# dark-Stallion/alac

Measured on AMD Instinct MI355X. Metric: encode Msamples/s (bit-exact) 44.1kHz/16-bit stereo, 1/2/4/8 GPU, higher is better.
Workload: dtype int32 (int16 PCM, int16 coefficients)

## Files before the change

alac_amd/csrc/alac_capi.hip:

```cpp
#include "alac_hip.h"
#include "alac_dev.hpp"
#include "alac_kernels.hpp"
#include "alac_verify.hpp"
#include "alac_encode_v1_types.hpp"
#include "alac_host.hpp"

#include <cstdio>
#include <cstdlib>
#include <cstring>
#include <new>
#include <string>
#include <vector>

using namespace alacdev;
using namespace alachost;

struct alac_hip_ctx {
    int device = 0;
    hipStream_t stream = nullptr;
    bool ownStream = false;
    std::string err;
    bool profile = false;
    std::vector<hipEvent_t> events;
    uint32_t profCalls = 0;
    std::vector<bool> profLane;
    V1Streams vs{};
    bool vsReady = false;
    hipStream_t mcStream = nullptr;
    hipEvent_t mcFork = nullptr, mcJoin = nullptr;
    bool mcReady = false;
    uint32_t *errHost = nullptr;
    uint32_t *errDev = nullptr;
    uint64_t *tabHost = nullptr;
    uint64_t tabCap = 0;
    hipEvent_t tabDone = nullptr;
    AlacOptions opt;
};

namespace alacdev {

const AlacOptionKey *alac_option_keys(uint32_t *count)
{
    static const AlacOptionKey table[] = {
        {"thru", "ALAC_HIP_THRU", &AlacOptions::thru, -1, 1},
        {"narrow", "ALAC_HIP_NARROW", &AlacOptions::narrow, -1, 1},
        {"split_coder", "ALAC_HIP_SPLIT_CODER", &AlacOptions::splitCoder, 0, 1},
        {"overlap_pos", "ALAC_HIP_OVERLAP_POS", &AlacOptions::overlapPos, 0, 1},
        {"fused", "ALAC_HIP_FUSED", &AlacOptions::fused, 0, 1},
        {"fold", "ALAC_HIP_FOLD", &AlacOptions::fold, 0, 1},
        {"fast_mode", nullptr, &AlacOptions::fastMode, 0, 1},
        {"encoder_lane", "ALAC_HIP_ENCODER", &AlacOptions::laneEncoder, 0, 1},
        {"decoder_lane", "ALAC_HIP_DECODER", &AlacOptions::laneDecoder, 0, 1},
        {"dec_fused", "ALAC_HIP_DEC_FUSED", &AlacOptions::decFused, -1, 1},
        {"dec_pair", "ALAC_HIP_DEC_PAIR", &AlacOptions::decPair, 0, 1},
        {"dec_direct", "ALAC_HIP_DEC_DIRECT", &AlacOptions::decDirect, 0, 2},
        {"stage_taps", "ALAC_HIP_STAGE_TAPS", &AlacOptions::stageTaps, 0, 1},
        {"lpc", nullptr, &AlacOptions::lpc, 0, 1},
        {"debug_lose_handoff", "ALAC_HIP_DEBUG_LOSE_HANDOFF", &AlacOptions::loseHandoff, 0, 1},
        {"debug_waves", nullptr, &AlacOptions::debugWaves, 0, 1},
    };
    if (count) *count = (uint32_t)(sizeof(table) / sizeof(table[0]));
    return table;
}

AlacOptions alac_options_from_env()
{
    AlacOptions o;
    uint32_t n = 0;
    const AlacOptionKey *t = alac_option_keys(&n);
    for (uint32_t i = 0; i < n; i++) {
        const char *v = t[i].env ? getenv(t[i].env) : nullptr;
        if (!v || !*v) continue;
        const bool lane = t[i].slot == &AlacOptions::laneEncoder || t[i].slot == &AlacOptions::laneDecoder;
        if (lane && strcmp(v, "lane") == 0) v = "1";
        char *end = nullptr;
        const long x = strtol(v, &end, 10);
        if (*end == '\0' && x >= t[i].lo && x <= t[i].hi) o.*(t[i].slot) = (int32_t)x;
    }
    return o;
}

const AlacOptionKey *alac_option_find(const char *key)
{
    if (!key) return nullptr;
    uint32_t n = 0;
    const AlacOptionKey *t = alac_option_keys(&n);
    for (uint32_t i = 0; i < n; i++)
        if (strcmp(t[i].name, key) == 0) return t + i;
    return nullptr;
}

}

namespace {

int32_t fail(alac_hip_ctx *ctx, int32_t code, const char *what, hipError_t e = hipSuccess)
{
    if (ctx) {
        ctx->err = what;
        if (e != hipSuccess) {
            ctx->err += ": ";
            ctx->err += hipGetErrorString(e);
        }
    }
    return code;
}

auto on_fail(alac_hip_ctx *ctx) { return [ctx](int32_t code, const char *what, hipError_t e) { return fail(ctx, code, what, e); }; }

bool format_ok(const alac_hip_format *f)
{
    if (!f) return false;
    if (!(f->bit_depth == 16 || f->bit_depth == 20 || f->bit_depth == 24 || f->bit_depth == 32)) return false;
    if (f->num_channels < 1 || f->num_channels > kMaxChannels) return false;
    if (f->frame_size == 0 || f->frame_size > (1u << 20)) return false;
    return true;
}

inline uint64_t align_up(uint64_t x, uint64_t a) { return (x + a - 1) / a * a; }

const uint8_t *read_cookie(const uint8_t *ck, uint32_t size, alac_hip_format *out)
{
    if (!ck || !out) return nullptr;
    for (const char *atom : {"frma", "alac"})
        if (size >= 12 && memcmp(ck + 4, atom, 4) == 0) {
            ck += 12;
            size -= 12;
        }
    if (size < 24 || ck[4] > 0) return nullptr;
    out->frame_size = ((uint32_t)ck[0] << 24) | ((uint32_t)ck[1] << 16) | ((uint32_t)ck[2] << 8) | ck[3];
    out->bit_depth = ck[5];
    out->num_channels = ck[9];
    out->sample_rate = ((uint32_t)ck[20] << 24) | ((uint32_t)ck[21] << 16) | ((uint32_t)ck[22] << 8) | ck[23];
    return ck;
}

HandoffCtl handoff_ctl(const alac_hip_ctx *ctx)
{
    HandoffCtl h;
    h.err = ctx->errDev;
    h.lose = ctx->opt.loseHandoff ? 1u : 0u;
    h.spinLimit = h.lose ? (1u << 8) : (1u << 22);
    return h;
}

bool ensure_second_stream(alac_hip_ctx *ctx)
{
    if (ctx->mcReady) return true;
    if (hipStreamCreateWithFlags(&ctx->mcStream, hipStreamNonBlocking) != hipSuccess ||
        hipEventCreateWithFlags(&ctx->mcFork, hipEventDisableTiming) != hipSuccess ||
        hipEventCreateWithFlags(&ctx->mcJoin, hipEventDisableTiming) != hipSuccess)
        return false;
    ctx->mcReady = true;
    return true;
}

int32_t check_handoff(alac_hip_ctx *ctx)
{
    if (!ctx->errHost) return ALAC_HIP_noErr;
    volatile uint32_t *w = (volatile uint32_t *)ctx->errHost;
    if (w[1] != 0) {
        w[1] = 0;
        w[0] = 0;
        return fail(ctx, ALAC_HIP_ParamError,
                    "d_seg_first is not ascending inside [0, num_packets] or a segment is longer than max_segment_packets: the "
                    "results of the calls since the last synchronize are invalid");
    }
    if (w[0] == 0) return ALAC_HIP_noErr;
    w[0] = 0;
    return fail(ctx, ALAC_HIP_MemFullError,
                "an in-launch producer/consumer hand-off timed out: the results of the calls since the last synchronize are invalid");
}

struct EncLayout {
    uint64_t recs, bitWords, pred, total;
    uint32_t wcap;
    uint64_t predStride;
    uint64_t resA, resB, resC, bits1, cost2, state, flags, rowReady, cls, colChain;
    uint64_t bitWordsB, bitsB;
    uint64_t segBad;
    uint32_t chainsPad, colsPad;
};

EncLayout enc_layout(const alac_hip_format *f, uint32_t numPackets, uint32_t numSegments)
{
    EncLayout L;
    const uint64_t escapeBits = (uint64_t)f->frame_size * f->bit_depth * f->num_channels + 32 + 16;
    L.wcap = (uint32_t)(((escapeBits + 31) / 32 + 44 + 3) & ~3ull);
    if (f->bit_depth == 24) L.wcap += 4;
    if (const char *e = getenv("ALAC_HIP_WCAP_PAD")) L.wcap += (uint32_t)atoi(e) & ~3u;
    const uint64_t lanes = align_up((uint64_t)numSegments * f->num_channels, 64);
    L.predStride = lanes;
    uint64_t off = 0;
    L.recs = off;
    off = align_up(off + (uint64_t)numPackets * sizeof(PacketRec), 256);
    L.bitWords = off;
    off = align_up(off + ((uint64_t)numPackets + 1) * 2 * L.wcap * 4, 256);
    L.pred = off;
    off = align_up(off + (uint64_t)(f->frame_size / 8 + 1) * lanes * 4, 256);
    L.chainsPad = (uint32_t)lanes;
    const uint64_t n8 = f->frame_size / 8 + 1 + 16;
    L.resA = off;
    off = align_up(off + (f->num_channels == 2 ? n8 * 5 * lanes * 4 : 0), 256);
    L.resB = off;
    off = align_up(off + n8 * 2 * lanes * 4, 256);
    L.colsPad = (uint32_t)lanes + 256;
    L.resC = off;
    off = align_up(off + ((uint64_t)f->frame_size + 16) * L.colsPad * 4, 256);
    L.bits1 = off;
    off = align_up(off + 5 * lanes * 4, 256);
    L.cost2 = off;
    off = align_up(off + 2 * lanes * 4, 256);
    L.state = off;
    off = align_up(off + (uint64_t)numSegments * 128, 256);
    L.flags = off;
    off = align_up(off + 2 * (lanes / 8 + 16) * 4, 256);
    L.rowReady = off;
    off = align_up(off + lanes * 4, 256);
    L.cls = off;
    off = align_up(off + 256 + ((uint64_t)numSegments / 1024 + 2) * 8, 256);
    L.colChain = off;
    off = align_up(off + (uint64_t)L.colsPad * 4, 256);
    L.bitWordsB = L.bitsB = 0;
    if (lanes <= kSplitCoderMaxChains) {
        L.bitWordsB = off;
        off = align_up(off + ((uint64_t)numPackets + 1) * 2 * L.wcap * 4, 256);
        L.bitsB = off;
        off = align_up(off + ((uint64_t)numPackets + 1) * 2 * 4, 256);
    }
    L.segBad = off;
    off += 256;
    L.total = off;
    return L;
}

bool use_lane_encoder(const alac_hip_ctx *ctx) { return ctx->opt.laneEncoder != 0; }

alac_hip_format element_format(const alac_hip_format *f, uint32_t channels)
{
    alac_hip_format e = *f;
    e.num_channels = channels;
    return e;
}

uint64_t max_output_bytes(const alac_hip_format *fmt, uint32_t num_packets)
{
    const uint64_t elems = fmt->num_channels > 2 ? fmt->num_channels : 1;
    const uint64_t per = ((uint64_t)fmt->frame_size * fmt->num_channels * fmt->bit_depth + 55 * elems + 3 + 7) / 8;
    return align_up(per * num_packets + 8, 16);
}

struct McGroup {
    uint32_t channels, count, elem[kMaxChannels];
    uint64_t gather, sub, subBytes, out, outCap, sizes, offs, ns, seg, state;
};

struct McLayout {
    uint32_t numElements;
    McElement el[kMaxChannels];
    uint32_t groupOf[kMaxChannels], indexInGroup[kMaxChannels];
    McGroup g[2];
    uint64_t elemBits, total;
};

McLayout mc_layout(const alac_hip_format *f, uint32_t numPackets, uint32_t numSegments)
{
    McLayout M;
    M.numElements = channel_elements(f->num_channels, M.el);
    M.g[0].channels = 2;
    M.g[1].channels = 1;
    M.g[0].count = M.g[1].count = 0;
    for (uint32_t e = 0; e < M.numElements; e++) {
        McGroup &G = M.g[M.el[e].channels == 2 ? 0 : 1];
        M.groupOf[e] = M.el[e].channels == 2 ? 0 : 1;
        M.indexInGroup[e] = G.count;
        G.elem[G.count++] = e;
    }
    uint64_t off = 0;
    for (int gi = 0; gi < 2; gi++) {
        McGroup &G = M.g[gi];
        const alac_hip_format gf = element_format(f, G.channels);
        const uint64_t subPackets = (uint64_t)G.count * numPackets, subSegments = (uint64_t)G.count * numSegments;
        G.gather = off;
        off = align_up(off + subPackets * f->frame_size * G.channels * bytes_per_sample(f->bit_depth) + 64, 256);
        G.sub = off;
        G.subBytes = G.count ? enc_layout(&gf, (uint32_t)subPackets, (uint32_t)subSegments).total : 0;
        off = align_up(off + G.subBytes, 256);
        G.outCap = max_output_bytes(&gf, (uint32_t)subPackets);
        G.out = off;
        off = align_up(off + G.outCap + 16, 256);
        G.sizes = off;
        off = align_up(off + subPackets * 4, 256);
        G.offs = off;
        off = align_up(off + (subPackets + 1) * 8, 256);
        G.ns = off;
        off = align_up(off + subPackets * 4, 256);
        G.seg = off;
        off = align_up(off + (subSegments + 1) * 4, 256);
        G.state = off;
        off = align_up(off + subSegments * ALAC_HIP_STATE_INT16 * 2, 256);
    }
    M.elemBits = off;
    off = align_up(off + (uint64_t)M.numElements * numPackets * 4, 256);
    M.total = off;
    return M;
}

struct DecLayout {
    uint64_t recs, resid, words, capWords, prog, elemBit, mismatch, total;
    uint32_t maxElems;
};

DecLayout dec_layout(const alac_hip_format *f, uint32_t numPackets, uint64_t streamBytes = 0)
{
    DecLayout L;
    uint64_t off = 0;
    L.recs = off;
    L.maxElems = f->num_channels;
    off = align_up(off + (uint64_t)numPackets * L.maxElems * sizeof(DecRec), 256);
    L.resid = off;
    off = align_up(off + (uint64_t)f->num_channels * f->frame_size * numPackets * 4 + 256, 256);
    L.prog = off;
    off = align_up(off + (uint64_t)numPackets * 28 + 64, 256);
    L.elemBit = off;
    off = align_up(off + (uint64_t)numPackets * 4, 256);
    L.mismatch = off;
    off = align_up(off + 4, 256);
    L.words = off;
    const uint64_t regular = (uint64_t)numPackets * max_output_bytes(f, 1);
    L.capWords = ((streamBytes > regular ? streamBytes : regular) + 3) / 4 + 64;
    off = align_up(off + L.capWords * 4, 256);
    L.total = off;
    return L;
}

uint64_t lpc_table_bytes(uint32_t numPackets) { return align_up((uint64_t)numPackets * 2 * sizeof(LpcChan), 256); }

bool use_lane_decoder(const alac_hip_ctx *ctx) { return ctx->opt.laneDecoder != 0; }

int32_t host_segment_refusal(alac_hip_ctx *ctx, const uint32_t *h_seg_first, uint32_t num_segments, uint32_t num_packets)
{
    if (h_seg_first[0] != 0 || h_seg_first[num_segments] != num_packets)
        return fail(ctx, ALAC_HIP_ParamError, "segment table must start at 0 and end at num_packets");
    for (uint32_t s = 0; s < num_segments; s++)
        if (h_seg_first[s] > h_seg_first[s + 1]) return fail(ctx, ALAC_HIP_ParamError, "segment table not ascending");
    if (hipSetDevice(ctx->device) != hipSuccess) return fail(ctx, ALAC_HIP_ParamError, "hipSetDevice");
    return ALAC_HIP_noErr;
}

}

extern "C" {

int32_t alac_hip_device_count(void)
{
    int n = 0;
    if (hipGetDeviceCount(&n) != hipSuccess) return -1;
    return n;
}

int32_t alac_hip_create(alac_hip_ctx **out_ctx, int32_t device, void *stream)
{
    if (!out_ctx) return ALAC_HIP_ParamError;
    *out_ctx = nullptr;
    int n = 0;
    if (hipGetDeviceCount(&n) != hipSuccess || device < 0 || device >= n) return ALAC_HIP_ParamError;
    alac_hip_ctx *c = new (std::nothrow) alac_hip_ctx;
    if (!c) return ALAC_HIP_MemFullError;
    c->device = device;
    c->opt = alac_options_from_env();
    if (hipSetDevice(device) != hipSuccess) {
        delete c;
        return ALAC_HIP_ParamError;
    }
    if (stream) {
        c->stream = (hipStream_t)stream;
    } else {
        if (hipStreamCreateWithFlags(&c->stream, hipStreamNonBlocking) != hipSuccess) {
            delete c;
            return ALAC_HIP_MemFullError;
        }
        c->ownStream = true;
    }
    if (hipHostMalloc((void **)&c->errHost, 64, hipHostMallocMapped) != hipSuccess ||
        hipHostGetDevicePointer((void **)&c->errDev, c->errHost, 0) != hipSuccess) {
        alac_hip_destroy(c);
        return ALAC_HIP_MemFullError;
    }
    c->errHost[0] = c->errHost[1] = 0;
    *out_ctx = c;
    return ALAC_HIP_noErr;
}

void alac_hip_destroy(alac_hip_ctx *ctx)
{
    if (!ctx) return;
    for (hipEvent_t e : ctx->events) (void)hipEventDestroy(e);
    ctx->events.clear();
    (void)hipSetDevice(ctx->device);
    if (ctx->vsReady) {
        (void)hipStreamSynchronize(ctx->vs.side[0]);
        (void)hipStreamDestroy(ctx->vs.side[0]);
        for (uint32_t i = 0; i < kSideEvents; i++) {
            (void)hipEventDestroy(ctx->vs.stagger[i]);
            (void)hipEventDestroy(ctx->vs.join[i]);
        }
        (void)hipEventDestroy(ctx->vs.fork);
    }
    if (ctx->mcReady) {
        (void)hipStreamSynchronize(ctx->mcStream);
        (void)hipStreamDestroy(ctx->mcStream);
        (void)hipEventDestroy(ctx->mcFork);
        (void)hipEventDestroy(ctx->mcJoin);
    }
    if (ctx->ownStream && ctx->stream) {
        (void)hipStreamSynchronize(ctx->stream);
        (void)hipStreamDestroy(ctx->stream);
    }
    if (ctx->errHost) (void)hipHostFree(ctx->errHost);
    if (ctx->tabDone) (void)hipEventDestroy(ctx->tabDone);
    if (ctx->tabHost) (void)hipHostFree(ctx->tabHost);
    delete ctx;
}

int32_t alac_hip_synchronize(alac_hip_ctx *ctx)
{
    if (!ctx) return ALAC_HIP_ParamError;
    hipError_t e = hipStreamSynchronize(ctx->stream);
    if (e != hipSuccess) return fail(ctx, ALAC_HIP_ParamError, "hipStreamSynchronize", e);
    return check_handoff(ctx);
}

int32_t alac_hip_set_option(alac_hip_ctx *ctx, const char *key, int32_t value)
{
    if (!ctx) return ALAC_HIP_ParamError;
    const AlacOptionKey *k = alac_option_find(key);
    if (!k) return fail(ctx, ALAC_HIP_ParamError, "unknown option");
    if (value < k->lo || value > k->hi) return fail(ctx, ALAC_HIP_ParamError, "option value outside its documented range");
    ctx->opt.*(k->slot) = value;
    return ALAC_HIP_noErr;
}

int32_t alac_hip_get_option(alac_hip_ctx *ctx, const char *key, int32_t *value)
{
    if (!ctx || !value) return ALAC_HIP_ParamError;
    const AlacOptionKey *k = alac_option_find(key);
    if (!k) return fail(ctx, ALAC_HIP_ParamError, "unknown option");
    *value = ctx->opt.*(k->slot);
    return ALAC_HIP_noErr;
}

uint64_t alac_hip_debug_waves_offset(const alac_hip_format *fmt, uint32_t num_packets, uint32_t num_segments)
{
    if (!format_ok(fmt) || fmt->num_channels > 2) return 0;
    return enc_layout(fmt, num_packets, num_segments ? num_segments : num_packets).rowReady;
}

const char *alac_hip_encode_regime(alac_hip_ctx *ctx, const alac_hip_format *fmt, uint32_t num_segments)
{
    if (!ctx || !format_ok(fmt)) return "";
    return v1_regime_name(v1_plan(fmt->num_channels, num_segments, 1, fmt->frame_size, ctx->opt).shape);
}

const char *alac_hip_last_error(const alac_hip_ctx *ctx) { return ctx ? ctx->err.c_str() : "null context"; }

void *alac_hip_stream(const alac_hip_ctx *ctx) { return ctx ? (void *)ctx->stream : nullptr; }

uint64_t alac_hip_encode_workspace_bytes(const alac_hip_format *fmt, uint32_t num_packets, uint32_t num_segments)
{
    if (!format_ok(fmt)) return 0;
    if (fmt->num_channels > 2) return mc_layout(fmt, num_packets, num_segments ? num_segments : num_packets).total;
    return enc_layout(fmt, num_packets, num_segments ? num_segments : num_packets).total + lpc_table_bytes(num_packets);
}

uint32_t alac_hip_state_int16(const alac_hip_format *fmt)
{
    if (!format_ok(fmt)) return 0;
    McElement el[kMaxChannels];
    return ALAC_HIP_STATE_INT16 * (fmt->num_channels > 2 ? channel_elements(fmt->num_channels, el) : 1);
}

uint64_t alac_hip_encode_max_output_bytes(const alac_hip_format *fmt, uint32_t num_packets)
{
    if (!format_ok(fmt)) return 0;
    return max_output_bytes(fmt, num_packets);
}

enum class SegKind {
    Host,
    Bound,
    Unread,
};

struct EncodeCall {
    alac_hip_format fmt;
    const void *pcm;
    const uint32_t *numSamples;
    uint32_t numPackets;
    const uint32_t *segFirst;
    uint32_t numSegments;
    SegKind segKind;
    uint32_t maxSeg;
    int16_t *state;
    int32_t stateIn;
    uint8_t *ws, *out;
    uint32_t *packetBytes;
    uint64_t *offsets;
    hipStream_t stream;
    bool lpc;
    bool fast;
    bool timed;
};

static EncodeCall describe_encode(const alac_hip_ctx *ctx, const alac_hip_format *fmt, const void *pcm,
                                  const uint32_t *num_samples, uint32_t num_packets, const uint32_t *seg_first,
                                  uint32_t num_segments, uint32_t max_segment_packets, int16_t *state, int32_t state_in,
                                  void *ws, uint8_t *out, uint32_t *packet_bytes, uint64_t *offsets)
{
    const bool lpc = ctx->opt.lpc != 0;
    const uint32_t *seg = lpc ? nullptr : seg_first;
    const SegKind kind = !seg ? SegKind::Host : max_segment_packets ? SegKind::Bound : SegKind::Unread;
    return {*fmt, pcm, num_samples, num_packets, seg, seg ? num_segments : num_packets, kind, seg ? max_segment_packets : 1,
            lpc ? nullptr : state, lpc ? 0 : state_in, (uint8_t *)ws, out, packet_bytes, offsets, ctx->stream, lpc,
            ctx->opt.fastMode != 0, true};
}

static int32_t encode_refusal(alac_hip_ctx *ctx, const alac_hip_format *fmt, uint32_t np, uint32_t num_segments,
                              const EncodeCall *b, uint64_t workspace_bytes, uint64_t out_capacity)
{
    const bool mc = fmt->num_channels > 2, lpc = ctx->opt.lpc != 0;
    if (mc && lpc) return fail(ctx, ALAC_HIP_ParamError, "option lpc: mono and stereo streams only");
    if (lpc) {
        if (ctx->opt.fastMode) return fail(ctx, ALAC_HIP_ParamError, "options lpc and fast_mode exclude each other");
        if ((uint64_t)fmt->frame_size * fmt->num_channels * 4 > 65536)
            return fail(ctx, ALAC_HIP_ParamError, "option lpc: frame_size x channels above 16 384");
    }
    if (np == 0) return ALAC_HIP_noErr;
    if (b && (!b->pcm || !b->ws || !b->out || !b->packetBytes || !b->offsets)) return fail(ctx, ALAC_HIP_ParamError, "null buffer");
    if (num_segments == 0 || num_segments > np) return fail(ctx, ALAC_HIP_ParamError, "bad segment count");
    if (mc) {
        if (b && ((uintptr_t)b->ws & 255)) return fail(ctx, ALAC_HIP_ParamError, "misaligned workspace (256 B)");
        if ((uint64_t)np * kMaxChannels > 0x7fffffffull) return fail(ctx, ALAC_HIP_ParamError, "too many packets");
        if (b && workspace_bytes < mc_layout(fmt, np, num_segments).total)
            return fail(ctx, ALAC_HIP_ParamError, "workspace too small");
    } else if (b) {
        if (((uintptr_t)b->out & 3) || ((uintptr_t)b->ws & 255) || ((uintptr_t)b->pcm & 15))
            return fail(ctx, ALAC_HIP_ParamError, "misaligned buffer (out 4 B, pcm 16 B, workspace 256 B)");
        if (workspace_bytes < enc_layout(fmt, np, num_segments).total + (lpc ? lpc_table_bytes(np) : 0))
            return fail(ctx, ALAC_HIP_ParamError, lpc ? "workspace too small (option lpc: size it for num_segments = num_packets)"
                                                      : "workspace too small");
    }
    if (b && out_capacity < max_output_bytes(fmt, np))
        return fail(ctx, ALAC_HIP_ParamError, "output capacity below alac_hip_encode_max_output_bytes");
    return ALAC_HIP_noErr;
}

static int32_t read_max_segment(alac_hip_ctx *ctx, hipStream_t st, const uint32_t *d_seg_first, uint32_t num_segments,
                                uint32_t num_packets, uint32_t &maxSeg)
{
    std::vector<uint32_t> sf(num_segments + 1);
    if (hipMemcpyAsync(sf.data(), d_seg_first, (num_segments + 1) * 4ull, hipMemcpyDeviceToHost, st) != hipSuccess ||
        hipStreamSynchronize(st) != hipSuccess)
        return fail(ctx, ALAC_HIP_ParamError, "reading d_seg_first");
    maxSeg = 0;
    for (uint32_t s = 0; s < num_segments; s++) {
        if (sf[s + 1] < sf[s] || sf[s + 1] > num_packets) return fail(ctx, ALAC_HIP_ParamError, "bad d_seg_first");
        maxSeg = sf[s + 1] - sf[s] > maxSeg ? sf[s + 1] - sf[s] : maxSeg;
    }
    return ALAC_HIP_noErr;
}

static V1Args v1_args(const alac_hip_ctx *ctx, const EncodeArgs &ea, const EncLayout &L, uint8_t *ws, const V1Plan &P,
                      bool stateInternal)
{
    V1Args A{};
    A.S = {ea.pcm, ea.numSamples, ea.segFirst, ea.numSegments, ea.frameSize, 0, 0, ea.numSegments, ea.numPackets, ea.segMax};
    A.state = stateInternal ? (int16_t *)(ws + L.state) : ea.state;
    A.recs = ea.recs;
    A.resA = (int32_t *)(ws + L.resA);
    A.resB = (int32_t *)(ws + L.resB);
    A.resC = (int32_t *)(ws + L.resC);
    A.bits1 = (uint32_t *)(ws + L.bits1);
    A.cost2 = (uint32_t *)(ws + L.cost2);
    A.chainsPad = L.chainsPad;
    A.bitWords = ea.bitWords;
    A.wcap = ea.wcap;
    A.dumpSlot = ea.numPackets * 2;
    A.packetBytes = ea.packetBytes;
    A.flags = (uint32_t *)(ws + L.flags);
    A.flagsF = A.ovFlagsF = A.flags + (L.chainsPad / 8 + 16);
    A.ovRowReady = (uint32_t *)(ws + L.rowReady);
    A.dbg = ctx->opt.debugWaves ? A.ovRowReady : nullptr;
    A.virgin = stateInternal && !P.fast ? 1u : 0u;
    A.foldDecide = P.shape == V1Shape::Latency ? 1u : 0u;
    A.idleFast = P.shape == V1Shape::Throughput ? 0u : 1u;
    A.ho = handoff_ctl(ctx);
    A.cls = (ClassInfo *)(ws + L.cls);
    A.colChain = (uint32_t *)(ws + L.colChain);
    A.colsPad = L.colsPad;
    A.bitWordsB = P.split ? (uint32_t *)(ws + L.bitWordsB) : nullptr;
    A.bitsB = L.bitsB ? (uint32_t *)(ws + L.bitsB) : nullptr;
    A.splitAt = v1_split_at(ea.frameSize);
    return A;
}

static int32_t encode_core(alac_hip_ctx *ctx, const EncodeCall &c)
{
    const alac_hip_format *fmt = &c.fmt;
    const uint32_t num_packets = c.numPackets;
    const EncLayout L = enc_layout(fmt, num_packets, c.numSegments);
    uint8_t *ws = c.ws;
    EncodeArgs ea;
    ea.pcm = (const uint8_t *)c.pcm;
    ea.numSamples = c.numSamples;
    ea.segFirst = c.segFirst;
    ea.numSegments = c.numSegments;
    ea.frameSize = fmt->frame_size;
    ea.state = c.state;
    ea.stateIn = c.stateIn;
    ea.pred = (int32_t *)(ws + L.pred);
    ea.predStride = L.predStride;
    ea.bitWords = (uint32_t *)(ws + L.bitWords);
    ea.wcap = L.wcap;
    ea.recs = (PacketRec *)(ws + L.recs);
    ea.packetBytes = c.packetBytes;
    const bool bound = c.segKind == SegKind::Bound;
    ea.numPackets = num_packets;
    ea.segMax = bound ? (c.maxSeg < num_packets ? c.maxSeg : num_packets) : 0xffffffffu;
    ea.segBad = bound ? (uint32_t *)(ws + L.segBad) : nullptr;
    PackArgs pa;
    pa.pcm = ea.pcm;
    pa.recs = ea.recs;
    pa.bitWords = ea.bitWords;
    pa.wcap = L.wcap;
    pa.frameSize = fmt->frame_size;
    pa.offsets = c.offsets;
    pa.out = c.out;
    pa.segBad = ea.segBad;
    constexpr uint32_t EV = kEventBlocks * (kNumStages + 1);
    hipEvent_t *ev = nullptr;
    if (c.timed && ctx->profile && (uint64_t)(ctx->profCalls + 1) * EV <= ctx->events.size())
        ev = &ctx->events[ctx->profCalls++ * EV];
    if (ev) ctx->profLane.push_back(use_lane_encoder(ctx));
    hipError_t e;
    if (bound && (e = launch_check_segments(c.segFirst, c.numSegments, num_packets, ea.segMax, ctx->errDev ? ctx->errDev + 1 : nullptr,
                                            ea.segBad, c.stream)))
        return fail(ctx, ALAC_HIP_ParamError, "segment check launch", e);
    if (use_lane_encoder(ctx)) {
        e = launch_encode(fmt->bit_depth, fmt->num_channels, ea, pa, num_packets, c.stream, ev ? ev + (kNumStages + 1) : nullptr);
    } else {
        if (!ctx->vsReady) {
            bool ok = hipEventCreateWithFlags(&ctx->vs.fork, hipEventDisableTiming) == hipSuccess &&
                      hipStreamCreateWithFlags(&ctx->vs.side[0], hipStreamNonBlocking) == hipSuccess;
            for (uint32_t i = 0; ok && i < kSideEvents; i++)
                ok = hipEventCreateWithFlags(&ctx->vs.stagger[i], hipEventDisableTiming) == hipSuccess &&
                     hipEventCreateWithFlags(&ctx->vs.join[i], hipEventDisableTiming) == hipSuccess;
            if (!ok) return fail(ctx, ALAC_HIP_MemFullError, "creating side streams");
            ctx->vsReady = true;
        }
        uint32_t maxSeg = bound ? ea.segMax : c.maxSeg;
        if (c.segKind == SegKind::Unread)
            if (int32_t rc = read_max_segment(ctx, c.stream, c.segFirst, c.numSegments, num_packets, maxSeg)) return rc;
        AlacOptions opt = ctx->opt;
        opt.fastMode = c.fast ? 1 : 0;
        const V1Plan P = v1_plan(fmt->num_channels, c.numSegments, maxSeg, fmt->frame_size, opt);
        const V1Args A = v1_args(ctx, ea, L, ws, P, c.state == nullptr);
        const bool initState = !(c.state && c.stateIn) && !A.virgin;
        e = launch_encode_v1(fmt->bit_depth, fmt->num_channels, A, P, initState, pa, ctx->vs, num_packets, maxSeg, c.stream, ev);
    }
    if (e != hipSuccess) return fail(ctx, ALAC_HIP_ParamError, "encode launch", e);
    if (c.lpc) {
        LpcArgs la;
        la.pcm = ea.pcm;
        la.frameSize = fmt->frame_size;
        la.recs = ea.recs;
        la.packetBytes = c.packetBytes;
        la.bitWords = ea.bitWords;
        la.wcap = L.wcap;
        la.lpc = (LpcChan *)(ws + L.total);
        e = launch_lpc(fmt->bit_depth, fmt->num_channels, la, num_packets, c.stream);
        if (e != hipSuccess) return fail(ctx, ALAC_HIP_ParamError, "lpc launch", e);
        pa.lpc = la.lpc;
        e = launch_scan_pack(fmt->bit_depth, fmt->num_channels, c.packetBytes, pa, num_packets, c.stream, nullptr);
        if (e != hipSuccess) return fail(ctx, ALAC_HIP_ParamError, "lpc pack launch", e);
    }
    return ALAC_HIP_noErr;
}

static int32_t encode_elements(alac_hip_ctx *ctx, const EncodeCall &c)
{
    const alac_hip_format *fmt = &c.fmt;
    const uint32_t num_packets = c.numPackets;
    const McLayout M = mc_layout(fmt, num_packets, c.numSegments);
    uint8_t *ws = c.ws;
    const uint32_t bps = bytes_per_sample(fmt->bit_depth);

    const bool side = M.g[0].count && M.g[1].count;
    if (side && !ensure_second_stream(ctx)) return fail(ctx, ALAC_HIP_MemFullError, "creating the second stream");
    hipError_t e;
    if (side && ((e = hipEventRecord(ctx->mcFork, c.stream)) || (e = hipStreamWaitEvent(ctx->mcStream, ctx->mcFork, 0))))
        return fail(ctx, ALAC_HIP_ParamError, "forking the second stream", e);
    int32_t rc = ALAC_HIP_noErr;
    hipError_t copyErr = hipSuccess;
    for (int gi = 0; gi < 2 && rc == ALAC_HIP_noErr; gi++) {
        const McGroup &G = M.g[gi];
        if (!G.count) continue;
        hipStream_t st = (side && gi == 1) ? ctx->mcStream : c.stream;
        const uint64_t elemPcm = (uint64_t)num_packets * fmt->frame_size * G.channels * bps;
        e = hipSuccess;
        for (uint32_t k = 0; k < G.count && e == hipSuccess; k++)
            e = launch_mc_gather((const uint8_t *)c.pcm, ws + G.gather + k * elemPcm, c.numSamples, num_packets, fmt->frame_size,
                                 fmt->num_channels, M.el[G.elem[k]].first, G.channels, bps, st);
        uint32_t *ns = c.numSamples ? (uint32_t *)(ws + G.ns) : nullptr;
        uint32_t *seg = c.segFirst ? (uint32_t *)(ws + G.seg) : nullptr;
        if (e == hipSuccess) e = launch_mc_tables(c.numSamples, num_packets, c.segFirst, c.numSegments, G.count, ns, seg, st);
        if (e != hipSuccess) {
            rc = fail(ctx, ALAC_HIP_ParamError, "element gather launch", e);
            break;
        }
        int16_t *gstate = c.state ? (int16_t *)(ws + G.state) : nullptr;
        const uint64_t rowBytes = (uint64_t)c.numSegments * ALAC_HIP_STATE_INT16 * 2;
        if (gstate && c.stateIn)
            for (uint32_t k = 0; k < G.count && copyErr == hipSuccess; k++)
                copyErr = hipMemcpyAsync((uint8_t *)gstate + k * rowBytes, (const uint8_t *)c.state + G.elem[k] * rowBytes,
                                         rowBytes, hipMemcpyDeviceToDevice, st);
        const EncodeCall g{element_format(fmt, G.channels), ws + G.gather, ns, G.count * num_packets, seg,
                           G.count * c.numSegments, c.segKind, c.maxSeg, gstate, c.stateIn, ws + G.sub, ws + G.out,
                           (uint32_t *)(ws + G.sizes), (uint64_t *)(ws + G.offs), st, false, false, false};
        rc = encode_core(ctx, g);
        if (gstate && rc == ALAC_HIP_noErr)
            for (uint32_t k = 0; k < G.count && copyErr == hipSuccess; k++)
                copyErr = hipMemcpyAsync((uint8_t *)c.state + G.elem[k] * rowBytes, (const uint8_t *)gstate + k * rowBytes,
                                         rowBytes, hipMemcpyDeviceToDevice, st);
    }
    if (side && ((e = hipEventRecord(ctx->mcJoin, ctx->mcStream)) || (e = hipStreamWaitEvent(c.stream, ctx->mcJoin, 0))) &&
        rc == ALAC_HIP_noErr)
        rc = fail(ctx, ALAC_HIP_ParamError, "joining the second stream", e);
    if (rc != ALAC_HIP_noErr) return rc;
    if (copyErr != hipSuccess) return fail(ctx, ALAC_HIP_ParamError, "coefficient state copy", copyErr);
    McSpliceArgs sa;
    sa.numElements = M.numElements;
    sa.numPackets = num_packets;
    for (uint32_t el = 0; el < M.numElements; el++) {
        const McGroup &G = M.g[M.groupOf[el]];
        sa.el[el] = M.el[el];
        sa.src[el] = ws + G.out;
        sa.srcOffsets[el] = (const uint64_t *)(ws + G.offs) + (uint64_t)M.indexInGroup[el] * num_packets;
    }
    sa.elemBits = (uint32_t *)(ws + M.elemBits);
    sa.packetBytes = c.packetBytes;
    sa.offsets = c.offsets;
    sa.out = c.out;
    e = launch_mc_splice(sa, c.stream);
    if (e != hipSuccess) return fail(ctx, ALAC_HIP_ParamError, "splice launch", e);
    return ALAC_HIP_noErr;
}

static int32_t encode_device(alac_hip_ctx *ctx, const alac_hip_format *fmt, const void *d_pcm, const uint32_t *d_num_samples,
                             uint32_t num_packets, const uint32_t *d_seg_first, uint32_t num_segments,
                             uint32_t max_segment_packets, int16_t *d_state, int32_t state_in, void *d_workspace,
                             uint64_t workspace_bytes, uint8_t *d_out, uint64_t out_capacity, uint32_t *d_packet_bytes,
                             uint64_t *d_packet_offsets)
{
    if (!ctx) return ALAC_HIP_ParamError;
    if (!format_ok(fmt)) return fail(ctx, ALAC_HIP_ParamError, "unsupported format");
    const EncodeCall c = describe_encode(ctx, fmt, d_pcm, d_num_samples, num_packets, d_seg_first, num_segments,
                                         max_segment_packets, d_state, state_in, d_workspace, d_out, d_packet_bytes,
                                         d_packet_offsets);
    if (int32_t rc = encode_refusal(ctx, fmt, num_packets, c.numSegments, &c, workspace_bytes, out_capacity)) return rc;
    if (num_packets == 0) return ALAC_HIP_noErr;
    if (hipSetDevice(ctx->device) != hipSuccess) return fail(ctx, ALAC_HIP_ParamError, "hipSetDevice");
    return (c.fmt.num_channels > 2 ? encode_elements : encode_core)(ctx, c);
}

int32_t alac_hip_encode_segmented(alac_hip_ctx *ctx, const alac_hip_format *fmt, const void *d_pcm,
                                  const uint32_t *d_num_samples, uint32_t num_packets, const uint32_t *d_seg_first,
                                  uint32_t num_segments, uint32_t max_segment_packets, int16_t *d_state, int32_t state_in,
                                  void *d_workspace, uint64_t workspace_bytes, uint8_t *d_out, uint64_t out_capacity,
                                  uint32_t *d_packet_bytes, uint64_t *d_packet_offsets)
{
    return encode_device(ctx, fmt, d_pcm, d_num_samples, num_packets, d_seg_first, num_segments, max_segment_packets, d_state,
                         state_in, d_workspace, workspace_bytes, d_out, out_capacity, d_packet_bytes, d_packet_offsets);
}

int32_t alac_hip_encode(alac_hip_ctx *ctx, const alac_hip_format *fmt, const void *d_pcm,
                        const uint32_t *d_num_samples, uint32_t num_packets, const uint32_t *d_seg_first,
                        uint32_t num_segments, int16_t *d_state, int32_t state_in, void *d_workspace,
                        uint64_t workspace_bytes, uint8_t *d_out, uint64_t out_capacity,
                        uint32_t *d_packet_bytes, uint64_t *d_packet_offsets)
{
    return encode_device(ctx, fmt, d_pcm, d_num_samples, num_packets, d_seg_first, num_segments, 0, d_state, state_in,
                         d_workspace, workspace_bytes, d_out, out_capacity, d_packet_bytes, d_packet_offsets);
}

static uint64_t float_stage_bytes(const alac_hip_format *fmt, uint32_t num_packets)
{
    return align_up((uint64_t)num_packets * fmt->frame_size * fmt->num_channels * bytes_per_sample(fmt->bit_depth) + 64, 256);
}

uint64_t alac_hip_encode_float_workspace_bytes(const alac_hip_format *fmt, uint32_t num_packets, uint32_t num_segments)
{
    if (!format_ok(fmt)) return 0;
    return align_up(alac_hip_encode_workspace_bytes(fmt, num_packets, num_segments), 256) + float_stage_bytes(fmt, num_packets);
}

static int32_t float_stride_refusal(alac_hip_ctx *ctx, const alac_hip_format *fmt, uint32_t num_packets, uint64_t channel_stride,
                                    uint64_t frame_stride)
{
    const uint32_t C = fmt->num_channels;
    if (frame_stride == 0) return fail(ctx, ALAC_HIP_ParamError, "frame_stride 0");
    if (channel_stride == 0 && C > 1) return fail(ctx, ALAC_HIP_ParamError, "channel_stride 0 with more than one channel");
    uint64_t rows, cols, last;
    if (__builtin_mul_overflow((uint64_t)(C - 1), channel_stride, &rows) ||
        __builtin_mul_overflow((uint64_t)num_packets * fmt->frame_size - 1, frame_stride, &cols) ||
        __builtin_add_overflow(rows, cols, &last) || last > UINT64_MAX / sizeof(float))
        return fail(ctx, ALAC_HIP_ParamError, "the largest index into d_in overflows 64 bits");
    return ALAC_HIP_noErr;
}

static const char *dither_refusal(const alac_hip_format *fmt, const alac_hip_dither *dither, const uint64_t *packet_origin)
{
    if (!dither) return nullptr;
    if (dither->mode > ALAC_HIP_DITHER_TPDF) return "unknown dither mode";
    if (dither->reserved != 0) return "alac_hip_dither.reserved is not 0";
    if (dither->mode == ALAC_HIP_DITHER_NONE) return nullptr;
    if (fmt->bit_depth == 32) return "no dither at 32 bits: a float32 carries nothing below a 32-bit LSB";
    if ((uintptr_t)packet_origin & 7) return "misaligned packet origin table (8 B)";
    return nullptr;
}
static bool dither_on(const alac_hip_dither *dither) { return dither && dither->mode == ALAC_HIP_DITHER_TPDF; }

static int32_t float_host_span(alac_hip_ctx *ctx, const alac_hip_format *fmt, const uint32_t *h_num_samples, uint32_t np,
                               uint64_t channel_stride, uint64_t frame_stride, uint64_t &span)
{
    const uint32_t fs = fmt->frame_size;
    span = 0;
    for (uint32_t p = 0; p < np; p++) {
        const uint32_t n = h_num_samples && h_num_samples[p] < fs ? h_num_samples[p] : fs;
        if (!n) continue;
        uint64_t rows, cols, last;
        if (__builtin_mul_overflow((uint64_t)(fmt->num_channels - 1), channel_stride, &rows) ||
            __builtin_mul_overflow((uint64_t)p * fs + n - 1, frame_stride, &cols) || __builtin_add_overflow(rows, cols, &last) ||
            last >= UINT64_MAX / sizeof(float))
            return fail(ctx, ALAC_HIP_ParamError, "the largest index into h_in overflows 64 bits");
        span = last + 1 > span ? last + 1 : span;
    }
    return ALAC_HIP_noErr;
}

static int32_t encode_float_run(alac_hip_ctx *ctx, const EncodeCall &c, const float *d_in, uint64_t channel_stride,
                                uint64_t frame_stride, uint32_t *d_clipped, const alac_hip_dither *dither = nullptr,
                                const uint64_t *d_origin = nullptr)
{
    const FloatInArgs a{d_in,        channel_stride,     frame_stride,    c.numSamples, c.numPackets, c.fmt.frame_size,
                        c.fmt.num_channels, (uint8_t *)c.pcm, d_clipped};
    FloatDitherArgs dz = {};
    if (dither_on(dither)) {
        dz.origin = d_origin;
        philox_round_keys(dither->seed, dz.roundKey);
    }
    const hipError_t e = launch_float_to_pcm(c.fmt.bit_depth, a, c.stream, dither_on(dither) ? &dz : nullptr);
    if (e != hipSuccess) return fail(ctx, ALAC_HIP_ParamError, "float conversion launch", e);
    return (c.fmt.num_channels > 2 ? encode_elements : encode_core)(ctx, c);
}

int32_t alac_hip_encode_float(alac_hip_ctx *ctx, const alac_hip_format *fmt, const float *d_in, uint64_t channel_stride,
                              uint64_t frame_stride, const uint32_t *d_num_samples, uint32_t num_packets,
                              const uint32_t *d_seg_first, uint32_t num_segments, uint32_t max_segment_packets,
                              int16_t *d_state, int32_t state_in, void *d_workspace, uint64_t workspace_bytes, uint8_t *d_out,
                              uint64_t out_capacity, uint32_t *d_packet_bytes, uint64_t *d_packet_offsets,
                              uint32_t *d_clipped)
{
    return alac_hip_encode_float_dither(ctx, fmt, d_in, channel_stride, frame_stride, d_num_samples, num_packets, d_seg_first,
                                        num_segments, max_segment_packets, d_state, state_in, d_workspace, workspace_bytes,
                                        d_out, out_capacity, d_packet_bytes, d_packet_offsets, d_clipped, nullptr, nullptr);
}

int32_t alac_hip_encode_float_dither(alac_hip_ctx *ctx, const alac_hip_format *fmt, const float *d_in, uint64_t channel_stride,
                                     uint64_t frame_stride, const uint32_t *d_num_samples, uint32_t num_packets,
                                     const uint32_t *d_seg_first, uint32_t num_segments, uint32_t max_segment_packets,
                                     int16_t *d_state, int32_t state_in, void *d_workspace, uint64_t workspace_bytes,
                                     uint8_t *d_out, uint64_t out_capacity, uint32_t *d_packet_bytes,
                                     uint64_t *d_packet_offsets, uint32_t *d_clipped, const alac_hip_dither *dither,
                                     const uint64_t *d_packet_origin)
{
    if (!ctx) return ALAC_HIP_ParamError;
    if (!format_ok(fmt)) return fail(ctx, ALAC_HIP_ParamError, "unsupported format");
    if (const char *why = dither_refusal(fmt, dither, d_packet_origin)) return fail(ctx, ALAC_HIP_ParamError, why);
    EncodeCall c = describe_encode(ctx, fmt, nullptr, d_num_samples, num_packets, d_seg_first, num_segments, max_segment_packets,
                                   d_state, state_in, d_workspace, d_out, d_packet_bytes, d_packet_offsets);
    if (num_packets == 0) return encode_refusal(ctx, fmt, 0, c.numSegments, &c, workspace_bytes, out_capacity);
    if (!d_in) return fail(ctx, ALAC_HIP_ParamError, "null d_in");
    if ((uintptr_t)d_in & 3) return fail(ctx, ALAC_HIP_ParamError, "misaligned d_in (4 B)");
    if (int32_t rc = float_stride_refusal(ctx, fmt, num_packets, channel_stride, frame_stride)) return rc;
    const uint64_t stage = float_stage_bytes(fmt, num_packets);
    if (workspace_bytes < stage) return fail(ctx, ALAC_HIP_ParamError, "workspace too small");
    const uint64_t encBytes = (workspace_bytes - stage) & ~255ull;
    c.pcm = d_workspace ? (uint8_t *)d_workspace + encBytes : nullptr;
    if (int32_t rc = encode_refusal(ctx, fmt, num_packets, c.numSegments, &c, encBytes, out_capacity)) return rc;
    if (c.segKind == SegKind::Unread && fmt->num_channels <= 2 && !use_lane_encoder(ctx)) {
        if (int32_t rc = read_max_segment(ctx, c.stream, c.segFirst, c.numSegments, num_packets, c.maxSeg)) return rc;
        c.segKind = SegKind::Host;
    }
    if (hipSetDevice(ctx->device) != hipSuccess) return fail(ctx, ALAC_HIP_ParamError, "hipSetDevice");
    return encode_float_run(ctx, c, d_in, channel_stride, frame_stride, d_clipped, dither, d_packet_origin);
}

uint64_t alac_hip_float_probe_workspace_bytes(uint32_t num_segments)
{
    return num_segments ? align_up(((uint64_t)num_segments + 1) * 8, 256) : 0;
}

static int32_t float_probe_refusal(alac_hip_ctx *ctx, const float *in, uint32_t num_channels, uint64_t channel_stride,
                                   uint64_t frame_stride, uint64_t total_frames, const uint64_t *h_seg_first_frame,
                                   uint32_t num_segments, uint64_t &lo, uint64_t &hi)
{
    if (!in) return fail(ctx, ALAC_HIP_ParamError, "null input");
    if ((uintptr_t)in & 3) return fail(ctx, ALAC_HIP_ParamError, "misaligned input (4 B)");
    if (num_channels < 1 || num_channels > kMaxChannels) return fail(ctx, ALAC_HIP_ParamError, "num_channels outside 1..8");
    if (frame_stride == 0) return fail(ctx, ALAC_HIP_ParamError, "frame_stride 0");
    if (channel_stride == 0 && num_channels > 1)
        return fail(ctx, ALAC_HIP_ParamError, "channel_stride 0 with more than one channel");
    uint64_t rows, cols, last;
    if (total_frames &&
        (__builtin_mul_overflow((uint64_t)(num_channels - 1), channel_stride, &rows) ||
         __builtin_mul_overflow(total_frames - 1, frame_stride, &cols) || __builtin_add_overflow(rows, cols, &last) ||
         last >= UINT64_MAX / sizeof(float)))
        return fail(ctx, ALAC_HIP_ParamError, "the largest index into the input overflows 64 bits");
    if (num_segments == 0) return fail(ctx, ALAC_HIP_ParamError, "num_segments 0");
    lo = 0, hi = total_frames;
    if (!h_seg_first_frame)
        return num_segments == 1 ? ALAC_HIP_noErr : fail(ctx, ALAC_HIP_ParamError, "no segment table for more than one segment");
    for (uint32_t s = 0; s < num_segments; s++)
        if (h_seg_first_frame[s] > h_seg_first_frame[s + 1]) return fail(ctx, ALAC_HIP_ParamError, "segment table not ascending");
    if (h_seg_first_frame[num_segments] > total_frames)
        return fail(ctx, ALAC_HIP_ParamError, "segment table ends behind total_frames");
    lo = h_seg_first_frame[0], hi = h_seg_first_frame[num_segments];
    return ALAC_HIP_noErr;
}

static hipError_t upload_segment_table(alac_hip_ctx *ctx, const uint64_t *h_table, uint64_t entries, void *d_dst)
{
    hipError_t e;
    if (!ctx->tabDone && (e = hipEventCreateWithFlags(&ctx->tabDone, hipEventDisableTiming))) return e;
    if (ctx->tabHost && (e = hipEventSynchronize(ctx->tabDone))) return e;
    if (entries > ctx->tabCap) {
        if (ctx->tabHost) (void)hipHostFree(ctx->tabHost);
        ctx->tabHost = nullptr, ctx->tabCap = 0;
        const uint64_t cap = entries < 1024 ? 1024 : entries;
        if ((e = hipHostMalloc((void **)&ctx->tabHost, cap * 8, hipHostMallocDefault))) return e;
        ctx->tabCap = cap;
    }
    memcpy(ctx->tabHost, h_table, entries * 8);
    if ((e = hipMemcpyAsync(d_dst, ctx->tabHost, entries * 8, hipMemcpyHostToDevice, ctx->stream))) return e;
    return hipEventRecord(ctx->tabDone, ctx->stream);
}

int32_t alac_hip_float_probe(alac_hip_ctx *ctx, const float *d_in, uint32_t num_channels, uint64_t channel_stride,
                             uint64_t frame_stride, uint64_t total_frames, const uint64_t *h_seg_first_frame,
                             uint32_t num_segments, void *d_workspace, uint64_t workspace_bytes,
                             alac_hip_float_report *d_reports)
{
    if (!ctx) return ALAC_HIP_ParamError;
    uint64_t lo, hi;
    if (int32_t rc = float_probe_refusal(ctx, d_in, num_channels, channel_stride, frame_stride, total_frames, h_seg_first_frame,
                                         num_segments, lo, hi))
        return rc;
    if (!d_reports || ((uintptr_t)d_reports & 7)) return fail(ctx, ALAC_HIP_ParamError, "null or misaligned d_reports (8 B)");
    if (workspace_bytes < alac_hip_float_probe_workspace_bytes(num_segments))
        return fail(ctx, ALAC_HIP_ParamError, "workspace too small");
    if (h_seg_first_frame && (!d_workspace || ((uintptr_t)d_workspace & 7)))
        return fail(ctx, ALAC_HIP_ParamError, "null or misaligned workspace (8 B)");
    if (hipSetDevice(ctx->device) != hipSuccess) return fail(ctx, ALAC_HIP_ParamError, "hipSetDevice");
    hipError_t e;
    if (h_seg_first_frame && (e = upload_segment_table(ctx, h_seg_first_frame, (uint64_t)num_segments + 1, d_workspace)))
        return fail(ctx, ALAC_HIP_ParamError, "segment table upload", e);
    const FloatProbeArgs a{d_in, channel_stride, frame_stride, lo, hi, h_seg_first_frame ? (const uint64_t *)d_workspace : nullptr,
                           num_segments, num_channels, (uint32_t *)d_reports};
    if ((e = launch_float_probe(a, ctx->stream))) return fail(ctx, ALAC_HIP_ParamError, "float probe launch", e);
    return ALAC_HIP_noErr;
}

uint32_t alac_hip_float_report_depth(const alac_hip_float_report *r)
{
    if (!r || r->nan || r->over_range || r->need_bits > 32) return 0;
    return r->need_bits <= 16 ? 16 : r->need_bits <= 20 ? 20 : r->need_bits <= 24 ? 24 : 32;
}

uint64_t alac_hip_pcm_crc32_workspace_bytes(uint32_t num_ranges)
{
    return num_ranges ? align_up((uint64_t)num_ranges * 16, 256) : 0;
}

static int32_t pcm_crc_refusal(alac_hip_ctx *ctx, const void *pcm, uint64_t total_bytes, const uint64_t *h_ranges,
                               uint32_t num_ranges, uint64_t &lo, uint64_t &hi)
{
    if (!pcm && total_bytes) return fail(ctx, ALAC_HIP_ParamError, "null PCM");
    if (num_ranges == 0) return fail(ctx, ALAC_HIP_ParamError, "num_ranges 0");
    lo = 0, hi = total_bytes;
    if (!h_ranges) return num_ranges == 1 ? ALAC_HIP_noErr : fail(ctx, ALAC_HIP_ParamError, "no range table for more than one range");
    uint64_t at = 0;
    for (uint32_t s = 0; s < num_ranges; s++) {
        uint64_t end;
        if (h_ranges[2 * s] < at) return fail(ctx, ALAC_HIP_ParamError, "range table not ascending, or ranges overlap");
        if (__builtin_add_overflow(h_ranges[2 * s], h_ranges[2 * s + 1], &end))
            return fail(ctx, ALAC_HIP_ParamError, "a range's end overflows 64 bits");
        at = end;
    }
    if (at > total_bytes) return fail(ctx, ALAC_HIP_ParamError, "range table ends behind total_bytes");
    lo = h_ranges[0], hi = at;
    return ALAC_HIP_noErr;
}

int32_t alac_hip_pcm_crc32(alac_hip_ctx *ctx, const void *d_pcm, uint64_t total_bytes, const uint64_t *h_ranges,
                           uint32_t num_ranges, void *d_workspace, uint64_t workspace_bytes, alac_hip_pcm_digest *d_digests)
{
    if (!ctx) return ALAC_HIP_ParamError;
    uint64_t lo, hi;
    if (int32_t rc = pcm_crc_refusal(ctx, d_pcm, total_bytes, h_ranges, num_ranges, lo, hi)) return rc;
    if (!d_digests || ((uintptr_t)d_digests & 7)) return fail(ctx, ALAC_HIP_ParamError, "null or misaligned d_digests (8 B)");
    if (h_ranges && workspace_bytes < alac_hip_pcm_crc32_workspace_bytes(num_ranges))
        return fail(ctx, ALAC_HIP_ParamError, "workspace too small");
    if (h_ranges && (!d_workspace || ((uintptr_t)d_workspace & 7)))
        return fail(ctx, ALAC_HIP_ParamError, "null or misaligned workspace (8 B)");
    if (hipSetDevice(ctx->device) != hipSuccess) return fail(ctx, ALAC_HIP_ParamError, "hipSetDevice");
    hipError_t e;
    if (h_ranges && (e = upload_segment_table(ctx, h_ranges, (uint64_t)num_ranges * 2, d_workspace)))
        return fail(ctx, ALAC_HIP_ParamError, "range table upload", e);
    const PcmCrcArgs a{(const uint8_t *)d_pcm, lo, hi, h_ranges ? (const uint64_t *)d_workspace : nullptr, num_ranges,
                       (uint32_t *)d_digests};
    if ((e = launch_pcm_crc(a, ctx->stream))) return fail(ctx, ALAC_HIP_ParamError, "pcm crc launch", e);
    return ALAC_HIP_noErr;
}

uint32_t alac_hip_crc32_combine(uint32_t crc_a, uint32_t crc_b, uint64_t len_b)
{
    return crc_mul_host(crc_a, crc_x8_pow(len_b)) ^ crc_b;
}

uint32_t alac_hip_num_stages(void) { return kNumStages; }

const char *alac_hip_stage_name(uint32_t stage)
{
    static const char *names[kNumStages] = {"lms_search1", "golomb_count1", "lms_search2", "golomb_count2",
                                            "lms_final",   "golomb_final",  "finalize_scan", "pack"};
    return stage < kNumStages ? names[stage] : "";
}

int32_t alac_hip_profile_begin(alac_hip_ctx *ctx, uint32_t max_calls)
{
    if (!ctx) return ALAC_HIP_ParamError;
    if (hipSetDevice(ctx->device) != hipSuccess) return fail(ctx, ALAC_HIP_ParamError, "hipSetDevice");
    while (ctx->events.size() < (size_t)max_calls * kEventBlocks * (kNumStages + 1)) {
        hipEvent_t e;
        if (hipEventCreate(&e) != hipSuccess) return fail(ctx, ALAC_HIP_MemFullError, "hipEventCreate");
        ctx->events.push_back(e);
    }
    ctx->profCalls = 0;
    ctx->profLane.clear();
    ctx->profile = max_calls != 0;
    return ALAC_HIP_noErr;
}

int32_t alac_hip_profile_end(alac_hip_ctx *ctx, uint32_t *out_calls, float *out_stage_ms, uint32_t *out_launches)
{
    if (!ctx) return ALAC_HIP_ParamError;
    ctx->profile = false;
    hipError_t e = hipStreamSynchronize(ctx->stream);
    if (e != hipSuccess) return fail(ctx, ALAC_HIP_ParamError, "hipStreamSynchronize", e);
    constexpr uint32_t BLK = kNumStages + 1;
    constexpr uint32_t EV = kEventBlocks * BLK;
    double t[kNumStages] = {0};
    double launches[kNumStages] = {0};
    auto elapsed = [&](hipEvent_t a, hipEvent_t b, double &acc) -> bool {
        float ms = 0;
        if (hipEventElapsedTime(&ms, a, b) != hipSuccess) return false;
        acc += ms;
        return true;
    };
    for (uint32_t c = 0; c < ctx->profCalls; c++) {
        hipEvent_t *base = &ctx->events[(size_t)c * EV];
        for (uint32_t k = 0; k < kNumStages; k++) {
            hipEvent_t *blk = (ctx->profLane[c] || k >= kStageScan) ? base + BLK : base;
            if (!elapsed(blk[k], blk[k + 1], t[k])) return fail(ctx, ALAC_HIP_ParamError, "hipEventElapsedTime");
            launches[k] += 1;
        }
    }
    if (out_calls) *out_calls = ctx->profCalls;
    const double n = ctx->profCalls ? ctx->profCalls : 1;
    for (uint32_t k = 0; k < kNumStages; k++) {
        if (out_stage_ms) out_stage_ms[k] = launches[k] > 0 ? (float)(t[k] / launches[k]) : 0.0f;
        if (out_launches) out_launches[k] = (uint32_t)(launches[k] / n + 0.5);
    }
    return ALAC_HIP_noErr;
}

uint32_t alac_hip_magic_cookie(const alac_hip_format *fmt, uint32_t max_frame_bytes, uint32_t avg_bit_rate,
                               uint8_t *c)
{
    if (!format_ok(fmt) || !c) return 0;
    auto be32 = [](uint8_t *p, uint32_t v) {
        p[0] = (uint8_t)(v >> 24);
        p[1] = (uint8_t)(v >> 16);
        p[2] = (uint8_t)(v >> 8);
        p[3] = (uint8_t)v;
    };
    be32(c + 0, fmt->frame_size);
    c[4] = 0;
    c[5] = (uint8_t)fmt->bit_depth;
    c[6] = (uint8_t)kPB0;
    c[7] = (uint8_t)kMB0;
    c[8] = (uint8_t)kKB0;
    c[9] = (uint8_t)fmt->num_channels;
    c[10] = 0;
    c[11] = 255;
    be32(c + 12, max_frame_bytes);
    be32(c + 16, avg_bit_rate);
    be32(c + 20, fmt->sample_rate);
    return 24;
}

uint32_t alac_hip_magic_cookie_size(const alac_hip_format *fmt)
{
    if (!format_ok(fmt)) return 0;
    return fmt->num_channels > 2 ? 48 : 24;
}

uint32_t alac_hip_magic_cookie_full(const alac_hip_format *fmt, uint32_t max_frame_bytes, uint32_t avg_bit_rate,
                                    uint8_t *c, uint32_t capacity)
{
    const uint32_t need = alac_hip_magic_cookie_size(fmt);
    if (!need || !c || capacity < need) return 0;
    alac_hip_magic_cookie(fmt, max_frame_bytes, avg_bit_rate, c);
    if (need == 24) return 24;
    static const uint32_t tags[kMaxChannels] = {(100u << 16) | 1, (101u << 16) | 2, (113u << 16) | 3, (116u << 16) | 4,
                                                (120u << 16) | 5, (124u << 16) | 6, (142u << 16) | 7, (127u << 16) | 8};
    memset(c + 24, 0, 24);
    c[27] = 24;
    memcpy(c + 28, "chan", 4);
    const uint32_t t = tags[fmt->num_channels - 1];
    c[36] = (uint8_t)t;
    c[37] = (uint8_t)(t >> 8);
    c[38] = (uint8_t)(t >> 16);
    c[39] = (uint8_t)(t >> 24);
    return 48;
}

int32_t alac_hip_format_from_cookie(const uint8_t *ck, uint32_t size, alac_hip_format *out)
{
    return read_cookie(ck, size, out) ? ALAC_HIP_noErr : ALAC_HIP_ParamError;
}

uint64_t alac_hip_decode_workspace_bytes(const alac_hip_format *fmt, uint32_t num_packets)
{
    return alac_hip_decode_workspace_bytes_stream(fmt, num_packets, 0);
}

uint64_t alac_hip_decode_workspace_bytes_stream(const alac_hip_format *fmt, uint32_t num_packets, uint64_t stream_bytes)
{
    if (!format_ok(fmt)) return 0;
    return dec_layout(fmt, num_packets, stream_bytes).total;
}

}

namespace {
int32_t parse_cookie(alac_hip_ctx *ctx, const uint8_t *cookie, uint32_t size, alac_hip_format &fmt, DecodeArgs &da)
{
    if (!ctx) return ALAC_HIP_ParamError;
    const uint8_t *ck = read_cookie(cookie, size, &fmt);
    if (!ck) return fail(ctx, ALAC_HIP_ParamError, "bad magic cookie");
    if (!format_ok(&fmt)) return fail(ctx, ALAC_HIP_ParamError, "unsupported format in cookie");
    da.frameSize = fmt.frame_size;
    da.bitDepth = fmt.bit_depth;
    da.numChannels = fmt.num_channels;
    da.pb = ck[6];
    da.mb = ck[7];
    da.kb = ck[8];
    da.frameBytes = fmt.num_channels * bytes_per_sample(fmt.bit_depth);
    return ALAC_HIP_noErr;
}

void decode_buffers(DecodeArgs &da, const uint8_t *stream, const uint64_t *offsets, uint32_t num_packets, const void *pcm_out,
                    uint32_t *num_samples_out, int32_t *status)
{
    da.stream = stream;
    da.offsets = offsets;
    da.numPackets = num_packets;
    da.pcmOut = (uint8_t *)pcm_out;
    da.numSamplesOut = num_samples_out;
    da.statusOut = status;
}

int32_t decode_impl(alac_hip_ctx *ctx, const alac_hip_format &fmt, DecodeArgs da, void *d_workspace, uint64_t workspace_bytes)
{
    const uint32_t num_packets = da.numPackets;
    if (num_packets == 0) return ALAC_HIP_noErr;
    if (!da.stream || !da.offsets || !d_workspace || !da.pcmOut || !da.numSamplesOut || !da.statusOut)
        return fail(ctx, ALAC_HIP_ParamError, "null buffer");
    if (((uintptr_t)d_workspace & 255) || ((uintptr_t)da.pcmOut & 3)) return fail(ctx, ALAC_HIP_ParamError, "misaligned buffer");
    DecLayout L = dec_layout(&fmt, num_packets);
    if (workspace_bytes < L.total) return fail(ctx, ALAC_HIP_ParamError, "workspace too small");
    L.capWords = (workspace_bytes - L.words) / 4;
    if (hipSetDevice(ctx->device) != hipSuccess) return fail(ctx, ALAC_HIP_ParamError, "hipSetDevice");
    if (da.kb < 1 || da.kb > 16 || da.pb == 0) return fail(ctx, ALAC_HIP_ParamError, "bad AG parameters in cookie (pb / kb)");
    uint8_t *ws = (uint8_t *)d_workspace;
    da.maxElems = L.maxElems;
    da.recs = (DecRec *)(ws + L.recs);
    da.resid = (int32_t *)(ws + L.resid);
    da.ho = handoff_ctl(ctx);
    da.optFused = ctx->opt.decFused;
    da.optPair = ctx->opt.decPair;
    da.optDirect = ctx->opt.decDirect;
    hipError_t e;
    if (use_lane_decoder(ctx)) {
        e = launch_decode(da, ctx->stream);
    } else if (fmt.num_channels > 2) {
        McElement el[kMaxChannels];
        const uint32_t nel = channel_elements(fmt.num_channels, el);
        e = launch_decode_v1_elements(da, el, nel, (uint32_t *)(ws + L.words), L.capWords, da.resid, (uint32_t *)(ws + L.prog),
                                      (uint32_t *)(ws + L.elemBit), (uint32_t *)(ws + L.mismatch), ctx->stream);
        uint32_t mismatch = 0;
        if (e == hipSuccess) e = hipMemcpyAsync(&mismatch, ws + L.mismatch, 4, hipMemcpyDeviceToHost, ctx->stream);
        if (e == hipSuccess) e = hipStreamSynchronize(ctx->stream);
        if (e == hipSuccess && mismatch) e = launch_decode(da, ctx->stream);
    } else {
        e = launch_decode_v1(da, (uint32_t *)(ws + L.words), L.capWords, da.resid, (uint32_t *)(ws + L.prog), ctx->stream,
                             (uint32_t *)(ws + L.mismatch));
        if (e == hipSuccess) {
            DecodeArgs dg = da;
            dg.gate = (const uint32_t *)(ws + L.mismatch);
            e = launch_decode(dg, ctx->stream);
        }
    }
    if (e != hipSuccess) return fail(ctx, ALAC_HIP_ParamError, "decode launch", e);
    return ALAC_HIP_noErr;
}

uint64_t verify_ns_bytes(uint32_t numPackets) { return align_up((uint64_t)numPackets * 4, 256); }

VerifyFloatArgs verify_float_args(uint64_t channel_stride, uint64_t frame_stride, const alac_hip_dither *dither,
                                  const uint64_t *d_origin)
{
    VerifyFloatArgs vf = {};
    vf.channelStride = channel_stride;
    vf.frameStride = frame_stride;
    if (dither_on(dither)) {
        vf.dither = 1;
        vf.dz.origin = d_origin;
        philox_round_keys(dither->seed, vf.dz.roundKey);
    }
    return vf;
}

int32_t verify_impl(alac_hip_ctx *ctx, const alac_hip_format &fmt, DecodeArgs da, uint32_t *d_first_mismatch,
                    const uint32_t *d_num_samples_expected, void *d_workspace, uint64_t workspace_bytes, uint32_t *d_bad_packets,
                    const VerifyFloatArgs *vf = nullptr)
{
    const uint32_t num_packets = da.numPackets;
    VerifyFloatArgs block;
    if (vf) {
        block = *vf;
        block.firstMismatch = d_first_mismatch;
        block.numSamplesExpected = d_num_samples_expected;
        da.pcmMode = kPcmVerifyFloat;
        da.verifyFloat = &block;
    } else {
        da.pcmMode = kPcmVerify;
        da.firstMismatch = d_first_mismatch;
    }
    if (!d_bad_packets) return fail(ctx, ALAC_HIP_ParamError, "null buffer");
    if (hipSetDevice(ctx->device) != hipSuccess) return fail(ctx, ALAC_HIP_ParamError, "hipSetDevice");
    if (num_packets == 0) {
        const hipError_t e = hipMemsetAsync(d_bad_packets, 0, 4, ctx->stream);
        return e == hipSuccess ? ALAC_HIP_noErr : fail(ctx, ALAC_HIP_ParamError, "verify launch", e);
    }
    if (!da.stream || !da.offsets || !d_workspace || !da.pcmOut || !d_first_mismatch || !da.statusOut)
        return fail(ctx, ALAC_HIP_ParamError, "null buffer");
    if (((uintptr_t)d_workspace & 255) || ((uintptr_t)da.pcmOut & 3)) return fail(ctx, ALAC_HIP_ParamError, "misaligned buffer");
    const DecLayout L = dec_layout(&fmt, num_packets);
    const uint64_t nsBytes = verify_ns_bytes(num_packets);
    if (workspace_bytes < nsBytes + L.total) return fail(ctx, ALAC_HIP_ParamError, "workspace too small");
    uint8_t *ws = (uint8_t *)d_workspace;
    da.numSamplesOut = (uint32_t *)ws;
    hipError_t e = launch_verify_init(d_first_mismatch, num_packets, d_bad_packets, ctx->stream);
    if (e != hipSuccess) return fail(ctx, ALAC_HIP_ParamError, "verify launch", e);
    if (int32_t rc = decode_impl(ctx, fmt, da, ws + nsBytes, workspace_bytes - nsBytes)) return rc;
    e = launch_verify_finish(da.statusOut, da.numSamplesOut, d_num_samples_expected, fmt.frame_size, num_packets,
                             d_first_mismatch, d_bad_packets, ctx->stream);
    if (e != hipSuccess) return fail(ctx, ALAC_HIP_ParamError, "verify launch", e);
    return ALAC_HIP_noErr;
}

int32_t verify_float_refusal(alac_hip_ctx *ctx, const alac_hip_format &fmt, uint32_t num_packets, const float *in,
                             uint64_t channel_stride, uint64_t frame_stride, const alac_hip_dither *dither,
                             const uint64_t *packet_origin)
{
    if (const char *why = dither_refusal(&fmt, dither, packet_origin)) return fail(ctx, ALAC_HIP_ParamError, why);
    if (num_packets == 0) return ALAC_HIP_noErr;
    if (!in) return fail(ctx, ALAC_HIP_ParamError, "null d_in");
    if ((uintptr_t)in & 3) return fail(ctx, ALAC_HIP_ParamError, "misaligned d_in (4 B)");
    return float_stride_refusal(ctx, &fmt, num_packets, channel_stride, frame_stride);
}

int32_t decode_host_common(alac_hip_ctx *ctx, const alac_hip_format &fmt, DecodeArgs &da, const uint8_t *h_stream,
                           const uint32_t *h_packet_bytes, uint32_t num_packets, uint64_t pcmBytes, const void *h_expected,
                           const uint32_t *h_ns_expected, void *h_out, uint32_t rows, uint64_t pitch, uint32_t *h_ns_out,
                           uint32_t *h_fm, uint32_t *bad, int32_t *h_status, const VerifyFloatArgs *vf = nullptr,
                           const uint64_t *h_origin = nullptr)
{
    const bool verify = bad != nullptr;
    if (hipSetDevice(ctx->device) != hipSuccess) return fail(ctx, ALAC_HIP_ParamError, "hipSetDevice");
    const uint64_t n4 = num_packets * 4ull;
    hipStream_t st = ctx->stream;
    DevStream d;
    if (int32_t rc = upload_stream(h_stream, h_packet_bytes, num_packets, st, d, on_fail(ctx))) return rc;
    const uint64_t wsBytes = (verify ? alac_hip_verify_workspace_bytes_stream : alac_hip_decode_workspace_bytes_stream)(
        &fmt, num_packets, d.total);
    DevBuf dWs, dPcm, dNs, dSt, dFm, dBad, dOrigin;
    hipError_t e;
    if ((e = dWs.alloc(wsBytes)) || (e = dPcm.alloc(pcmBytes)) || (e = dNs.alloc(n4)) || (e = dSt.alloc(n4)) ||
        (verify && ((e = dFm.alloc(n4)) || (e = dBad.alloc(4)))) || (h_origin && (e = dOrigin.alloc(num_packets * 8ull))))
        return fail(ctx, ALAC_HIP_MemFullError, "hipMalloc", e);
    if (h_origin && (e = hipMemcpyAsync(dOrigin.p, h_origin, num_packets * 8ull, hipMemcpyHostToDevice, st)))
        return fail(ctx, ALAC_HIP_ParamError, "H2D copy", e);
    if ((e = verify ? hipMemcpyAsync(dPcm.p, h_expected, pcmBytes, hipMemcpyHostToDevice, st)
                    : hipMemsetAsync(dPcm.p, 0, pcmBytes, st)) ||
        (h_ns_expected && (e = hipMemcpyAsync(dNs.p, h_ns_expected, n4, hipMemcpyHostToDevice, st))))
        return fail(ctx, ALAC_HIP_ParamError, "H2D copy", e);
    decode_buffers(da, (const uint8_t *)d.bytes.p, (const uint64_t *)d.offs.p, num_packets, dPcm.p, (uint32_t *)dNs.p,
                   (int32_t *)dSt.p);
    if (verify) {
        const uint32_t *ns = h_ns_expected ? (const uint32_t *)dNs.p : nullptr;
        VerifyFloatArgs block;
        if (vf) {
            block = *vf;
            block.dz.origin = h_origin ? (const uint64_t *)dOrigin.p : nullptr;
        }
        if (int32_t rc = verify_impl(ctx, fmt, da, (uint32_t *)dFm.p, ns, dWs.p, wsBytes, (uint32_t *)dBad.p, vf ? &block : nullptr))
            return rc;
        if (!(e = hipMemcpyAsync(bad, dBad.p, 4, hipMemcpyDeviceToHost, st)) && h_fm)
            e = hipMemcpyAsync(h_fm, dFm.p, n4, hipMemcpyDeviceToHost, st);
    } else {
        if (int32_t rc = decode_impl(ctx, fmt, da, dWs.p, wsBytes)) return rc;
        const uint64_t w = pcmBytes / rows;
        if (!(e = pitch ? hipMemcpy2DAsync(h_out, pitch, dPcm.p, w, w, rows, hipMemcpyDeviceToHost, st)
                        : hipMemcpyAsync(h_out, dPcm.p, pcmBytes, hipMemcpyDeviceToHost, st)))
            e = hipMemcpyAsync(h_ns_out, dNs.p, n4, hipMemcpyDeviceToHost, st);
    }
    if (e || (h_status && (e = hipMemcpyAsync(h_status, dSt.p, n4, hipMemcpyDeviceToHost, st))) || (e = hipStreamSynchronize(st)))
        return fail(ctx, ALAC_HIP_ParamError, verify ? "verify execution" : "decode execution", e);
    return check_handoff(ctx);
}
}

extern "C" {

int32_t alac_hip_decode(alac_hip_ctx *ctx, const uint8_t *h_cookie, uint32_t cookie_size, const uint8_t *d_stream,
                        const uint64_t *d_packet_offsets, uint32_t num_packets, void *d_workspace,
                        uint64_t workspace_bytes, uint8_t *d_pcm_out, uint32_t *d_num_samples_out,
                        int32_t *d_status)
{
    alac_hip_format fmt;
    DecodeArgs da;
    if (int32_t rc = parse_cookie(ctx, h_cookie, cookie_size, fmt, da)) return rc;
    decode_buffers(da, d_stream, d_packet_offsets, num_packets, d_pcm_out, d_num_samples_out, d_status);
    return decode_impl(ctx, fmt, da, d_workspace, workspace_bytes);
}

int32_t alac_hip_decode_float(alac_hip_ctx *ctx, const uint8_t *h_cookie, uint32_t cookie_size, const uint8_t *d_stream,
                              const uint64_t *d_packet_offsets, uint32_t num_packets, void *d_workspace,
                              uint64_t workspace_bytes, float *d_out, uint64_t channel_stride, uint32_t *d_num_samples_out,
                              int32_t *d_status)
{
    alac_hip_format fmt;
    DecodeArgs da;
    if (int32_t rc = parse_cookie(ctx, h_cookie, cookie_size, fmt, da)) return rc;
    if (num_packets == 0) return ALAC_HIP_noErr;
    if (!d_out) return fail(ctx, ALAC_HIP_ParamError, "null buffer");
    if ((uintptr_t)d_out & 3) return fail(ctx, ALAC_HIP_ParamError, "misaligned buffer");
    if (channel_stride < (uint64_t)num_packets * fmt.frame_size)
        return fail(ctx, ALAC_HIP_ParamError, "channel_stride below num_packets * frame_size");
    if (channel_stride > UINT64_MAX / sizeof(float) / fmt.num_channels)
        return fail(ctx, ALAC_HIP_ParamError, "channel_stride * channels overflows");
    decode_buffers(da, d_stream, d_packet_offsets, num_packets, d_out, d_num_samples_out, d_status);
    da.pcmMode = kPcmFloat;
    da.channelStride = channel_stride;
    return decode_impl(ctx, fmt, da, d_workspace, workspace_bytes);
}

uint64_t alac_hip_verify_workspace_bytes_stream(const alac_hip_format *fmt, uint32_t num_packets, uint64_t stream_bytes)
{
    if (!format_ok(fmt)) return 0;
    return verify_ns_bytes(num_packets) + dec_layout(fmt, num_packets, stream_bytes).total;
}

int32_t alac_hip_verify(alac_hip_ctx *ctx, const uint8_t *h_cookie, uint32_t cookie_size, const uint8_t *d_stream,
                        const uint64_t *d_packet_offsets, uint32_t num_packets, const uint8_t *d_pcm_expected,
                        const uint32_t *d_num_samples_expected, void *d_workspace, uint64_t workspace_bytes,
                        uint32_t *d_first_mismatch, int32_t *d_status, uint32_t *d_bad_packets)
{
    alac_hip_format fmt;
    DecodeArgs da;
    if (int32_t rc = parse_cookie(ctx, h_cookie, cookie_size, fmt, da)) return rc;
    decode_buffers(da, d_stream, d_packet_offsets, num_packets, d_pcm_expected, nullptr, d_status);
    return verify_impl(ctx, fmt, da, d_first_mismatch, d_num_samples_expected, d_workspace, workspace_bytes, d_bad_packets);
}

int32_t alac_hip_verify_float(alac_hip_ctx *ctx, const uint8_t *h_cookie, uint32_t cookie_size, const uint8_t *d_stream,
                              const uint64_t *d_packet_offsets, uint32_t num_packets, const float *d_in,
                              uint64_t channel_stride, uint64_t frame_stride, const uint32_t *d_num_samples_expected,
                              const alac_hip_dither *dither, const uint64_t *d_packet_origin, void *d_workspace,
                              uint64_t workspace_bytes, uint32_t *d_first_mismatch, int32_t *d_status, uint32_t *d_bad_packets)
{
    alac_hip_format fmt;
    DecodeArgs da;
    if (int32_t rc = parse_cookie(ctx, h_cookie, cookie_size, fmt, da)) return rc;
    if (int32_t rc = verify_float_refusal(ctx, fmt, num_packets, d_in, channel_stride, frame_stride, dither, d_packet_origin))
        return rc;
    decode_buffers(da, d_stream, d_packet_offsets, num_packets, d_in, nullptr, d_status);
    const VerifyFloatArgs vf = verify_float_args(channel_stride, frame_stride, dither, d_packet_origin);
    return verify_impl(ctx, fmt, da, d_first_mismatch, d_num_samples_expected, d_workspace, workspace_bytes, d_bad_packets, &vf);
}


static int32_t pc_block_any(alac_hip_ctx *ctx, const int32_t *d_in, int32_t *d_out, uint32_t num_rows, uint32_t row_stride,
                            int32_t num, int16_t *d_coefs, int32_t numactive, uint32_t chanbits, uint32_t denshift, bool decode)
{
    if (!ctx || !d_in || !d_out) return ALAC_HIP_ParamError;
    if (numactive < 0 || numactive > 31 || chanbits < 1 || chanbits > 32 || denshift > 15 || num < 0)
        return fail(ctx, ALAC_HIP_ParamError, decode ? "bad unpc_block parameters" : "bad pc_block parameters");
    if (numactive != 0 && numactive != 31 && !d_coefs) return fail(ctx, ALAC_HIP_ParamError, "null coefs");
    hipError_t e = launch_pc_block(d_in, d_out, num_rows, row_stride, num, d_coefs, numactive, chanbits, denshift, decode,
                                   ctx->stream, decode || ctx->opt.stageTaps != 0);
    return e == hipSuccess ? ALAC_HIP_noErr : fail(ctx, ALAC_HIP_ParamError, decode ? "unpc_block launch" : "pc_block launch", e);
}

int32_t alac_hip_pc_block(alac_hip_ctx *ctx, const int32_t *d_in, int32_t *d_pc, uint32_t num_rows,
                          uint32_t row_stride, int32_t num, int16_t *d_coefs, int32_t numactive, uint32_t chanbits,
                          uint32_t denshift)
{
    return pc_block_any(ctx, d_in, d_pc, num_rows, row_stride, num, d_coefs, numactive, chanbits, denshift, false);
}

int32_t alac_hip_unpc_block(alac_hip_ctx *ctx, const int32_t *d_pc, int32_t *d_out, uint32_t num_rows,
                            uint32_t row_stride, int32_t num, int16_t *d_coefs, int32_t numactive,
                            uint32_t chanbits, uint32_t denshift)
{
    return pc_block_any(ctx, d_pc, d_out, num_rows, row_stride, num, d_coefs, numactive, chanbits, denshift, true);
}

int32_t alac_hip_dyn_comp(alac_hip_ctx *ctx, uint32_t mb0, uint32_t pb, uint32_t kb, const int32_t *d_pc,
                          uint32_t num_rows, uint32_t row_stride, int32_t num_samples, int32_t bit_size,
                          uint8_t *d_bits, uint32_t bytes_stride, uint32_t *d_num_bits)
{
    if (!ctx || !d_pc || !d_num_bits) return ALAC_HIP_ParamError;
    if (bit_size < 1 || bit_size > 32 || kb < 1 || kb > 16 || num_samples < 0)
        return fail(ctx, ALAC_HIP_ParamError, "bad dyn_comp parameters");
    if (d_bits && ((bytes_stride & 3) || ((uintptr_t)d_bits & 3)))
        return fail(ctx, ALAC_HIP_ParamError, "bit buffer must be 4-byte aligned/strided");
    hipError_t e = launch_dyn_comp(mb0, pb, kb, d_pc, num_rows, row_stride, num_samples, bit_size, d_bits,
                                   bytes_stride, d_num_bits, ctx->stream);
    return e == hipSuccess ? ALAC_HIP_noErr : fail(ctx, ALAC_HIP_ParamError, "dyn_comp launch", e);
}

int32_t alac_hip_dyn_decomp(alac_hip_ctx *ctx, uint32_t mb0, uint32_t pb, uint32_t kb, const uint8_t *d_bits,
                            uint32_t bytes_stride, uint32_t num_rows, int32_t *d_pc, uint32_t row_stride,
                            int32_t num_samples, int32_t max_size, uint32_t *d_num_bits, int32_t *d_status)
{
    if (!ctx || !d_bits || !d_pc || !d_num_bits || !d_status) return ALAC_HIP_ParamError;
    if (max_size < 1 || max_size > 32 || kb < 1 || kb > 16 || num_samples < 0)
        return fail(ctx, ALAC_HIP_ParamError, "bad dyn_decomp parameters");
    hipError_t e = launch_dyn_decomp(mb0, pb, kb, d_bits, bytes_stride, num_rows, d_pc, row_stride, num_samples,
                                     max_size, d_num_bits, d_status, ctx->stream);
    return e == hipSuccess ? ALAC_HIP_noErr : fail(ctx, ALAC_HIP_ParamError, "dyn_decomp launch", e);
}


static int32_t encode_host_segments(alac_hip_ctx *ctx, const alac_hip_format *fmt, const void *h_pcm,
                                    const uint32_t *h_num_samples, uint32_t num_packets, const uint32_t *h_seg_first,
                                    uint32_t num_segments, int16_t *h_state, int32_t state_in, uint8_t *h_out,
                                    uint64_t out_capacity, uint32_t *h_packet_bytes, uint64_t *out_total_bytes)
{
    if (out_total_bytes) *out_total_bytes = 0;
    if (num_packets == 0) return ALAC_HIP_noErr;
    if (!h_pcm || !h_out || !h_packet_bytes || !h_num_samples || !h_seg_first || num_segments == 0)
        return fail(ctx, ALAC_HIP_ParamError, "null buffer");
    if (int32_t rc = host_segment_refusal(ctx, h_seg_first, num_segments, num_packets)) return rc;
    if (int32_t rc = encode_refusal(ctx, fmt, num_packets, ctx->opt.lpc ? num_packets : num_segments, nullptr, 0, 0)) return rc;
    const uint32_t np = num_packets, nseg = num_segments;
    const uint64_t pcmBytes = (uint64_t)np * fmt->frame_size * fmt->num_channels * bytes_per_sample(fmt->bit_depth);
    const uint64_t wsBytes = alac_hip_encode_workspace_bytes(fmt, np, ctx->opt.lpc ? np : nseg);
    DevBuf dPcm;
    hipError_t e;
    if ((e = dPcm.alloc(pcmBytes))) return fail(ctx, ALAC_HIP_MemFullError, "hipMalloc", e);
    if ((e = hipMemcpyAsync(dPcm.p, h_pcm, pcmBytes, hipMemcpyHostToDevice, ctx->stream)))
        return fail(ctx, ALAC_HIP_ParamError, "H2D copy", e);
    return encode_host_common(
        ctx->stream, fmt, h_num_samples, np, h_seg_first, nseg, h_state, state_in, h_out, out_capacity, h_packet_bytes,
        out_total_bytes, wsBytes,
        [&](uint32_t maxSeg, const uint32_t *ns, const uint32_t *seg, int16_t *state, int32_t stIn, void *ws, uint8_t *out,
            uint64_t, uint32_t *sizes, uint64_t *offs) {
            const EncodeCall c = describe_encode(ctx, fmt, dPcm.p, ns, np, seg, nseg, maxSeg, state, stIn, ws, out, sizes, offs);
            return (c.fmt.num_channels > 2 ? encode_elements : encode_core)(ctx, c);
        },
        on_fail(ctx), [ctx] { return alac_hip_synchronize(ctx); });
}

int32_t alac_hip_encode_host_segments(alac_hip_ctx *ctx, const alac_hip_format *fmt, const void *h_pcm,
                                      const uint32_t *h_num_samples, uint32_t num_packets, const uint32_t *h_seg_first,
                                      uint32_t num_segments, int16_t *h_state, int32_t state_in, uint8_t *h_out,
                                      uint64_t out_capacity, uint32_t *h_packet_bytes, uint64_t *out_total_bytes)
{
    if (!ctx) return ALAC_HIP_ParamError;
    if (!format_ok(fmt)) return fail(ctx, ALAC_HIP_ParamError, "unsupported format");
    return encode_host_segments(ctx, fmt, h_pcm, h_num_samples, num_packets, h_seg_first, num_segments, h_state, state_in,
                                h_out, out_capacity, h_packet_bytes, out_total_bytes);
}

int32_t alac_hip_encode_float_host(alac_hip_ctx *ctx, const alac_hip_format *fmt, const float *h_in, uint64_t channel_stride,
                                   uint64_t frame_stride, const uint32_t *h_num_samples, uint32_t num_packets,
                                   const uint32_t *h_seg_first, uint32_t num_segments, int16_t *h_state, int32_t state_in,
                                   uint8_t *h_out, uint64_t out_capacity, uint32_t *h_packet_bytes, uint64_t *out_total_bytes,
                                   uint32_t *h_clipped)
{
    return alac_hip_encode_float_dither_host(ctx, fmt, h_in, channel_stride, frame_stride, h_num_samples, num_packets,
                                             h_seg_first, num_segments, h_state, state_in, h_out, out_capacity, h_packet_bytes,
                                             out_total_bytes, h_clipped, nullptr, nullptr);
}

int32_t alac_hip_encode_float_dither_host(alac_hip_ctx *ctx, const alac_hip_format *fmt, const float *h_in,
                                          uint64_t channel_stride, uint64_t frame_stride, const uint32_t *h_num_samples,
                                          uint32_t num_packets, const uint32_t *h_seg_first, uint32_t num_segments,
                                          int16_t *h_state, int32_t state_in, uint8_t *h_out, uint64_t out_capacity,
                                          uint32_t *h_packet_bytes, uint64_t *out_total_bytes, uint32_t *h_clipped,
                                          const alac_hip_dither *dither, const uint64_t *h_packet_origin)
{
    if (!ctx) return ALAC_HIP_ParamError;
    if (!format_ok(fmt)) return fail(ctx, ALAC_HIP_ParamError, "unsupported format");
    if (const char *why = dither_refusal(fmt, dither, h_packet_origin)) return fail(ctx, ALAC_HIP_ParamError, why);
    if (out_total_bytes) *out_total_bytes = 0;
    if (num_packets == 0) return ALAC_HIP_noErr;
    if (!h_in || !h_out || !h_packet_bytes || !h_num_samples || !h_seg_first || num_segments == 0)
        return fail(ctx, ALAC_HIP_ParamError, "null buffer");
    if (int32_t rc = host_segment_refusal(ctx, h_seg_first, num_segments, num_packets)) return rc;
    const uint32_t np = num_packets, nseg = num_segments;
    uint64_t span = 0;
    if (int32_t rc = float_host_span(ctx, fmt, h_num_samples, np, channel_stride, frame_stride, span)) return rc;
    if (int32_t rc = float_stride_refusal(ctx, fmt, np, channel_stride, frame_stride)) return rc;
    if (int32_t rc = encode_refusal(ctx, fmt, np, ctx->opt.lpc ? np : nseg, nullptr, 0, 0)) return rc;
    const uint64_t wsBytes = alac_hip_encode_float_workspace_bytes(fmt, np, ctx->opt.lpc ? np : nseg);
    const uint64_t encBytes = (wsBytes - float_stage_bytes(fmt, np)) & ~255ull;
    const bool origin = dither_on(dither) && h_packet_origin;
    DevBuf dIn, dClip, dOrigin;
    hipError_t e;
    if ((e = dIn.alloc(span * sizeof(float))) || (e = dClip.alloc(np * 4ull)) || (origin && (e = dOrigin.alloc(np * 8ull))))
        return fail(ctx, ALAC_HIP_MemFullError, "hipMalloc", e);
    if ((e = hipMemcpyAsync(dIn.p, h_in, span * sizeof(float), hipMemcpyHostToDevice, ctx->stream)) ||
        (origin && (e = hipMemcpyAsync(dOrigin.p, h_packet_origin, np * 8ull, hipMemcpyHostToDevice, ctx->stream))))
        return fail(ctx, ALAC_HIP_ParamError, "H2D copy", e);
    int32_t rc = encode_host_common(
        ctx->stream, fmt, h_num_samples, np, h_seg_first, nseg, h_state, state_in, h_out, out_capacity, h_packet_bytes,
        out_total_bytes, wsBytes,
        [&](uint32_t maxSeg, const uint32_t *ns, const uint32_t *seg, int16_t *state, int32_t stIn, void *ws, uint8_t *out,
            uint64_t, uint32_t *sizes, uint64_t *offs) {
            const EncodeCall c = describe_encode(ctx, fmt, (uint8_t *)ws + encBytes, ns, np, seg, nseg, maxSeg, state, stIn, ws,
                                                 out, sizes, offs);
            return encode_float_run(ctx, c, (const float *)dIn.p, channel_stride, frame_stride,
                                    h_clipped ? (uint32_t *)dClip.p : nullptr, dither, (const uint64_t *)dOrigin.p);
        },
        on_fail(ctx), [ctx] { return alac_hip_synchronize(ctx); });
    if (rc != ALAC_HIP_noErr || !h_clipped) return rc;
    if ((e = hipMemcpyAsync(h_clipped, dClip.p, np * 4ull, hipMemcpyDeviceToHost, ctx->stream)) ||
        (e = hipStreamSynchronize(ctx->stream)))
        return fail(ctx, ALAC_HIP_ParamError, "D2H copy", e);
    return ALAC_HIP_noErr;
}

int32_t alac_hip_float_probe_host(alac_hip_ctx *ctx, const float *h_in, uint32_t num_channels, uint64_t channel_stride,
                                  uint64_t frame_stride, uint64_t total_frames, const uint64_t *h_seg_first_frame,
                                  uint32_t num_segments, alac_hip_float_report *h_reports)
{
    if (!ctx) return ALAC_HIP_ParamError;
    uint64_t lo, hi;
    if (int32_t rc = float_probe_refusal(ctx, h_in, num_channels, channel_stride, frame_stride, total_frames, h_seg_first_frame,
                                         num_segments, lo, hi))
        return rc;
    if (!h_reports) return fail(ctx, ALAC_HIP_ParamError, "null h_reports");
    if (hipSetDevice(ctx->device) != hipSuccess) return fail(ctx, ALAC_HIP_ParamError, "hipSetDevice");
    const uint64_t span = hi > lo ? (num_channels - 1) * channel_stride + (hi - 1) * frame_stride + 1 : 0;
    const uint64_t wsBytes = alac_hip_float_probe_workspace_bytes(num_segments), repBytes = (uint64_t)num_segments * 32;
    DevBuf dIn, dWs, dRep;
    hipError_t e;
    if ((e = dIn.alloc(span * sizeof(float))) || (e = dWs.alloc(wsBytes)) || (e = dRep.alloc(repBytes)))
        return fail(ctx, ALAC_HIP_MemFullError, "hipMalloc", e);
    if (span && (e = hipMemcpyAsync(dIn.p, h_in, span * sizeof(float), hipMemcpyHostToDevice, ctx->stream)))
        return fail(ctx, ALAC_HIP_ParamError, "H2D copy", e);
    if (int32_t rc = alac_hip_float_probe(ctx, (const float *)dIn.p, num_channels, channel_stride, frame_stride, total_frames,
                                          h_seg_first_frame, num_segments, dWs.p, wsBytes, (alac_hip_float_report *)dRep.p))
        return rc;
    if ((e = hipMemcpyAsync(h_reports, dRep.p, repBytes, hipMemcpyDeviceToHost, ctx->stream)) ||
        (e = hipStreamSynchronize(ctx->stream)))
        return fail(ctx, ALAC_HIP_ParamError, "D2H copy", e);
    return ALAC_HIP_noErr;
}

int32_t alac_hip_pcm_crc32_host(alac_hip_ctx *ctx, const void *h_pcm, uint64_t total_bytes, const uint64_t *h_ranges,
                                uint32_t num_ranges, alac_hip_pcm_digest *h_digests)
{
    if (!ctx) return ALAC_HIP_ParamError;
    uint64_t lo, hi;
    if (int32_t rc = pcm_crc_refusal(ctx, h_pcm, total_bytes, h_ranges, num_ranges, lo, hi)) return rc;
    if (!h_digests) return fail(ctx, ALAC_HIP_ParamError, "null h_digests");
    if (hipSetDevice(ctx->device) != hipSuccess) return fail(ctx, ALAC_HIP_ParamError, "hipSetDevice");
    const uint64_t wsBytes = h_ranges ? alac_hip_pcm_crc32_workspace_bytes(num_ranges) : 0, digBytes = (uint64_t)num_ranges * 16;
    DevBuf dPcm, dWs, dDig;
    hipError_t e;
    if ((e = dPcm.alloc(hi)) || (e = dWs.alloc(wsBytes)) || (e = dDig.alloc(digBytes)))
        return fail(ctx, ALAC_HIP_MemFullError, "hipMalloc", e);
    if (hi && (e = hipMemcpyAsync(dPcm.p, h_pcm, hi, hipMemcpyHostToDevice, ctx->stream)))
        return fail(ctx, ALAC_HIP_ParamError, "H2D copy", e);
    if (int32_t rc = alac_hip_pcm_crc32(ctx, dPcm.p, hi, h_ranges, num_ranges, dWs.p, wsBytes, (alac_hip_pcm_digest *)dDig.p))
        return rc;
    if ((e = hipMemcpyAsync(h_digests, dDig.p, digBytes, hipMemcpyDeviceToHost, ctx->stream)) ||
        (e = hipStreamSynchronize(ctx->stream)))
        return fail(ctx, ALAC_HIP_ParamError, "D2H copy", e);
    return ALAC_HIP_noErr;
}

int32_t alac_hip_encode_host(alac_hip_ctx *ctx, const alac_hip_format *fmt, const void *h_pcm,
                             uint64_t total_samples, uint32_t segment_packets, int16_t *h_state, int32_t state_in,
                             uint8_t *h_out, uint64_t out_capacity, uint32_t *h_packet_bytes,
                             uint64_t *out_total_bytes)
{
    if (!ctx) return ALAC_HIP_ParamError;
    if (!format_ok(fmt)) return fail(ctx, ALAC_HIP_ParamError, "unsupported format");
    if (out_total_bytes) *out_total_bytes = 0;
    if (total_samples == 0) return ALAC_HIP_noErr;
    if (!h_pcm || !h_out || !h_packet_bytes) return fail(ctx, ALAC_HIP_ParamError, "null buffer");
    const uint32_t bpf = fmt->num_channels * bytes_per_sample(fmt->bit_depth);
    const uint64_t np64 = (total_samples + fmt->frame_size - 1) / fmt->frame_size;
    if (np64 > 0x7fffffffull) return fail(ctx, ALAC_HIP_ParamError, "too many packets");
    const uint32_t np = (uint32_t)np64;
    const uint32_t nseg = segment_packets ? (np + segment_packets - 1) / segment_packets : 1;
    std::vector<uint32_t> ns(np, fmt->frame_size), segFirst(nseg + 1);
    ns[np - 1] = (uint32_t)(total_samples - (uint64_t)(np - 1) * fmt->frame_size);
    for (uint32_t s = 0; s <= nseg; s++) {
        uint64_t f = segment_packets ? (uint64_t)s * segment_packets : (s ? np : 0);
        segFirst[s] = (uint32_t)(f < np ? f : np);
    }
    const uint64_t inBytes = total_samples * bpf, pcmBytes = (uint64_t)np * fmt->frame_size * bpf;
    const void *src = h_pcm;
    std::vector<uint8_t> padded;
    if (inBytes != pcmBytes) {
        padded.assign(pcmBytes, 0);
        memcpy(padded.data(), h_pcm, inBytes);
        src = padded.data();
    }
    return encode_host_segments(ctx, fmt, src, ns.data(), np, segFirst.data(), nseg, h_state, state_in, h_out, out_capacity,
                                h_packet_bytes, out_total_bytes);
}

int32_t alac_hip_decode_host(alac_hip_ctx *ctx, const uint8_t *h_cookie, uint32_t cookie_size,
                             const uint8_t *h_stream, const uint32_t *h_packet_bytes, uint32_t num_packets,
                             uint8_t *h_pcm_out, uint32_t *h_num_samples_out, int32_t *h_status)
{
    alac_hip_format fmt;
    DecodeArgs da;
    if (int32_t rc = parse_cookie(ctx, h_cookie, cookie_size, fmt, da)) return rc;
    if (num_packets == 0) return ALAC_HIP_noErr;
    if (!h_stream || !h_packet_bytes || !h_pcm_out || !h_num_samples_out || !h_status)
        return fail(ctx, ALAC_HIP_ParamError, "null buffer");
    const uint64_t pcmBytes = (uint64_t)num_packets * fmt.frame_size * fmt.num_channels * bytes_per_sample(fmt.bit_depth);
    return decode_host_common(ctx, fmt, da, h_stream, h_packet_bytes, num_packets, pcmBytes, nullptr, nullptr, h_pcm_out, 1, 0,
                              h_num_samples_out, nullptr, nullptr, h_status);
}

int32_t alac_hip_decode_float_host(alac_hip_ctx *ctx, const uint8_t *h_cookie, uint32_t cookie_size,
                                   const uint8_t *h_stream, const uint32_t *h_packet_bytes, uint32_t num_packets, float *h_out,
                                   uint64_t channel_stride, uint32_t *h_num_samples_out, int32_t *h_status)
{
    alac_hip_format fmt;
    DecodeArgs da;
    if (int32_t rc = parse_cookie(ctx, h_cookie, cookie_size, fmt, da)) return rc;
    if (num_packets == 0) return ALAC_HIP_noErr;
    if (!h_stream || !h_packet_bytes || !h_out || !h_num_samples_out || !h_status)
        return fail(ctx, ALAC_HIP_ParamError, "null buffer");
    if (channel_stride < (uint64_t)num_packets * fmt.frame_size)
        return fail(ctx, ALAC_HIP_ParamError, "channel_stride below num_packets * frame_size");
    if (channel_stride > UINT64_MAX / sizeof(float) / fmt.num_channels)
        return fail(ctx, ALAC_HIP_ParamError, "channel_stride * channels overflows");
    const uint64_t row = (uint64_t)num_packets * fmt.frame_size;
    da.pcmMode = kPcmFloat;
    da.channelStride = row;
    return decode_host_common(ctx, fmt, da, h_stream, h_packet_bytes, num_packets, row * fmt.num_channels * sizeof(float), nullptr,
                              nullptr, h_out, fmt.num_channels, channel_stride * sizeof(float), h_num_samples_out, nullptr,
                              nullptr, h_status);
}

int32_t alac_hip_verify_host(alac_hip_ctx *ctx, const uint8_t *h_cookie, uint32_t cookie_size, const uint8_t *h_stream,
                             const uint32_t *h_packet_bytes, uint32_t num_packets, const uint8_t *h_pcm_expected,
                             const uint32_t *h_num_samples_expected, uint32_t *h_first_mismatch, int32_t *h_status)
{
    alac_hip_format fmt;
    DecodeArgs da;
    if (int32_t rc = parse_cookie(ctx, h_cookie, cookie_size, fmt, da)) return rc;
    if (num_packets == 0) return 0;
    if (!h_stream || !h_packet_bytes || !h_pcm_expected) return fail(ctx, ALAC_HIP_ParamError, "null buffer");
    if (num_packets > 0x7fffffffu) return fail(ctx, ALAC_HIP_ParamError, "more packets than the return value counts");
    const uint64_t pcmBytes = (uint64_t)num_packets * fmt.frame_size * fmt.num_channels * bytes_per_sample(fmt.bit_depth);
    uint32_t bad = 0;
    const int32_t rc = decode_host_common(ctx, fmt, da, h_stream, h_packet_bytes, num_packets, pcmBytes, h_pcm_expected,
                                          h_num_samples_expected, nullptr, 1, 0, nullptr, h_first_mismatch, &bad, h_status);
    return rc != ALAC_HIP_noErr ? rc : (int32_t)bad;
}

int32_t alac_hip_verify_float_host(alac_hip_ctx *ctx, const uint8_t *h_cookie, uint32_t cookie_size, const uint8_t *h_stream,
                                   const uint32_t *h_packet_bytes, uint32_t num_packets, const float *h_in,
                                   uint64_t channel_stride, uint64_t frame_stride, const uint32_t *h_num_samples_expected,
                                   const alac_hip_dither *dither, const uint64_t *h_packet_origin, uint32_t *h_first_mismatch,
                                   int32_t *h_status)
{
    alac_hip_format fmt;
    DecodeArgs da;
    if (int32_t rc = parse_cookie(ctx, h_cookie, cookie_size, fmt, da)) return rc;
    if (int32_t rc = verify_float_refusal(ctx, fmt, num_packets, h_in, channel_stride, frame_stride, dither, h_packet_origin))
        return rc;
    if (num_packets == 0) return 0;
    if (!h_stream || !h_packet_bytes) return fail(ctx, ALAC_HIP_ParamError, "null buffer");
    if (num_packets > 0x7fffffffu) return fail(ctx, ALAC_HIP_ParamError, "more packets than the return value counts");
    uint64_t span = 0;
    if (int32_t rc = float_host_span(ctx, &fmt, h_num_samples_expected, num_packets, channel_stride, frame_stride, span)) return rc;
    static const float kNone = 0.0f;
    const VerifyFloatArgs vf = verify_float_args(channel_stride, frame_stride, dither, nullptr);
    uint32_t bad = 0;
    const int32_t rc = decode_host_common(ctx, fmt, da, h_stream, h_packet_bytes, num_packets, (span ? span : 1) * sizeof(float),
                                          span ? h_in : &kNone, h_num_samples_expected, nullptr, 1, 0, nullptr, h_first_mismatch,
                                          &bad, h_status, &vf, dither_on(dither) ? h_packet_origin : nullptr);
    return rc != ALAC_HIP_noErr ? rc : (int32_t)bad;
}

}
```

alac_amd/csrc/alac_dev.hpp:

```cpp
#pragma once

#include <hip/hip_runtime.h>
#include <stdint.h>

namespace alacdev {

constexpr uint32_t kQBShift = 9;
constexpr uint32_t kPB0 = 40;
constexpr uint32_t kMB0 = 10;
constexpr uint32_t kKB0 = 14;
constexpr uint32_t kDenShift = 9;
constexpr uint32_t kMaxPrefix = 9;
constexpr uint32_t kMaxRunBits = 16;
constexpr uint32_t kMeanClamp = 0xffffu;
constexpr int32_t kMixBits = 2;
constexpr int32_t kMaxRes = 4;

__host__ __device__ constexpr uint32_t bytes_per_sample(uint32_t depth)
{
    return depth == 16 ? 2u : (depth == 32 ? 4u : 3u);
}
__host__ __device__ constexpr uint32_t bytes_shifted(uint32_t depth)
{
    return depth == 32 ? 2u : (depth >= 24 ? 1u : 0u);
}

__device__ __forceinline__ int32_t sext(int32_t x, uint32_t chanshift)
{
    return (int32_t)((uint32_t)x << chanshift) >> chanshift;
}
__device__ __forceinline__ int32_t sign_of(int32_t x) { return min(max(x, -1), 1); }
__device__ __forceinline__ int32_t wsub(int32_t a, int32_t b) { return (int32_t)((uint32_t)a - (uint32_t)b); }
__device__ __forceinline__ int32_t wadd(int32_t a, int32_t b) { return (int32_t)((uint32_t)a + (uint32_t)b); }
__device__ __forceinline__ int32_t wmul(int32_t a, int32_t b) { return (int32_t)((uint32_t)a * (uint32_t)b); }
__device__ __forceinline__ int32_t wabs(int32_t a) { return a < 0 ? wsub(0, a) : a; }
__device__ __forceinline__ uint32_t times5(uint32_t x)
{
    uint32_t r;
    asm("v_lshl_add_u32 %0, %1, 2, %1" : "=v"(r) : "v"(x));
    return r;
}

__device__ __forceinline__ int32_t lead(uint32_t m) { return m ? __clz((int)m) : 32; }
__device__ __forceinline__ int32_t lg3a(uint32_t x) { return 31 - lead(x + 3); }

template <int DEPTH>
__device__ __forceinline__ int32_t load_sample(const uint8_t *pk, uint32_t t)
{
    if constexpr (DEPTH == 16) {
        return ((const int16_t *)pk)[t];
    } else if constexpr (DEPTH == 32) {
        return ((const int32_t *)pk)[t];
    } else {
        const uint8_t *p = pk + 3u * t;
        uint32_t w = ((uint32_t)p[2] << 24) | ((uint32_t)p[1] << 16) | ((uint32_t)p[0] << 8);
        return (int32_t)w >> (DEPTH == 20 ? 12 : 8);
    }
}

template <int DEPTH>
__device__ __forceinline__ void load_lr(const uint8_t *pk, uint32_t j, int32_t &l, int32_t &r)
{
    constexpr int SH = 8 * (int)bytes_shifted(DEPTH);
    if constexpr (DEPTH == 16) {
        int32_t w = ((const int32_t *)pk)[j];
        l = (int16_t)w;
        r = w >> 16;
    } else {
        l = load_sample<DEPTH>(pk, 2 * j) >> SH;
        r = load_sample<DEPTH>(pk, 2 * j + 1) >> SH;
    }
}

__device__ __forceinline__ int32_t mix_sample(int32_t mixres, int ch, int32_t l, int32_t r)
{
    if (mixres != 0) {
        int32_t m2 = (1 << kMixBits) - mixres;
        return ch == 0 ? ((mixres * l + m2 * r) >> kMixBits) : (l - r);
    }
    return ch == 0 ? l : r;
}

template <int NA>
struct Lms {
    int32_t a[NA];
    int32_t h[NA + 1];
};

template <int NA>
__device__ __forceinline__ void lms_push(Lms<NA> &s, int32_t x)
{
#pragma unroll
    for (int k = NA; k > 0; k--) s.h[k] = s.h[k - 1];
    s.h[0] = x;
}

template <int NA>
__device__ __forceinline__ void lms_adapt(Lms<NA> &s, const int32_t (&b)[NA], int32_t del, uint32_t denshift)
{
    const int32_t sg = sign_of(del);
    int32_t del0 = del;
    bool go = sg != 0;
#pragma unroll
    for (int k = NA - 1; k >= 0; k--) {
        const int32_t sgn = sign_of(b[k]);
        const int32_t step = wmul(sg, sgn);
        s.a[k] = (int16_t)(s.a[k] - (go ? step : 0));
        del0 = wsub(del0, wmul(NA - k, wmul(step, b[k]) >> denshift));
        go = go && (sg > 0 ? del0 > 0 : del0 < 0);
    }
}

template <int NA>
__device__ __forceinline__ int32_t lms_step_enc(Lms<NA> &s, int32_t x, uint32_t chanshift)
{
    const int32_t top = s.h[NA];
    int32_t b[NA];
    int32_t sum = 0;
#pragma unroll
    for (int k = 0; k < NA; k++) {
        b[k] = wsub(top, s.h[k]);
        sum = wadd(sum, wmul(s.a[k], b[k]));
    }
    int32_t del = sext(wsub(wsub(x, top), wsub(1 << (kDenShift - 1), sum) >> kDenShift), chanshift);
    lms_adapt<NA>(s, b, del, kDenShift);
    lms_push<NA>(s, x);
    return del;
}

template <int NA>
__device__ __forceinline__ int32_t lms_step_dec(Lms<NA> &s, int32_t del, uint32_t chanshift,
                                                uint32_t denshift)
{
    const int32_t top = s.h[NA];
    int32_t b[NA];
    int32_t sum = 0;
#pragma unroll
    for (int k = 0; k < NA; k++) {
        b[k] = wsub(top, s.h[k]);
        sum = wadd(sum, wmul(s.a[k], b[k]));
    }
    const int32_t denhalf = denshift ? (1 << (denshift - 1)) : 0;
    const int32_t out = sext(wadd(wadd(del, top), wsub(denhalf, sum) >> denshift), chanshift);
    lms_adapt<NA>(s, b, del, denshift);
    lms_push<NA>(s, out);
    return out;
}

struct Golomb {
    uint32_t mb, zmode, inrun, nz, bits;
    uint32_t pb, kb, wb;
    uint64_t acc;
    uint32_t nacc, widx, wcap;
    uint32_t *wp;
};

__device__ __forceinline__ void gol_reset(Golomb &g, uint32_t mb0, uint32_t pb, uint32_t kb)
{
    g.mb = mb0;
    g.zmode = 0;
    g.inrun = 0;
    g.nz = 0;
    g.bits = 0;
    g.pb = pb;
    g.kb = kb;
    g.wb = (1u << kb) - 1;
    g.acc = 0;
    g.nacc = 0;
    g.widx = 0;
}

template <bool WRITE>
__device__ __forceinline__ void gol_put(Golomb &g, uint32_t value, uint32_t nbits)
{
    g.bits += nbits;
    if constexpr (WRITE) {
        const uint64_t v = nbits >= 32 ? (uint64_t)value : (uint64_t)(value & ((1u << nbits) - 1));
        g.acc = (g.acc << nbits) | v;
        g.nacc += nbits;
        if (g.nacc >= 32) {
            g.nacc -= 32;
            if (g.widx < g.wcap) g.wp[g.widx] = (uint32_t)(g.acc >> g.nacc);
            g.widx++;
        }
    }
}

template <bool WRITE>
__device__ __forceinline__ void gol_flush(Golomb &g)
{
    if constexpr (WRITE) {
        if (g.nacc > 0) {
            if (g.widx < g.wcap) g.wp[g.widx] = (uint32_t)(g.acc << (32 - g.nacc));
            g.widx++;
            g.nacc = 0;
        }
    }
}

template <bool WRITE>
__device__ __forceinline__ void gol_close_run(Golomb &g)
{
    const uint32_t k = (uint32_t)(lead(g.mb) - 24 + (int32_t)((g.mb + 16u) >> 6));
    const uint32_t mz = ((1u << k) - 1) & g.wb;
    const uint32_t nz = g.nz;
    const uint32_t div = nz / mz;
    uint32_t numBits, value;
    if (div >= kMaxPrefix) {
        numBits = kMaxPrefix + kMaxRunBits;
        value = (((1u << kMaxPrefix) - 1) << kMaxRunBits) + nz;
    } else {
        const uint32_t mod = nz - div * mz;
        const uint32_t de = (mod == 0);
        numBits = div + k + 1 - de;
        value = (((1u << div) - 1) << (numBits - div)) + mod + 1 - de;
        if (numBits > kMaxPrefix + kMaxRunBits) {
            numBits = kMaxPrefix + kMaxRunBits;
            value = (((1u << kMaxPrefix) - 1) << kMaxRunBits) + nz;
        }
    }
    gol_put<WRITE>(g, value, numBits);
    g.mb = 0;
    g.inrun = 0;
}

template <bool WRITE>
__device__ __forceinline__ void gol_sym(Golomb &g, int32_t del, bool last, uint32_t bitSize)
{
    if (g.inrun) {
        if (del == 0) {
            g.nz++;
            if (g.nz >= 65535) {
                gol_close_run<WRITE>(g);
                g.zmode = 0;
            } else if (last) {
                gol_close_run<WRITE>(g);
            }
            return;
        }
        gol_close_run<WRITE>(g);
    }
    uint32_t m = g.mb >> kQBShift;
    uint32_t k = (uint32_t)lg3a(m);
    k = k > g.kb ? g.kb : k;
    m = (1u << k) - 1;
    const uint32_t a = (uint32_t)(del < 0 ? -del : del);
    const uint32_t n = (a << 1) - ((uint32_t)del >> 31) - g.zmode;
    const uint32_t div = n / m;
    bool esc = true;
    if (div < kMaxPrefix) {
        const uint32_t mod = n - m * div;
        const uint32_t de = (mod == 0);
        const uint32_t numBits = div + k + 1 - de;
        if (numBits <= 25) {
            gol_put<WRITE>(g, (((1u << div) - 1) << (numBits - div)) + mod + 1 - de, numBits);
            esc = false;
        }
    }
    if (esc) {
        gol_put<WRITE>(g, (1u << kMaxPrefix) - 1, kMaxPrefix);
        gol_put<WRITE>(g, n, bitSize);
    }
    g.mb = g.pb * (n + g.zmode) + g.mb - ((g.pb * g.mb) >> kQBShift);
    if (n > kMeanClamp) g.mb = kMeanClamp;
    g.zmode = 0;
    if (((g.mb << 2) < (1u << kQBShift)) && !last) {
        g.zmode = 1;
        g.inrun = 1;
        g.nz = 0;
    }
}

__device__ __forceinline__ uint32_t peek32(const uint8_t *base, uint64_t limitBytes, uint64_t pos)
{
    const uint64_t byte = pos >> 3;
    uint64_t v = 0;
#pragma unroll
    for (int i = 0; i < 5; i++) {
        const uint64_t bi = byte + i;
        v = (v << 8) | (bi < limitBytes ? (uint64_t)base[bi] : 0ull);
    }
    return (uint32_t)(v >> (8 - (pos & 7)));
}

__device__ __forceinline__ uint32_t read_bits(const uint8_t *base, uint64_t limitBytes,
                                              uint64_t &pos, uint32_t n)
{
    const uint32_t v = n ? (peek32(base, limitBytes, pos) >> (32 - n)) : 0u;
    pos += n;
    return v;
}

}
```

alac_amd/csrc/alac_encode.hip:

```cpp
#include <cstdlib>
#include <type_traits>
#include "alac_dev.hpp"
#include "alac_kernels.hpp"

namespace alacdev {


template <int DEPTH, int CH, int NA, class Sink>
__device__ __forceinline__ void lms_pass(const uint8_t *pk, int mixres, int ch, uint32_t P,
                                         uint32_t num, int32_t *coefs, uint32_t chanshift,
                                         Sink &&sink)
{
    Lms<NA> s;
#pragma unroll
    for (int k = 0; k < NA; k++) s.a[k] = coefs[k];
#pragma unroll
    for (int k = 0; k <= NA; k++) s.h[k] = 0;

    auto fetch = [&](uint32_t j) -> int32_t {
        if constexpr (CH == 2) {
            int32_t l, r;
            load_lr<DEPTH>(pk, j, l, r);
            return mix_sample(mixres, ch, l, r);
        } else {
            return load_sample<DEPTH>(pk, j) >> (8 * (int)bytes_shifted(DEPTH));
        }
    };

    int32_t xn = P ? fetch(0) : 0;
    for (uint32_t j = 0; j < P; j++) {
        const int32_t x = xn;
        if (j + 1 < P) xn = fetch(j + 1);
        int32_t del;
        if (j == 0) {
            del = x;
            lms_push<NA>(s, x);
        } else if (j <= (uint32_t)NA) {
            del = sext(x - s.h[0], chanshift);
            lms_push<NA>(s, x);
        } else {
            del = lms_step_enc<NA>(s, x, chanshift);
        }
        sink(j, del);
    }
#pragma unroll
    for (int k = 0; k < NA; k++) coefs[k] = s.a[k];
    (void)num;
}


template <int DEPTH, int NA>
__device__ __forceinline__ uint32_t numuv_cost(const uint8_t *pk, int best, int ch, uint32_t N,
                                               int32_t *row, uint32_t chanBits,
                                               const int32_t *pred, uint64_t predStride)
{
    const uint32_t chanshift = 32 - chanBits;
    const uint32_t n8 = N / 8, n32 = N / 32;
    uint32_t P2 = n32 > (uint32_t)(NA + 1) ? n32 : (uint32_t)(NA + 1);
    P2 = P2 < n8 ? P2 : n8;
    Golomb g;
    gol_reset(g, kMB0, kPB0, kKB0);
    for (int conv = 0; conv < 8; conv++) {
        if (conv < 7) {
            if (n32 > (uint32_t)(NA + 1))
                lms_pass<DEPTH, 2, NA>(pk, best, ch, n32, n32, row, chanshift, [](uint32_t, int32_t) {});
        } else {
            lms_pass<DEPTH, 2, NA>(pk, best, ch, P2, n32, row, chanshift, [&](uint32_t j, int32_t del) {
                gol_sym<false>(g, del, j + 1 == n8, chanBits);
            });
        }
    }
    for (uint32_t j = P2; j < n8; j++) gol_sym<false>(g, pred[(uint64_t)j * predStride], j + 1 == n8, chanBits);
    return g.bits * 8 + 16 * NA;
}

template <int DEPTH, int NA>
__device__ __forceinline__ uint32_t final_pass(const uint8_t *pk, int best, int ch, uint32_t N,
                                               int32_t *row, uint32_t chanBits, uint32_t pb,
                                               uint32_t *words, uint32_t wcap)
{
    Golomb g;
    gol_reset(g, kMB0, pb, kKB0);
    g.wp = words;
    g.wcap = wcap;
    lms_pass<DEPTH, 2, NA>(pk, best, ch, N, N, row, 32 - chanBits, [&](uint32_t j, int32_t del) {
        gol_sym<true>(g, del, j + 1 == N, chanBits);
    });
    gol_flush<true>(g);
    return g.bits;
}

template <int DEPTH>
__global__ __launch_bounds__(64) void k_encode_stereo(EncodeArgs A)
{
    const uint32_t gl = blockIdx.x * 64u + threadIdx.x;
    const uint32_t seg = gl >> 1;
    const int ch = (int)(gl & 1);
    if (seg >= A.numSegments) return;

    constexpr uint32_t SHB = bytes_shifted(DEPTH);
    constexpr uint32_t chanBits = DEPTH - 8 * SHB + 1;
    constexpr uint32_t chanshift = 32 - chanBits;
    const uint32_t frameBytes = A.frameSize * 2u * bytes_per_sample(DEPTH);

    int32_t a3[4], a7[8];
    if (A.state && A.stateIn) {
        const int16_t *s = A.state + (uint64_t)seg * 64 + ch * 32;
#pragma unroll
        for (int k = 0; k < 4; k++) a3[k] = s[k];
#pragma unroll
        for (int k = 0; k < 8; k++) a7[k] = s[16 + k];
    } else {
        a3[0] = a7[0] = (38 * 512) >> 4;
        a3[1] = a7[1] = (-29 * 512) >> 4;
        a3[2] = a7[2] = (-2 * 512) >> 4;
        a3[3] = a7[3] = 0;
#pragma unroll
        for (int k = 4; k < 8; k++) a7[k] = 0;
    }

    uint32_t p0 = A.segFirst ? A.segFirst[seg] : seg;
    const uint32_t p1 = A.segFirst ? A.segFirst[seg + 1] : seg + 1;
    if (p1 < p0 || p1 > A.numPackets || p1 - p0 > A.segMax) p0 = p1;
    int32_t *pred = A.pred + gl;
    const uint64_t predStride = A.predStride;

    for (uint32_t p = p0; p < p1; p++) {
        uint32_t N = A.numSamples ? A.numSamples[p] : A.frameSize;
        N = N < A.frameSize ? N : A.frameSize;
        const uint8_t *pk = A.pcm + (uint64_t)p * frameBytes;
        const uint32_t partial = (N != A.frameSize);
        const uint32_t n8 = N / 8;

        int best = 0;
        uint32_t minb = 1u << 31;
        for (int r = 0; r <= kMaxRes; r++) {
            Golomb g;
            gol_reset(g, kMB0, kPB0, kKB0);
            const bool keep = (r == kMaxRes);
            lms_pass<DEPTH, 2, 8>(pk, r, ch, n8, n8, a7, chanshift, [&](uint32_t j, int32_t del) {
                gol_sym<false>(g, del, j + 1 == n8, chanBits);
                if (keep) pred[(uint64_t)j * predStride] = del;
            });
            const uint32_t tot = g.bits + __shfl_xor(g.bits, 1);
            if (tot < minb) {
                minb = tot;
                best = r;
            }
        }

        uint32_t numMine = 4;
        uint32_t minMine = numuv_cost<DEPTH, 4>(pk, best, ch, N, a3, chanBits, pred, predStride);
        {
            const uint32_t c8 = numuv_cost<DEPTH, 8>(pk, best, ch, N, a7, chanBits, pred, predStride);
            if (c8 < minMine) {
                minMine = c8;
                numMine = 8;
            }
        }

        uint32_t minBits = minMine + __shfl_xor(minMine, 1) + 64 + (partial ? 32 : 0);
        minBits += N * (SHB * 8) * 2;
        const uint32_t escapeBits = N * DEPTH * 2 + (partial ? 32 : 0) + 16;
        bool doEscape = (minBits >= escapeBits);

        PacketRec *rec = A.recs + p;
        rec->c[ch].num = (uint16_t)numMine;
#pragma unroll
        for (int k = 0; k < 8; k++) rec->c[ch].coefs[k] = (int16_t)(numMine == 4 ? (k < 4 ? a3[k] : 0) : a7[k]);

        uint32_t bits = 0;
        if (!doEscape) {
            uint32_t *words = A.bitWords + ((uint64_t)p * 2 + ch) * A.wcap;
            bits = numMine == 4
                       ? final_pass<DEPTH, 4>(pk, best, ch, N, a3, chanBits, kPB0, words, A.wcap)
                       : final_pass<DEPTH, 8>(pk, best, ch, N, a7, chanBits, kPB0, words, A.wcap);
        }
        rec->c[ch].bits = bits;
        const uint32_t obits = __shfl_xor(bits, 1);
        const uint32_t onum = __shfl_xor(numMine, 1);
        uint32_t body = 0;
        if (!doEscape) {
            body = 12 + 4 + (partial ? 32 : 0) + 16 + (16 + 16 * numMine) + (16 + 16 * onum) +
                   N * (SHB * 8) * 2 + bits + obits;
            if (body >= escapeBits) doEscape = true;
        }
        if (doEscape) body = 12 + 4 + (partial ? 32 : 0) + N * DEPTH * 2;
        if (ch == 0) {
            rec->numSamples = N;
            rec->escape = doEscape ? 1u : 0u;
            rec->mixRes = (uint32_t)best;
            rec->totalBits = 7 + body + 3;
            A.packetBytes[p] = (7 + body + 3 + 7) / 8;
        }
    }

    if (A.state) {
        int16_t *s = A.state + (uint64_t)seg * 64 + ch * 32;
#pragma unroll
        for (int k = 0; k < 16; k++) {
            s[k] = (int16_t)(k < 4 ? a3[k] : 0);
            s[16 + k] = (int16_t)(k < 8 ? a7[k] : 0);
        }
    }
}


template <int DEPTH, int NA>
__device__ __forceinline__ uint32_t mono_cost(const uint8_t *pk, uint32_t N, int32_t *row,
                                              uint32_t chanBits)
{
    const uint32_t chanshift = 32 - chanBits;
    const uint32_t n8 = N / 8, n32 = N / 32;
    for (int conv = 0; conv < 7; conv++)
        if (n32 > (uint32_t)(NA + 1))
            lms_pass<DEPTH, 1, NA>(pk, 0, 0, n32, n32, row, chanshift, [](uint32_t, int32_t) {});
    Golomb g;
    gol_reset(g, kMB0, kPB0, kKB0);
    lms_pass<DEPTH, 1, NA>(pk, 0, 0, n8, n8, row, chanshift, [&](uint32_t j, int32_t del) {
        gol_sym<false>(g, del, j + 1 == n8, chanBits);
    });
    return g.bits * 8 + 16 * NA;
}

template <int DEPTH, int NA>
__device__ __forceinline__ uint32_t mono_final(const uint8_t *pk, uint32_t N, int32_t *row,
                                               uint32_t chanBits, uint32_t *words, uint32_t wcap)
{
    Golomb g;
    gol_reset(g, kMB0, kPB0, kKB0);
    g.wp = words;
    g.wcap = wcap;
    lms_pass<DEPTH, 1, NA>(pk, 0, 0, N, N, row, 32 - chanBits, [&](uint32_t j, int32_t del) {
        gol_sym<true>(g, del, j + 1 == N, chanBits);
    });
    gol_flush<true>(g);
    return g.bits;
}

template <int DEPTH>
__global__ __launch_bounds__(64) void k_encode_mono(EncodeArgs A)
{
    const uint32_t seg = blockIdx.x * 64u + threadIdx.x;
    if (seg >= A.numSegments) return;

    constexpr uint32_t SHB = bytes_shifted(DEPTH);
    constexpr uint32_t chanBits = DEPTH - 8 * SHB;
    const uint32_t frameBytes = A.frameSize * bytes_per_sample(DEPTH);

    int32_t a3[4], a7[8];
    if (A.state && A.stateIn) {
        const int16_t *s = A.state + (uint64_t)seg * 64;
#pragma unroll
        for (int k = 0; k < 4; k++) a3[k] = s[k];
#pragma unroll
        for (int k = 0; k < 8; k++) a7[k] = s[16 + k];
    } else {
        a3[0] = a7[0] = (38 * 512) >> 4;
        a3[1] = a7[1] = (-29 * 512) >> 4;
        a3[2] = a7[2] = (-2 * 512) >> 4;
        a3[3] = a7[3] = 0;
#pragma unroll
        for (int k = 4; k < 8; k++) a7[k] = 0;
    }

    uint32_t p0 = A.segFirst ? A.segFirst[seg] : seg;
    const uint32_t p1 = A.segFirst ? A.segFirst[seg + 1] : seg + 1;
    if (p1 < p0 || p1 > A.numPackets || p1 - p0 > A.segMax) p0 = p1;

    for (uint32_t p = p0; p < p1; p++) {
        uint32_t N = A.numSamples ? A.numSamples[p] : A.frameSize;
        N = N < A.frameSize ? N : A.frameSize;
        const uint8_t *pk = A.pcm + (uint64_t)p * frameBytes;
        const uint32_t partial = (N != A.frameSize);

        uint32_t bestU = 4;
        uint32_t minBits = mono_cost<DEPTH, 4>(pk, N, a3, chanBits);
        {
            const uint32_t c8 = mono_cost<DEPTH, 8>(pk, N, a7, chanBits);
            if (c8 < minBits) {
                minBits = c8;
                bestU = 8;
            }
        }
        minBits += 32 + (partial ? 32 : 0) + N * (SHB * 8);
        const uint32_t escapeBits = N * DEPTH + (partial ? 32 : 0) + 16;
        bool doEscape = (minBits >= escapeBits);

        PacketRec *rec = A.recs + p;
        rec->c[0].num = (uint16_t)bestU;
#pragma unroll
        for (int k = 0; k < 8; k++) rec->c[0].coefs[k] = (int16_t)(bestU == 4 ? (k < 4 ? a3[k] : 0) : a7[k]);
        rec->c[1].num = 0;
        rec->c[1].bits = 0;

        uint32_t bits = 0, body;
        if (!doEscape) {
            uint32_t *words = A.bitWords + (uint64_t)p * 2 * A.wcap;
            bits = bestU == 4 ? mono_final<DEPTH, 4>(pk, N, a3, chanBits, words, A.wcap)
                              : mono_final<DEPTH, 8>(pk, N, a7, chanBits, words, A.wcap);
            body = 12 + 4 + (partial ? 32 : 0) + 16 + (16 + 16 * bestU) + N * (SHB * 8) + bits;
            if (body >= escapeBits) doEscape = true;
        }
        if (doEscape) body = 12 + 4 + (partial ? 32 : 0) + N * DEPTH;
        rec->c[0].bits = bits;
        rec->numSamples = N;
        rec->escape = doEscape ? 1u : 0u;
        rec->mixRes = 0;
        rec->totalBits = 7 + body + 3;
        A.packetBytes[p] = (7 + body + 3 + 7) / 8;
    }

    if (A.state) {
        int16_t *s = A.state + (uint64_t)seg * 64;
#pragma unroll
        for (int k = 0; k < 16; k++) {
            s[k] = (int16_t)(k < 4 ? a3[k] : 0);
            s[16 + k] = (int16_t)(k < 8 ? a7[k] : 0);
            if (!A.stateIn) {
                const int16_t init = (int16_t)(k == 0 ? 1216 : k == 1 ? -928 : k == 2 ? -64 : 0);
                s[32 + k] = init;
                s[48 + k] = init;
            }
        }
    }
}


__global__ __launch_bounds__(1024) void k_scan_sizes(const uint32_t *sizes, uint64_t *offsets, uint32_t n, const uint32_t *segBad)
{
    const bool refused = segBad && *segBad != 0;
    __shared__ uint64_t waveSum[16];
    __shared__ uint64_t wavePre[16];
    const uint32_t tid = threadIdx.x, lane = tid & 63, wave = tid >> 6;
    const uint32_t base = blockIdx.x * 1024u;
    uint64_t before = 0;
    {
        typedef uint32_t U4 __attribute__((ext_vector_type(4), aligned(4)));
        const U4 *s4 = (const U4 *)sizes;
#pragma unroll 4
        for (uint32_t i = tid; i < base / 4; i += 1024) {
            const U4 q = s4[i];
            before += refused ? 0ull : (uint64_t)q.x + q.y + q.z + q.w;
        }
    }
#pragma unroll
    for (int d = 32; d >= 1; d >>= 1) before += __shfl_xor(before, d);
    const uint32_t i = base + tid;
    const uint64_t v = (i < n && !refused) ? sizes[i] : 0;
    uint64_t incl = v;
#pragma unroll
    for (int d = 1; d < 64; d <<= 1) {
        const uint64_t t = __shfl_up(incl, d);
        if ((int)lane >= d) incl += t;
    }
    if (lane == 63) waveSum[wave] = incl;
    if (lane == 0) wavePre[wave] = before;
    __syncthreads();
    uint64_t pre = 0;
    for (uint32_t w = 0; w < 16; w++) pre += wavePre[w] + (w < wave ? waveSum[w] : 0);
    if (i < n) offsets[i] = pre + incl - v;
    if (i == n - 1) offsets[n] = pre + incl;
    if (n == 0 && i == 0) offsets[0] = 0;
}


__device__ __forceinline__ uint32_t words_fetch32(const uint32_t *w, uint32_t len, uint32_t s0)
{
    const uint32_t i = s0 >> 5, sh = s0 & 31;
    const uint32_t nw = (len + 31) >> 5;
    const uint32_t a = w[i];
    const uint32_t b = (i + 1 < nw) ? w[i + 1] : 0u;
    uint32_t v = sh ? ((a << sh) | (b >> (32 - sh))) : a;
    const uint32_t rem = len - s0;
    if (rem < 32) v &= ~0u << (32 - rem);
    return v;
}

template <int W, class Field>
__device__ __forceinline__ uint32_t fields_fetch32(Field &&field, uint32_t count, uint64_t s0)
{
    uint32_t out = 0;
#pragma unroll
    for (int half = 0; half < 2; half++) {
        const uint64_t s = s0 + 16u * half;
        uint32_t t = (uint32_t)(s / W);
        const uint32_t o = (uint32_t)(s % W);
        uint64_t acc = 0;
        uint32_t have = 0;
        while (have < o + 16) {
            const uint64_t f = t < count ? (uint64_t)field(t) : 0ull;
            acc = (W == 32) ? ((acc << 32) | f) : ((acc << W) | (f & ((1ull << W) - 1)));
            have += W;
            t++;
        }
        out = (out << 16) | (uint32_t)((acc >> (have - o - 16)) & 0xffffu);
    }
    return out;
}

template <class Fetch>
__device__ __forceinline__ uint32_t take(Fetch &&fetch32, uint64_t len, int64_t s)
{
    if (s >= (int64_t)len || s <= -32) return 0;
    if (s >= 0) return fetch32((uint64_t)s);
    return fetch32(0) >> (uint32_t)(-s);
}

template <int DEPTH, int CH>
__global__ __launch_bounds__(256) void k_pack(PackArgs A, uint32_t numPackets)
{
    constexpr uint32_t kHdrWords = (23 + 32 + 16 + 2 * (16 + 16 * kLpcMaxOrder) + 31) / 32;
    __shared__ uint32_t hdr[kHdrWords];
    const uint32_t lane = threadIdx.x & 63;
    const bool seamWave = (threadIdx.x >> 6) == (blockDim.x >> 6) - 1;
    constexpr uint32_t SHB = bytes_shifted(DEPTH);
    const uint32_t refused = A.segBad ? *A.segBad : 0u;
    PacketRec recNext = A.recs[blockIdx.x];
    uint64_t offNext = A.offsets[blockIdx.x];
    if (refused) return;
    for (uint32_t p = blockIdx.x; p < numPackets; p += gridDim.x) {
    const PacketRec rec = recNext;
    const uint64_t outOff = offNext;
    if (p + gridDim.x < numPackets) {
        recNext = A.recs[p + gridDim.x];
        offNext = A.offsets[p + gridDim.x];
    }
    const uint32_t N = rec.numSamples;
    const uint32_t partial = (N != A.frameSize);
    const uint8_t *pk = A.pcm + (uint64_t)p * A.frameSize * CH * bytes_per_sample(DEPTH);
    uint32_t hb = 3 + 4 + 12 + 4 + (partial ? 32u : 0u);
    if (!rec.escape) {
        hb += 16;
        for (int c = 0; c < CH; c++) hb += 16 + 16 * rec.c[c].num;
    }
    const uint64_t lenHdr = hb;
    const uint64_t lenShift = rec.escape ? 0 : (uint64_t)N * CH * SHB * 8;
    const uint64_t lenU = rec.escape ? 0 : rec.c[0].bits;
    const uint64_t lenV = (rec.escape || CH == 1) ? 0 : rec.c[1].bits;
    const uint64_t lenRaw = rec.escape ? (uint64_t)N * CH * DEPTH : 0;
    const int64_t offShift = (int64_t)lenHdr;
    const int64_t offU = offShift + (int64_t)lenShift;
    const int64_t offV = offU + (int64_t)lenU;
    const int64_t offRaw = offV + (int64_t)lenV;
    const int64_t offEnd = offRaw + (int64_t)lenRaw;
    const uint32_t nb = (uint32_t)((offEnd + 3 + 7) / 8);

    const uint32_t *wU = A.bitWords + (uint64_t)p * 2 * A.wcap;
    const uint32_t *wV = wU + A.wcap;
    const uint32_t mis = (uint32_t)(outOff & 15);
    uint8_t *outAligned = A.out + (outOff - mis);
    const uint32_t nwords = (mis + nb + 3) / 4;

    auto sampleField = [&](uint32_t t) -> uint32_t { return (uint32_t)load_sample<DEPTH>(pk, t); };

    struct Span {
        uint32_t w0, w1;
    };
    auto span_of = [&](int64_t off, uint64_t len) {
        const int64_t base = off + (int64_t)mis * 8;
        Span sp;
        sp.w0 = ((uint32_t)((base + 31) >> 5) + 3) & ~3u;
        sp.w1 = (uint32_t)((base + (int64_t)len) >> 5) & ~3u;
        if (sp.w1 < sp.w0) sp.w1 = sp.w0;
        return sp;
    };
    auto first_bit = [&](const Span &sp, int64_t off) { return (uint32_t)((int64_t)sp.w0 * 32 - (off + (int64_t)mis * 8)); };
    auto load5 = [&](uint32_t a[5], bool have, uint32_t i, uint32_t sh, auto &&src) {
        if constexpr (std::is_pointer_v<std::decay_t<decltype(src)>>) {
            typedef uint32_t U4 __attribute__((ext_vector_type(4), aligned(4)));
            const char *at = (const char *)src + i * 4u;
            U4 v = {0, 0, 0, 0};
            uint32_t e = 0;
            if (have) {
                v = *(const U4 *)at;
                if (sh) e = *(const uint32_t *)(at + 16);
            }
            a[0] = v.x, a[1] = v.y, a[2] = v.z, a[3] = v.w, a[4] = e;
        } else {
#pragma unroll
            for (int q = 0; q < 5; q++) a[q] = (have && (q < 4 || sh)) ? src(i + q) : 0u;
        }
    };
    auto store4 = [&](const uint32_t a[5], uint32_t sh, uint32_t w) {
        uint4 v;
        v.x = __builtin_bswap32(sh ? __builtin_amdgcn_alignbit(a[0], a[1], 32 - sh) : a[0]);
        v.y = __builtin_bswap32(sh ? __builtin_amdgcn_alignbit(a[1], a[2], 32 - sh) : a[1]);
        v.z = __builtin_bswap32(sh ? __builtin_amdgcn_alignbit(a[2], a[3], 32 - sh) : a[2]);
        v.w = __builtin_bswap32(sh ? __builtin_amdgcn_alignbit(a[3], a[4], 32 - sh) : a[3]);
        *(uint4 *)(outAligned + (uint64_t)w * 4) = v;
    };
    auto copy_span = [&](const Span &sp, int64_t off, auto &&srcWord) {
        const uint32_t fb = first_bit(sp, off), i0 = fb >> 5, sh = fb & 31;
        for (uint32_t w = sp.w0 + 4 * threadIdx.x; w < sp.w1; w += 4 * blockDim.x) {
            uint32_t a[5];
            load5(a, true, i0 + (w - sp.w0), sh, srcWord);
            store4(a, sh, w);
        }
    };
    typedef uint32_t U4 __attribute__((ext_vector_type(4), aligned(4)));
    auto shift_word24 = [](uint32_t d0, uint32_t d1, uint32_t d2) {
        return (d0 << 24) | ((d0 >> 24) << 16) | (((d1 >> 16) & 0xffu) << 8) | ((d2 >> 8) & 0xffu);
    };
    auto shift_word_slow = [&](uint32_t i) -> uint32_t {
        const uint32_t fields = N * CH;
        if constexpr (DEPTH == 24) {
            uint32_t v = 0;
            for (uint32_t q = 0; q < 4; q++)
                v = (v << 8) | (4 * i + q < fields ? ((uint32_t)load_sample<24>(pk, 4 * i + q) & 0xffu) : 0u);
            return v;
        } else {
            const uint32_t *pw = (const uint32_t *)pk;
            const uint32_t t = 2 * i;
            const uint32_t a = t < fields ? pw[t] : 0u, b = t + 1 < fields ? pw[t + 1] : 0u;
            return (a << 16) | (b & 0xffffu);
        }
    };
    auto load5_shift = [&](uint32_t a[5], bool have, uint32_t i, uint32_t sh) {
        const uint32_t *pw = (const uint32_t *)pk;
        const uint32_t fields = N * CH;
#pragma unroll
        for (int q = 0; q < 5; q++) a[q] = 0;
        if (!have) return;
        if constexpr (DEPTH == 24) {
            const char *at = (const char *)pw + i * 12u;
            const U4 x = *(const U4 *)at, y = *(const U4 *)(at + 16), z = *(const U4 *)(at + 32);
            a[0] = shift_word24(x.x, x.y, x.z);
            a[1] = shift_word24(x.w, y.x, y.y);
            a[2] = shift_word24(y.z, y.w, z.x);
            a[3] = shift_word24(z.y, z.z, z.w);
            if (sh) {
                if (4 * (i + 4) + 4 <= fields) {
                    const uint32_t d0 = *(const uint32_t *)(at + 48), d1 = *(const uint32_t *)(at + 52), d2 = *(const uint32_t *)(at + 56);
                    a[4] = shift_word24(d0, d1, d2);
                } else {
                    a[4] = shift_word_slow(i + 4);
                }
            }
        } else {
            const char *at = (const char *)pw + i * 8u;
            const U4 x = *(const U4 *)at, y = *(const U4 *)(at + 16);
            a[0] = (x.x << 16) | (x.y & 0xffffu);
            a[1] = (x.z << 16) | (x.w & 0xffffu);
            a[2] = (y.x << 16) | (y.y & 0xffffu);
            a[3] = (y.z << 16) | (y.w & 0xffffu);
            if (sh) {
                if (2 * (i + 4) + 2 <= fields) {
                    const uint32_t d0 = *(const uint32_t *)(at + 32), d1 = *(const uint32_t *)(at + 36);
                    a[4] = (d0 << 16) | (d1 & 0xffffu);
                } else {
                    a[4] = shift_word_slow(i + 4);
                }
            }
        }
    };
    auto copy_bulk = [&](const Span &ss, const Span &sa, const Span &sb) {
        constexpr bool SHIFT = SHB != 0 && (DEPTH == 24 || DEPTH == 32);
        const uint32_t fs = first_bit(ss, offShift), is0 = fs >> 5, shS = fs & 31;
        const uint32_t fa = first_bit(sa, offU), ia0 = fa >> 5, shA = fa & 31;
        const uint32_t fb = first_bit(sb, offV), ib0 = fb >> 5, shB = fb & 31;
        const uint32_t ns = SHIFT ? (ss.w1 - ss.w0) / 4 : 0u, na = (sa.w1 - sa.w0) / 4, nb2 = CH == 2 ? (sb.w1 - sb.w0) / 4 : 0u;
        for (uint32_t g = threadIdx.x; g < max(ns, max(na, nb2)); g += blockDim.x) {
            const bool hs = g < ns, ha = g < na, hb = g < nb2;
            uint32_t x[5], a[5], b[5];
            if constexpr (SHIFT) load5_shift(x, hs, is0 + 4 * g, shS);
            load5(a, ha, ia0 + 4 * g, shA, wU);
            if constexpr (CH == 2) load5(b, hb, ib0 + 4 * g, shB, wV);
            if constexpr (SHIFT)
                if (hs) store4(x, shS, ss.w0 + 4 * g);
            if (ha) store4(a, shA, sa.w0 + 4 * g);
            if constexpr (CH == 2)
                if (hb) store4(b, shB, sb.w0 + 4 * g);
        }
    };
    Span spU = {0, 0}, spV = {0, 0}, spR = {0, 0}, spS = {0, 0};
    if (!rec.escape) {
        if constexpr (SHB != 0 && (DEPTH == 24 || DEPTH == 32)) spS = span_of(offShift, lenShift);
        spU = span_of(offU, lenU);
        if constexpr (CH == 2) spV = span_of(offV, lenV);
    } else {
        spR = span_of(offRaw, lenRaw);
    }
    const Span s1 = rec.escape ? spR : spS, s2 = spU, s3 = spV;
    const uint32_t nSeam = nwords - (s1.w1 - s1.w0) - (s2.w1 - s2.w0) - (s3.w1 - s3.w0);
    auto seam_word = [&](uint32_t k) {
        uint32_t aw = k;
        if (aw >= s1.w0) aw += s1.w1 - s1.w0;
        if (aw >= s2.w0) aw += s2.w1 - s2.w0;
        if (aw >= s3.w0) aw += s3.w1 - s3.w0;
        return aw;
    };
    struct Pair {
        uint32_t a, b;
    };
    auto fetch_pair = [&](const uint32_t *w, uint64_t len, int64_t s) {
        const uint32_t nw = (uint32_t)((len + 31) >> 5);
        const uint32_t i = s > 0 ? (uint32_t)(s >> 5) : 0u;
        const uint32_t last = nw ? nw - 1 : 0u;
        Pair pr;
        pr.a = w[min(i, last)];
        pr.b = w[min(i + 1, last)];
        return pr;
    };
    auto combine_pair = [&](const Pair &pr, uint64_t len, int64_t s) -> uint32_t {
        if (s >= (int64_t)len || s <= -32) return 0u;
        const uint32_t s0 = s > 0 ? (uint32_t)s : 0u;
        const uint32_t i = s0 >> 5, sh = s0 & 31;
        const uint32_t nw = (uint32_t)((len + 31) >> 5);
        const uint32_t b = (i + 1 < nw) ? pr.b : 0u;
        uint32_t v = sh ? ((pr.a << sh) | (b >> (32 - sh))) : pr.a;
        const uint32_t rem = (uint32_t)len - s0;
        if (rem < 32) v &= ~0u << (32 - rem);
        return s < 0 ? v >> (uint32_t)(-s) : v;
    };
    auto seam_store = [&](uint32_t aw, uint32_t v) {
        const int64_t b0 = (int64_t)aw * 4 - mis;
        if (b0 >= 0 && b0 + 4 <= (int64_t)nb) {
            *(uint32_t *)(outAligned + (uint64_t)aw * 4) = __builtin_bswap32(v);
        } else {
#pragma unroll
            for (int b = 0; b < 4; b++) {
                const int64_t pb = b0 + b;
                if (pb >= 0 && pb < (int64_t)nb) outAligned[(uint64_t)aw * 4 + b] = (uint8_t)(v >> (24 - 8 * b));
            }
        }
    };
    auto shift_fetch32 = [&](uint32_t s0) -> uint32_t {
        if constexpr (SHB == 0) {
            return 0u;
        } else if constexpr (DEPTH != 24 && DEPTH != 32) {
            return fields_fetch32<SHB * 8>(sampleField, N * CH, s0);
        } else {
            const uint32_t *pw = (const uint32_t *)pk;
            const uint32_t fields = N * CH, perWord = DEPTH == 24 ? 4u : 2u, dwPerWord = DEPTH == 24 ? 3u : 2u;
            const uint32_t i = s0 >> 5, sh = s0 & 31;
            const uint32_t nFull = fields / perWord;
            const bool fullA = i < nFull, fullB = i + 1 < nFull;
            const uint32_t ia = fullA ? i : 0u, ib = fullB ? i + 1 : 0u;
            uint32_t da[3], db[3];
#pragma unroll
            for (uint32_t q = 0; q < dwPerWord; q++) da[q] = nFull ? pw[ia * dwPerWord + q] : 0u;
#pragma unroll
            for (uint32_t q = 0; q < dwPerWord; q++) db[q] = nFull ? pw[ib * dwPerWord + q] : 0u;
            uint32_t a, b;
            if constexpr (DEPTH == 24) {
                a = shift_word24(da[0], da[1], da[2]);
                b = shift_word24(db[0], db[1], db[2]);
            } else {
                a = (da[0] << 16) | (da[1] & 0xffffu);
                b = (db[0] << 16) | (db[1] & 0xffffu);
            }
            if (!fullA) a = shift_word_slow(i);
            if (!fullB) b = shift_word_slow(i + 1);
            uint32_t v = sh ? ((a << sh) | (b >> (32 - sh))) : a;
            const uint32_t rem = (uint32_t)lenShift - s0;
            if (rem < 32) v &= ~0u << (32 - rem);
            return v;
        }
    };
    auto seam_rest = [&](int64_t bp) {
        uint32_t v = take([&](uint64_t s0) { return words_fetch32(hdr, (uint32_t)lenHdr, (uint32_t)s0); }, lenHdr, bp);
        if (!rec.escape) {
            if constexpr (SHB != 0)
                v |= take([&](uint64_t s0) { return shift_fetch32((uint32_t)s0); }, lenShift, bp - offShift);
        } else {
            v |= take([&](uint64_t s0) { return fields_fetch32<DEPTH>(sampleField, N * CH, s0); }, lenRaw, bp - offRaw);
        }
        v |= take([](uint64_t s0) { return 0xE0000000u << (uint32_t)s0; }, 3, bp - offEnd);
        return v;
    };
    Pair seamU = {0, 0}, seamV = {0, 0};
    const uint32_t seamAw = seam_word(lane);
    const int64_t seamBp = (int64_t)seamAw * 32 - (int64_t)mis * 8;
    if (seamWave) {
        if (lane < kHdrWords) hdr[lane] = 0;
        const uint32_t perChan = A.lpc ? 1u + kLpcMaxOrder : 9u;
        const LpcChan *lpcRec = A.lpc ? A.lpc + (uint64_t)p * 2 : nullptr;
        const uint32_t base = 23 + (partial ? 32u : 0u);
        for (uint32_t f = lane; f < 3 + perChan * CH; f += 64) {
            uint32_t fpos = 0, fn = 0, fv = 0;
            if (f == 0) {
                fn = 23;
                fv = ((CH == 2 ? 1u : 0u) << 20) | (rec.escape ? ((partial << 3) | 1u) : ((partial << 3) | (SHB << 1)));
            } else if (f == 1) {
                fpos = 23, fn = partial ? 32u : 0u, fv = N;
            } else if (!rec.escape) {
                if (f == 2) {
                    fpos = base, fn = 16, fv = CH == 2 ? (((uint32_t)kMixBits << 8) | (rec.mixRes & 0xffu)) : 0u;
                } else {
                    const uint32_t c = (f - 3) / perChan, k = (f - 3) - perChan * c;
                    const uint32_t num = c ? rec.c[CH - 1].num : rec.c[0].num;
                    const uint32_t cstart = base + 16 + (c ? 16 + 16 * (uint32_t)rec.c[0].num : 0u);
                    const bool own = lpcRec && lpcRec[c].num != 0;
                    if (k == 0) {
                        const uint32_t den = own ? lpcRec[c].den : kDenShift;
                        fpos = cstart, fn = 16, fv = (((0u << 4) | den) << 8) | ((4u << 5) | num);
                    } else if (k - 1 < num) {
                        uint32_t coef = 0;
                        if (own) {
                            coef = (uint16_t)lpcRec[c].coefs[k - 1];
                        } else {
#pragma unroll
                            for (int q = 0; q < 8; q++) {
                                const uint32_t cq = (uint16_t)(c ? rec.c[CH - 1].coefs[q] : rec.c[0].coefs[q]);
                                coef = (k - 1 == (uint32_t)q) ? cq : coef;
                            }
                        }
                        fpos = cstart + 16 * k, fn = 16, fv = coef;
                    }
                }
            }
            if (fn) {
                const uint32_t i = fpos >> 5, o = fpos & 31;
                const uint64_t x = ((uint64_t)fv << (64 - fn)) >> o;
                atomicOr(&hdr[i], (uint32_t)(x >> 32));
                if (o + fn > 32) atomicOr(&hdr[i + 1], (uint32_t)x);
            }
        }
        if (!rec.escape && lane < nSeam) {
            seamU = fetch_pair(wU, lenU, seamBp - offU);
            if constexpr (CH == 2) seamV = fetch_pair(wV, lenV, seamBp - offV);
        }
    }
    if (!rec.escape) {
        copy_bulk(spS, spU, spV);
    } else if constexpr (DEPTH == 16) {
        const uint32_t *pw = (const uint32_t *)pk;
        copy_span(spR, offRaw, [&](uint32_t i) {
            const uint32_t x = pw[i];
            return (x << 16) | (x >> 16);
        });
    } else if constexpr (DEPTH == 32) {
        const uint32_t *pw = (const uint32_t *)pk;
        copy_span(spR, offRaw, [&](uint32_t i) { return pw[i]; });
    } else if constexpr (DEPTH == 24) {
        const uint32_t *pw = (const uint32_t *)pk;
        const uint32_t ndw = (N * CH * 3 + 3) / 4;
        const uint32_t fb = first_bit(spR, offRaw), i0 = fb >> 5, sh = fb & 31;
        for (uint32_t w = spR.w0 + 4 * threadIdx.x; w < spR.w1; w += 4 * blockDim.x) {
            const uint32_t i = i0 + (w - spR.w0);
            const uint32_t g = i / 3, r = i - 3 * g, base = 3 * g;
            uint32_t d[9];
            if (base + 9 <= ndw) {
                const U4 x = *(const U4 *)(pw + base), y = *(const U4 *)(pw + base + 4);
                d[0] = x.x, d[1] = x.y, d[2] = x.z, d[3] = x.w, d[4] = y.x, d[5] = y.y, d[6] = y.z, d[7] = y.w;
                d[8] = pw[base + 8];
            } else {
#pragma unroll
                for (uint32_t q = 0; q < 9; q++) d[q] = pw[min(base + q, ndw - 1)];
            }
            uint32_t W[9];
#pragma unroll
            for (int t = 0; t < 3; t++) {
                const uint32_t d0 = d[3 * t], d1 = d[3 * t + 1], d2 = d[3 * t + 2];
                W[3 * t] = (d0 << 8) | ((d1 >> 8) & 0xffu);
                W[3 * t + 1] = (d1 << 24) | ((d0 >> 24) << 16) | ((d2 & 0xffu) << 8) | (d1 >> 24);
                W[3 * t + 2] = (((d1 >> 16) & 0xffu) << 24) | ((d2 >> 24) << 16) | (((d2 >> 16) & 0xffu) << 8) | ((d2 >> 8) & 0xffu);
            }
            uint32_t a[5];
#pragma unroll
            for (int q = 0; q < 5; q++) a[q] = r == 0 ? W[q] : (r == 1 ? W[q + 1] : W[q + 2]);
            store4(a, sh, w);
        }
    } else {
        const uint32_t *pw = (const uint32_t *)pk;
        const uint32_t ndw = (N * CH * 3 + 3) / 4;
        const uint32_t fb = first_bit(spR, offRaw), i0 = fb >> 5, sh = fb & 31;
        for (uint32_t w = spR.w0 + 4 * threadIdx.x; w < spR.w1; w += 4 * blockDim.x) {
            const uint32_t i = i0 + (w - spR.w0);
            const uint32_t g = i / 5, r = i - 5 * g, base = 6 * g;
            uint32_t d[12];
            if (base + 12 <= ndw) {
                const U4 x = *(const U4 *)(pw + base), y = *(const U4 *)(pw + base + 4), z = *(const U4 *)(pw + base + 8);
                d[0] = x.x, d[1] = x.y, d[2] = x.z, d[3] = x.w, d[4] = y.x, d[5] = y.y, d[6] = y.z, d[7] = y.w;
                d[8] = z.x, d[9] = z.y, d[10] = z.z, d[11] = z.w;
            } else {
#pragma unroll
                for (uint32_t q = 0; q < 12; q++) d[q] = pw[min(base + q, ndw - 1)];
            }
            uint32_t W[10];
#pragma unroll
            for (int t = 0; t < 2; t++) {
                uint32_t sm[8];
#pragma unroll
                for (int h = 0; h < 2; h++) {
                    const uint32_t d0 = d[6 * t + 3 * h], d1 = d[6 * t + 3 * h + 1], d2 = d[6 * t + 3 * h + 2];
                    sm[4 * h] = (d0 & 0xffffffu) >> 4;
                    sm[4 * h + 1] = (((d0 >> 24) | (d1 << 8)) & 0xffffffu) >> 4;
                    sm[4 * h + 2] = (((d1 >> 16) | (d2 << 16)) & 0xffffffu) >> 4;
                    sm[4 * h + 3] = d2 >> 12;
                }
                W[5 * t] = (sm[0] << 12) | (sm[1] >> 8);
                W[5 * t + 1] = (sm[1] << 24) | (sm[2] << 4) | (sm[3] >> 16);
                W[5 * t + 2] = (sm[3] << 16) | (sm[4] >> 4);
                W[5 * t + 3] = (sm[4] << 28) | (sm[5] << 8) | (sm[6] >> 12);
                W[5 * t + 4] = (sm[6] << 20) | sm[7];
            }
            uint32_t a[5];
#pragma unroll
            for (int q = 0; q < 5; q++)
                a[q] = r == 0 ? W[q] : (r == 1 ? W[q + 1] : (r == 2 ? W[q + 2] : (r == 3 ? W[q + 3] : W[q + 4])));
            store4(a, sh, w);
        }
    }

    if (seamWave) {
        if (lane < nSeam) {
            uint32_t v = seam_rest(seamBp);
            if (!rec.escape) {
                v |= combine_pair(seamU, lenU, seamBp - offU);
                if constexpr (CH == 2) v |= combine_pair(seamV, lenV, seamBp - offV);
            }
            seam_store(seamAw, v);
        }
        for (uint32_t k = lane + 64; k < nSeam; k += 64) {
            const uint32_t aw = seam_word(k);
            const int64_t bp = (int64_t)aw * 32 - (int64_t)mis * 8;
            uint32_t v = seam_rest(bp);
            if (!rec.escape) {
                v |= combine_pair(fetch_pair(wU, lenU, bp - offU), lenU, bp - offU);
                if constexpr (CH == 2) v |= combine_pair(fetch_pair(wV, lenV, bp - offV), lenV, bp - offV);
            }
            seam_store(aw, v);
        }
    }
    }
}


template <int DEPTH>
static hipError_t launch_scan_pack_depth(uint32_t channels, uint32_t *packetBytes, const PackArgs &pa, uint32_t numPackets,
                                         hipStream_t st, hipEvent_t *ev, bool recordScan = true)
{
    if (ev && recordScan) ALAC_TRY(hipEventRecord(ev[kStageScan], st));
    ALAC_TRY(launch_kernel(k_scan_sizes, dim3(numPackets / 1024 + 1), dim3(1024), st, (const uint32_t *)packetBytes,
                           (uint64_t *)pa.offsets, numPackets, pa.segBad));
    if (ev) ALAC_TRY(hipEventRecord(ev[kStagePack], st));
    static const uint32_t tpb = getenv("ALAC_HIP_PACK_TPB") ? (uint32_t)atoi(getenv("ALAC_HIP_PACK_TPB")) : 128u;
    static const uint32_t wgs = getenv("ALAC_HIP_PACK_WGS") ? (uint32_t)atoi(getenv("ALAC_HIP_PACK_WGS")) : (1u << 20);
    const uint32_t grid = numPackets < wgs ? numPackets : wgs;
    if (channels == 2)
        ALAC_TRY(launch_kernel(k_pack<DEPTH, 2>, dim3(grid), dim3(tpb), st, pa, numPackets));
    else
        ALAC_TRY(launch_kernel(k_pack<DEPTH, 1>, dim3(grid), dim3(tpb), st, pa, numPackets));
    return ev ? hipEventRecord(ev[kNumStages], st) : hipSuccess;
}

hipError_t launch_scan_sizes(const uint32_t *sizes, uint64_t *offsets, uint32_t n, hipStream_t st, const uint32_t *segBad)
{
    return launch_kernel(k_scan_sizes, dim3(n / 1024 + 1), dim3(1024), st, sizes, offsets, n, segBad);
}

hipError_t launch_scan_pack(uint32_t depth, uint32_t channels, uint32_t *packetBytes, const PackArgs &pa, uint32_t numPackets,
                            hipStream_t st, hipEvent_t *ev, bool recordScan)
{
    switch (depth) {
    case 16: return launch_scan_pack_depth<16>(channels, packetBytes, pa, numPackets, st, ev, recordScan);
    case 20: return launch_scan_pack_depth<20>(channels, packetBytes, pa, numPackets, st, ev, recordScan);
    case 24: return launch_scan_pack_depth<24>(channels, packetBytes, pa, numPackets, st, ev, recordScan);
    default: return launch_scan_pack_depth<32>(channels, packetBytes, pa, numPackets, st, ev, recordScan);
    }
}

template <int DEPTH>
static hipError_t launch_encode_depth(const EncodeArgs &ea, const PackArgs &pa, uint32_t channels,
                                      uint32_t numPackets, hipStream_t st, hipEvent_t *ev)
{
    if (ev)
        for (int i = 0; i <= kStageLms3; i++) ALAC_TRY(hipEventRecord(ev[i], st));
    if (channels == 2) {
        const uint32_t lanes = ea.numSegments * 2;
        ALAC_TRY(launch_kernel(k_encode_stereo<DEPTH>, dim3((lanes + 63) / 64), dim3(64), st, ea));
    } else {
        ALAC_TRY(launch_kernel(k_encode_mono<DEPTH>, dim3((ea.numSegments + 63) / 64), dim3(64), st, ea));
    }
    if (ev) ALAC_TRY(hipEventRecord(ev[kStageGol3], st));
    return launch_scan_pack_depth<DEPTH>(channels, ea.packetBytes, pa, numPackets, st, ev);
}

hipError_t launch_encode(uint32_t depth, uint32_t channels, const EncodeArgs &ea, const PackArgs &pa,
                         uint32_t numPackets, hipStream_t st, hipEvent_t *ev)
{
    switch (depth) {
    case 16: return launch_encode_depth<16>(ea, pa, channels, numPackets, st, ev);
    case 20: return launch_encode_depth<20>(ea, pa, channels, numPackets, st, ev);
    case 24: return launch_encode_depth<24>(ea, pa, channels, numPackets, st, ev);
    case 32: return launch_encode_depth<32>(ea, pa, channels, numPackets, st, ev);
    default: return hipErrorInvalidValue;
    }
}

}
```

alac_amd/csrc/alac_kernels.hpp:

```cpp
#pragma once

#include <hip/hip_runtime.h>
#include <stdint.h>

namespace alacdev {

#define ALAC_TRY(call)                          \
    do {                                        \
        const hipError_t try_e_ = (call);       \
        if (try_e_ != hipSuccess) return try_e_; \
    } while (0)
template <typename K, typename... Args>
inline hipError_t launch_kernel_lds(K kernel, dim3 grid, dim3 block, size_t ldsBytes, hipStream_t st, const Args &...args)
{
    hipLaunchKernelGGL(kernel, grid, block, ldsBytes, st, args...);
    return hipGetLastError();
}
template <typename K, typename... Args>
inline hipError_t launch_kernel(K kernel, dim3 grid, dim3 block, hipStream_t st, const Args &...args)
{
    return launch_kernel_lds(kernel, grid, block, 0, st, args...);
}

struct ChanRec {
    uint32_t bits;
    uint16_t num;
    uint16_t pad;
    int16_t coefs[8];
};
struct PacketRec {
    uint32_t numSamples;
    uint32_t escape;
    uint32_t mixRes;
    uint32_t totalBits;
    ChanRec c[2];
};
static_assert(sizeof(PacketRec) == 64, "PacketRec layout");
constexpr int kLpcMaxOrder = 30;
struct LpcChan {
    uint16_t den;
    uint16_t num;
    int16_t coefs[kLpcMaxOrder];
};
static_assert(sizeof(LpcChan) == 64, "LpcChan layout");

struct EncodeArgs {
    const uint8_t *pcm;
    const uint32_t *numSamples;
    const uint32_t *segFirst;
    uint32_t numSegments;
    uint32_t frameSize;
    int16_t *state;
    int32_t stateIn;
    int32_t *pred;
    uint64_t predStride;
    uint32_t *bitWords;
    uint32_t wcap;
    PacketRec *recs;
    uint32_t *packetBytes;
    uint32_t numPackets;
    uint32_t segMax;
    uint32_t *segBad;
};

struct PackArgs {
    const uint8_t *pcm;
    const PacketRec *recs;
    const uint32_t *bitWords;
    uint32_t wcap;
    uint32_t frameSize;
    const uint64_t *offsets;
    uint8_t *out;
    const uint32_t *segBad;
    const LpcChan *lpc = nullptr;
};

struct LpcArgs {
    const uint8_t *pcm;
    uint32_t frameSize;
    PacketRec *recs;
    uint32_t *packetBytes;
    uint32_t *bitWords;
    uint32_t wcap;
    LpcChan *lpc;
};
hipError_t launch_lpc(uint32_t depth, uint32_t channels, const LpcArgs &a, uint32_t numPackets, hipStream_t st);

enum EncodeStage {
    kStageLms1 = 0,
    kStageGol1,
    kStageLms2,
    kStageGol2,
    kStageLms3,
    kStageGol3,
    kStageScan,
    kStagePack,
    kNumStages
};

hipError_t launch_encode(uint32_t depth, uint32_t channels, const EncodeArgs &ea, const PackArgs &pa,
                         uint32_t numPackets, hipStream_t st, hipEvent_t *ev);
hipError_t launch_scan_pack(uint32_t depth, uint32_t channels, uint32_t *packetBytes, const PackArgs &pa,
                            uint32_t numPackets, hipStream_t st, hipEvent_t *ev, bool recordScan = true);

struct HandoffCtl {
    uint32_t *err = nullptr;
    uint32_t spinLimit = 1u << 22;
    uint32_t lose = 0;
};

struct AlacOptions {
    int32_t thru = -1;
    int32_t narrow = -1;
    int32_t splitCoder = 1;
    int32_t overlapPos = 1;
    int32_t fused = 1;
    int32_t fold = 1;
    int32_t fastMode = 0;
    int32_t laneEncoder = 0;
    int32_t laneDecoder = 0;
    int32_t decFused = -1;
    int32_t decPair = 1;
    int32_t decDirect = 1;
    int32_t stageTaps = 1;
    int32_t loseHandoff = 0;
    int32_t lpc = 0;
    int32_t debugWaves = 0;
};
AlacOptions alac_options_from_env();
struct AlacOptionKey {
    const char *name;
    const char *env;
    int32_t AlacOptions::*slot;
    int32_t lo, hi;
};
const AlacOptionKey *alac_option_keys(uint32_t *count);
const AlacOptionKey *alac_option_find(const char *key);

constexpr uint32_t kSideEvents = 2;
struct V1Streams {
    hipStream_t side[1];
    hipEvent_t fork, stagger[kSideEvents], join[kSideEvents];
};
constexpr uint32_t kEventBlocks = 2;
hipError_t launch_check_segments(const uint32_t *segFirst, uint32_t numSegments, uint32_t numPackets, uint32_t maxSeg, uint32_t *err,
                                 uint32_t *segBad,
                                 hipStream_t st);
enum class V1Shape { Lane, Tiny, Latency, LatencyUnfolded, Stagewise, Throughput };
struct V1Plan {
    V1Shape shape;
    bool fast;
    bool fusedSearch;
    bool split;
    bool overlap;
    bool fused() const { return shape == V1Shape::Tiny || shape == V1Shape::Latency || shape == V1Shape::LatencyUnfolded; }
};
V1Plan v1_plan(uint32_t channels, uint32_t numSegments, uint32_t maxSegPackets, uint32_t frameSize, const AlacOptions &opt);
const char *v1_regime_name(V1Shape shape);
constexpr uint32_t kSplitCoderMaxChains = 4096;
inline uint32_t v1_split_at(uint32_t frameSize) { return (frameSize * 2 / 3) / 48 * 48; }

struct DecChan {
    uint16_t mode, denShift, pbFactor, num;
    int16_t coefs[32];
};
struct DecRec {
    uint32_t numSamples;
    uint32_t escape;
    int32_t mixBits, mixRes;
    uint32_t bytesShifted;
    uint32_t elementChannels;
    uint64_t shiftPos;
    int32_t status;
    uint32_t pad;
    uint32_t chanIndex;
    uint32_t pad2;
    DecChan c[2];
};

struct DecodeArgs {
    const uint8_t *stream;
    const uint64_t *offsets;
    uint32_t numPackets;
    uint32_t frameSize, bitDepth, numChannels;
    uint32_t mb, pb, kb;
    uint32_t maxElems;
    DecRec *recs;
    const uint32_t *gate = nullptr;
    HandoffCtl ho;
    int32_t optFused = -1, optPair = 1, optDirect = 1;
    int32_t *resid;
    uint8_t *pcmOut;
    uint32_t *numSamplesOut;
    int32_t *statusOut;
    union {
        const struct VerifyFloatArgs *verifyFloat;
        uint32_t *firstMismatch = nullptr;
        uint64_t channelStride;
    };
    uint32_t frameBytes = 0;
    uint32_t pcmMode = 0;
};

hipError_t launch_decode(const DecodeArgs &da, hipStream_t st);
hipError_t launch_verify_init(uint32_t *firstMismatch, uint32_t numPackets, uint32_t *bad, hipStream_t st);
hipError_t launch_verify_finish(const int32_t *status, const uint32_t *numSamplesDecoded, const uint32_t *numSamplesExpected,
                                uint32_t frameSize, uint32_t numPackets, uint32_t *firstMismatch, uint32_t *bad, hipStream_t st);
hipError_t launch_decode_v1(const DecodeArgs &da, uint32_t *words, uint64_t capWords, int32_t *plane, uint32_t *prog,
                            hipStream_t st, uint32_t *mismatch);

struct McElement {
    uint32_t first;
    uint32_t channels;
    uint32_t tag;
};
constexpr uint32_t kMaxChannels = 8;
uint32_t channel_elements(uint32_t numChannels, McElement *out);
struct McSpliceArgs {
    uint32_t numElements, numPackets;
    McElement el[kMaxChannels];
    const uint8_t *src[kMaxChannels];
    const uint64_t *srcOffsets[kMaxChannels];
    uint32_t *elemBits;
    uint32_t *packetBytes;
    uint64_t *offsets;
    uint8_t *out;
};
hipError_t launch_mc_gather(const uint8_t *pcm, uint8_t *out, const uint32_t *numSamples, uint32_t numPackets,
                            uint32_t frameSize, uint32_t numChannels, uint32_t first, uint32_t channels, uint32_t bytesPerSample,
                            hipStream_t st);
hipError_t launch_mc_tables(const uint32_t *numSamples, uint32_t numPackets, const uint32_t *segFirst, uint32_t numSegments,
                            uint32_t count, uint32_t *numSamplesOut, uint32_t *segFirstOut, hipStream_t st);
hipError_t launch_mc_splice(const McSpliceArgs &a, hipStream_t st);
hipError_t launch_scan_sizes(const uint32_t *sizes, uint64_t *offsets, uint32_t n, hipStream_t st, const uint32_t *segBad = nullptr);

hipError_t launch_decode_v1_elements(const DecodeArgs &da, const McElement *el, uint32_t numElements, uint32_t *words,
                                     uint64_t capWords, int32_t *plane, uint32_t *prog, uint32_t *elemBit,
                                     uint32_t *mismatch, hipStream_t st);

struct FloatInArgs {
    const float *in;
    uint64_t channelStride, frameStride;
    const uint32_t *numSamples;
    uint32_t numPackets, frameSize, channels;
    uint8_t *pcm;
    uint32_t *clipped;
};
struct FloatDitherArgs {
    const uint64_t *origin;
    uint32_t roundKey[10][2];
};
void philox_round_keys(uint64_t seed, uint32_t (&roundKey)[10][2]);
enum FloatLayout : int {
    kFloatPlanar = 0,
    kFloatInterleaved = 1,
    kFloatGeneral = 2,
};
inline FloatLayout float_layout(const float *in, uint32_t channels, uint64_t channelStride, uint64_t frameStride)
{
    const bool vec = ((uintptr_t)in & 15) == 0 && channels <= 2;
    if (vec && frameStride == 1 && (channels == 1 || channelStride % 4 == 0)) return kFloatPlanar;
    if (vec && channels == 2 && channelStride == 1 && frameStride == 2) return kFloatInterleaved;
    return kFloatGeneral;
}
hipError_t launch_float_to_pcm(uint32_t depth, const FloatInArgs &a, hipStream_t st, const FloatDitherArgs *dither = nullptr);

struct FloatProbeArgs {
    const float *in;
    uint64_t channelStride, frameStride;
    uint64_t lo, hi;
    const uint64_t *segFirst;
    uint32_t numSegments, channels;
    uint32_t *reports;
};
hipError_t launch_float_probe(const FloatProbeArgs &a, hipStream_t st);

struct PcmCrcArgs {
    const uint8_t *pcm;
    uint64_t lo, hi;
    const uint64_t *ranges;
    uint32_t numRanges;
    uint32_t *digests;
};
constexpr uint32_t kPcmCrcLaneShift = 6;
constexpr uint32_t kPcmCrcLaneBytes = 1u << kPcmCrcLaneShift;
constexpr uint32_t kPcmCrcWaveBytes = 64 * kPcmCrcLaneBytes;
constexpr uint32_t kPcmCrcBlockBytes = 4 * kPcmCrcWaveBytes;
hipError_t launch_pcm_crc(const PcmCrcArgs &a, hipStream_t st);
uint32_t crc_x8_pow(uint64_t bytes);
uint32_t crc_mul_host(uint32_t a, uint32_t b);

struct VerifyFloatArgs {
    uint32_t *firstMismatch;
    const uint32_t *numSamplesExpected;
    uint64_t channelStride, frameStride;
    uint32_t dither;
    uint32_t pad;
    FloatDitherArgs dz;
};

hipError_t launch_pc_block(const int32_t *in, int32_t *pc, uint32_t rows, uint32_t stride, int32_t num,
                           int16_t *coefs, int32_t numactive, uint32_t chanbits, uint32_t denshift,
                           bool decode, hipStream_t st, bool allowTaps = true);
bool pc_block_taps_ok(int32_t num, int32_t na, uint32_t chanbits, uint32_t denshift);
hipError_t launch_pc_block_taps(const int32_t *in, int32_t *pc, uint32_t rows, uint32_t stride, int32_t num, int16_t *coefs,
                                int32_t na, uint32_t chanbits, uint32_t denshift, hipStream_t st);
hipError_t launch_dyn_comp(uint32_t mb0, uint32_t pb, uint32_t kb, const int32_t *pc, uint32_t rows,
                           uint32_t stride, int32_t numSamples, int32_t bitSize, uint8_t *bits,
                           uint32_t bytesStride, uint32_t *numBits, hipStream_t st);
hipError_t launch_dyn_decomp(uint32_t mb0, uint32_t pb, uint32_t kb, const uint8_t *bits,
                             uint32_t bytesStride, uint32_t rows, int32_t *pc, uint32_t stride,
                             int32_t numSamples, int32_t maxSize, uint32_t *numBits, int32_t *status,
                             hipStream_t st);

}
```

Baseline: 29550.

## Precompute per-packet pack plans in a scan-stage kernel

Adds a per-packet PackPlan (spans, offsets, pre-assembled header words) computed by a new k_scan_plans kernel after the size scan. k_pack reads the plan instead of rebuilding the header with LDS atomics and recomputing span geometry in every block. The seam path now uses 32-bit arithmetic throughout. The cost is an extra kernel launch and a 240-byte-per-packet workspace write and read.

```diff
diff --git a/alac_amd/csrc/alac_capi.hip b/alac_amd/csrc/alac_capi.hip
--- a/alac_amd/csrc/alac_capi.hip
+++ b/alac_amd/csrc/alac_capi.hip
@@ -179,6 +179,7 @@
     uint64_t resA, resB, resC, bits1, cost2, state, flags, rowReady, cls, colChain;
     uint64_t bitWordsB, bitsB;
     uint64_t segBad;
+    uint64_t plans;
     uint32_t chainsPad, colsPad;
 };
 
@@ -230,6 +231,8 @@
     }
     L.segBad = off;
     off += 256;
+    L.plans = off;
+    off = align_up(off + (uint64_t)numPackets * sizeof(PackPlan), 256);
     L.total = off;
     return L;
 }
@@ -637,6 +640,7 @@
     pa.offsets = c.offsets;
     pa.out = c.out;
     pa.segBad = ea.segBad;
+    pa.plans = (PackPlan *)(ws + L.plans);
     constexpr uint32_t EV = kEventBlocks * (kNumStages + 1);
     hipEvent_t *ev = nullptr;
     if (c.timed && ctx->profile && (uint64_t)(ctx->profCalls + 1) * EV <= ctx->events.size())
diff --git a/alac_amd/csrc/alac_dev.hpp b/alac_amd/csrc/alac_dev.hpp
--- a/alac_amd/csrc/alac_dev.hpp
+++ b/alac_amd/csrc/alac_dev.hpp
@@ -2,6 +2,8 @@
 
 #include <hip/hip_runtime.h>
 #include <stdint.h>
+
+#include "alac_pack_plan.hpp"
 
 namespace alacdev {
 
@@ -9,21 +11,10 @@
 constexpr uint32_t kPB0 = 40;
 constexpr uint32_t kMB0 = 10;
 constexpr uint32_t kKB0 = 14;
-constexpr uint32_t kDenShift = 9;
 constexpr uint32_t kMaxPrefix = 9;
 constexpr uint32_t kMaxRunBits = 16;
 constexpr uint32_t kMeanClamp = 0xffffu;
-constexpr int32_t kMixBits = 2;
 constexpr int32_t kMaxRes = 4;
-
-__host__ __device__ constexpr uint32_t bytes_per_sample(uint32_t depth)
-{
-    return depth == 16 ? 2u : (depth == 32 ? 4u : 3u);
-}
-__host__ __device__ constexpr uint32_t bytes_shifted(uint32_t depth)
-{
-    return depth == 32 ? 2u : (depth >= 24 ? 1u : 0u);
-}
 
 __device__ __forceinline__ int32_t sext(int32_t x, uint32_t chanshift)
 {
diff --git a/alac_amd/csrc/alac_encode.hip b/alac_amd/csrc/alac_encode.hip
--- a/alac_amd/csrc/alac_encode.hip
+++ b/alac_amd/csrc/alac_encode.hip
@@ -364,28 +364,30 @@
     if (n == 0 && i == 0) offsets[0] = 0;
 }
 
-
-__device__ __forceinline__ uint32_t words_fetch32(const uint32_t *w, uint32_t len, uint32_t s0)
-{
-    const uint32_t i = s0 >> 5, sh = s0 & 31;
-    const uint32_t nw = (len + 31) >> 5;
-    const uint32_t a = w[i];
-    const uint32_t b = (i + 1 < nw) ? w[i + 1] : 0u;
-    uint32_t v = sh ? ((a << sh) | (b >> (32 - sh))) : a;
-    const uint32_t rem = len - s0;
-    if (rem < 32) v &= ~0u << (32 - rem);
-    return v;
-}
+struct ScanPlanArgs {
+    const PacketRec *recs;
+    const LpcChan *lpc;
+    PackPlan *plans;
+    uint32_t frameSize, depth, channels;
+};
+__global__ __launch_bounds__(64) void k_scan_plans(const uint64_t *offsets, uint32_t n, const uint32_t *segBad, ScanPlanArgs S)
+{
+    if (segBad && *segBad != 0) return;
+    const uint32_t i = blockIdx.x * 64u + threadIdx.x;
+    if (i < n)
+        write_pack_plan(&S.plans[i], S.recs[i], offsets[i], S.frameSize, S.depth, S.channels, S.lpc ? S.lpc + (uint64_t)i * 2 : nullptr);
+}
+
 
 template <int W, class Field>
-__device__ __forceinline__ uint32_t fields_fetch32(Field &&field, uint32_t count, uint64_t s0)
+__device__ __forceinline__ uint32_t fields_fetch32(Field &&field, uint32_t count, uint32_t s0)
 {
     uint32_t out = 0;
 #pragma unroll
     for (int half = 0; half < 2; half++) {
-        const uint64_t s = s0 + 16u * half;
-        uint32_t t = (uint32_t)(s / W);
-        const uint32_t o = (uint32_t)(s % W);
+        const uint32_t s = s0 + 16u * half;
+        uint32_t t = s / W;
+        const uint32_t o = s - t * W;
         uint64_t acc = 0;
         uint32_t have = 0;
         while (have < o + 16) {
@@ -400,72 +402,33 @@
 }
 
 template <class Fetch>
-__device__ __forceinline__ uint32_t take(Fetch &&fetch32, uint64_t len, int64_t s)
-{
-    if (s >= (int64_t)len || s <= -32) return 0;
-    if (s >= 0) return fetch32((uint64_t)s);
-    return fetch32(0) >> (uint32_t)(-s);
+__device__ __forceinline__ uint32_t take(Fetch &&fetch32, uint32_t len, int32_t s)
+{
+    if (s >= (int32_t)len || s <= -32) return 0;
+    if (s >= 0) return fetch32((uint32_t)s);
+    return fetch32(0u) >> (uint32_t)(-s);
 }
 
 template <int DEPTH, int CH>
-__global__ __launch_bounds__(256) void k_pack(PackArgs A, uint32_t numPackets)
-{
-    constexpr uint32_t kHdrWords = (23 + 32 + 16 + 2 * (16 + 16 * kLpcMaxOrder) + 31) / 32;
-    __shared__ uint32_t hdr[kHdrWords];
+__global__ __launch_bounds__(256) void k_pack(PackArgs A, const PackPlan *__restrict__ plans, uint32_t numPackets)
+{
     const uint32_t lane = threadIdx.x & 63;
     const bool seamWave = (threadIdx.x >> 6) == (blockDim.x >> 6) - 1;
     constexpr uint32_t SHB = bytes_shifted(DEPTH);
-    const uint32_t refused = A.segBad ? *A.segBad : 0u;
-    PacketRec recNext = A.recs[blockIdx.x];
-    uint64_t offNext = A.offsets[blockIdx.x];
-    if (refused) return;
+    if (A.segBad && *A.segBad) return;
     for (uint32_t p = blockIdx.x; p < numPackets; p += gridDim.x) {
-    const PacketRec rec = recNext;
-    const uint64_t outOff = offNext;
-    if (p + gridDim.x < numPackets) {
-        recNext = A.recs[p + gridDim.x];
-        offNext = A.offsets[p + gridDim.x];
-    }
-    const uint32_t N = rec.numSamples;
-    const uint32_t partial = (N != A.frameSize);
+    const PackPlan &P = plans[p];
+    const uint32_t N = P.numSamples, escape = P.escape, mis = P.mis, nb = P.nb, nSeam = P.nSeam;
+    const uint32_t lenHdr = P.lenHdr, offU = P.offU, offV = P.offV, offEnd = P.offEnd;
+    const uint32_t offFirst = lenHdr, lenFirst = offU - lenHdr, lenU = offV - offU, lenV = offEnd - offV;
+    const PackSpan s1 = P.span[0], s2 = P.span[1], s3 = P.span[2];
     const uint8_t *pk = A.pcm + (uint64_t)p * A.frameSize * CH * bytes_per_sample(DEPTH);
-    uint32_t hb = 3 + 4 + 12 + 4 + (partial ? 32u : 0u);
-    if (!rec.escape) {
-        hb += 16;
-        for (int c = 0; c < CH; c++) hb += 16 + 16 * rec.c[c].num;
-    }
-    const uint64_t lenHdr = hb;
-    const uint64_t lenShift = rec.escape ? 0 : (uint64_t)N * CH * SHB * 8;
-    const uint64_t lenU = rec.escape ? 0 : rec.c[0].bits;
-    const uint64_t lenV = (rec.escape || CH == 1) ? 0 : rec.c[1].bits;
-    const uint64_t lenRaw = rec.escape ? (uint64_t)N * CH * DEPTH : 0;
-    const int64_t offShift = (int64_t)lenHdr;
-    const int64_t offU = offShift + (int64_t)lenShift;
-    const int64_t offV = offU + (int64_t)lenU;
-    const int64_t offRaw = offV + (int64_t)lenV;
-    const int64_t offEnd = offRaw + (int64_t)lenRaw;
-    const uint32_t nb = (uint32_t)((offEnd + 3 + 7) / 8);
-
     const uint32_t *wU = A.bitWords + (uint64_t)p * 2 * A.wcap;
     const uint32_t *wV = wU + A.wcap;
-    const uint32_t mis = (uint32_t)(outOff & 15);
-    uint8_t *outAligned = A.out + (outOff - mis);
-    const uint32_t nwords = (mis + nb + 3) / 4;
+    uint8_t *outAligned = A.out + P.outBase;
 
     auto sampleField = [&](uint32_t t) -> uint32_t { return (uint32_t)load_sample<DEPTH>(pk, t); };
 
-    struct Span {
-        uint32_t w0, w1;
-    };
-    auto span_of = [&](int64_t off, uint64_t len) {
-        const int64_t base = off + (int64_t)mis * 8;
-        Span sp;
-        sp.w0 = ((uint32_t)((base + 31) >> 5) + 3) & ~3u;
-        sp.w1 = (uint32_t)((base + (int64_t)len) >> 5) & ~3u;
-        if (sp.w1 < sp.w0) sp.w1 = sp.w0;
-        return sp;
-    };
-    auto first_bit = [&](const Span &sp, int64_t off) { return (uint32_t)((int64_t)sp.w0 * 32 - (off + (int64_t)mis * 8)); };
     auto load5 = [&](uint32_t a[5], bool have, uint32_t i, uint32_t sh, auto &&src) {
         if constexpr (std::is_pointer_v<std::decay_t<decltype(src)>>) {
             typedef uint32_t U4 __attribute__((ext_vector_type(4), aligned(4)));
@@ -490,8 +453,8 @@
         v.w = __builtin_bswap32(sh ? __builtin_amdgcn_alignbit(a[3], a[4], 32 - sh) : a[3]);
         *(uint4 *)(outAligned + (uint64_t)w * 4) = v;
     };
-    auto copy_span = [&](const Span &sp, int64_t off, auto &&srcWord) {
-        const uint32_t fb = first_bit(sp, off), i0 = fb >> 5, sh = fb & 31;
+    auto copy_span = [&](const PackSpan &sp, auto &&srcWord) {
+        const uint32_t i0 = sp.i0, sh = sp.sh;
         for (uint32_t w = sp.w0 + 4 * threadIdx.x; w < sp.w1; w += 4 * blockDim.x) {
             uint32_t a[5];
             load5(a, true, i0 + (w - sp.w0), sh, srcWord);
@@ -554,11 +517,9 @@
             }
         }
     };
-    auto copy_bulk = [&](const Span &ss, const Span &sa, const Span &sb) {
+    auto copy_bulk = [&](const PackSpan &ss, const PackSpan &sa, const PackSpan &sb) {
         constexpr bool SHIFT = SHB != 0 && (DEPTH == 24 || DEPTH == 32);
-        const uint32_t fs = first_bit(ss, offShift), is0 = fs >> 5, shS = fs & 31;
-        const uint32_t fa = first_bit(sa, offU), ia0 = fa >> 5, shA = fa & 31;
-        const uint32_t fb = first_bit(sb, offV), ib0 = fb >> 5, shB = fb & 31;
+        const uint32_t is0 = ss.i0, shS = ss.sh, ia0 = sa.i0, shA = sa.sh, ib0 = sb.i0, shB = sb.sh;
         const uint32_t ns = SHIFT ? (ss.w1 - ss.w0) / 4 : 0u, na = (sa.w1 - sa.w0) / 4, nb2 = CH == 2 ? (sb.w1 - sb.w0) / 4 : 0u;
         for (uint32_t g = threadIdx.x; g < max(ns, max(na, nb2)); g += blockDim.x) {
             const bool hs = g < ns, ha = g < na, hb = g < nb2;
@@ -573,55 +534,26 @@
                 if (hb) store4(b, shB, sb.w0 + 4 * g);
         }
     };
-    Span spU = {0, 0}, spV = {0, 0}, spR = {0, 0}, spS = {0, 0};
-    if (!rec.escape) {
-        if constexpr (SHB != 0 && (DEPTH == 24 || DEPTH == 32)) spS = span_of(offShift, lenShift);
-        spU = span_of(offU, lenU);
-        if constexpr (CH == 2) spV = span_of(offV, lenV);
-    } else {
-        spR = span_of(offRaw, lenRaw);
-    }
-    const Span s1 = rec.escape ? spR : spS, s2 = spU, s3 = spV;
-    const uint32_t nSeam = nwords - (s1.w1 - s1.w0) - (s2.w1 - s2.w0) - (s3.w1 - s3.w0);
-    auto seam_word = [&](uint32_t k) {
-        uint32_t aw = k;
-        if (aw >= s1.w0) aw += s1.w1 - s1.w0;
-        if (aw >= s2.w0) aw += s2.w1 - s2.w0;
-        if (aw >= s3.w0) aw += s3.w1 - s3.w0;
-        return aw;
-    };
     struct Pair {
         uint32_t a, b;
     };
-    auto fetch_pair = [&](const uint32_t *w, uint64_t len, int64_t s) {
-        const uint32_t nw = (uint32_t)((len + 31) >> 5);
-        const uint32_t i = s > 0 ? (uint32_t)(s >> 5) : 0u;
-        const uint32_t last = nw ? nw - 1 : 0u;
+    auto fetch_pair = [&](const uint32_t *w, uint32_t len, int32_t s) {
+        uint32_t ia, ib;
+        pack_pair_index(len, s, ia, ib);
         Pair pr;
-        pr.a = w[min(i, last)];
-        pr.b = w[min(i + 1, last)];
+        pr.a = w[ia];
+        pr.b = w[ib];
         return pr;
     };
-    auto combine_pair = [&](const Pair &pr, uint64_t len, int64_t s) -> uint32_t {
-        if (s >= (int64_t)len || s <= -32) return 0u;
-        const uint32_t s0 = s > 0 ? (uint32_t)s : 0u;
-        const uint32_t i = s0 >> 5, sh = s0 & 31;
-        const uint32_t nw = (uint32_t)((len + 31) >> 5);
-        const uint32_t b = (i + 1 < nw) ? pr.b : 0u;
-        uint32_t v = sh ? ((pr.a << sh) | (b >> (32 - sh))) : pr.a;
-        const uint32_t rem = (uint32_t)len - s0;
-        if (rem < 32) v &= ~0u << (32 - rem);
-        return s < 0 ? v >> (uint32_t)(-s) : v;
-    };
     auto seam_store = [&](uint32_t aw, uint32_t v) {
-        const int64_t b0 = (int64_t)aw * 4 - mis;
-        if (b0 >= 0 && b0 + 4 <= (int64_t)nb) {
+        const int32_t b0 = (int32_t)(aw * 4) - (int32_t)mis;
+        if (b0 >= 0 && b0 + 4 <= (int32_t)nb) {
             *(uint32_t *)(outAligned + (uint64_t)aw * 4) = __builtin_bswap32(v);
         } else {
 #pragma unroll
             for (int b = 0; b < 4; b++) {
-                const int64_t pb = b0 + b;
-                if (pb >= 0 && pb < (int64_t)nb) outAligned[(uint64_t)aw * 4 + b] = (uint8_t)(v >> (24 - 8 * b));
+                const int32_t pb = b0 + b;
+                if (pb >= 0 && pb < (int32_t)nb) outAligned[(uint64_t)aw * 4 + b] = (uint8_t)(v >> (24 - 8 * b));
             }
         }
     };
@@ -653,92 +585,57 @@
             if (!fullA) a = shift_word_slow(i);
             if (!fullB) b = shift_word_slow(i + 1);
             uint32_t v = sh ? ((a << sh) | (b >> (32 - sh))) : a;
-            const uint32_t rem = (uint32_t)lenShift - s0;
+            const uint32_t rem = lenFirst - s0;
             if (rem < 32) v &= ~0u << (32 - rem);
             return v;
         }
     };
-    auto seam_rest = [&](int64_t bp) {
-        uint32_t v = take([&](uint64_t s0) { return words_fetch32(hdr, (uint32_t)lenHdr, (uint32_t)s0); }, lenHdr, bp);
-        if (!rec.escape) {
+    auto seam_rest = [&](int32_t bp) {
+        uint32_t v = 0;
+        if (!escape) {
             if constexpr (SHB != 0)
-                v |= take([&](uint64_t s0) { return shift_fetch32((uint32_t)s0); }, lenShift, bp - offShift);
-        } else {
-            v |= take([&](uint64_t s0) { return fields_fetch32<DEPTH>(sampleField, N * CH, s0); }, lenRaw, bp - offRaw);
-        }
-        v |= take([](uint64_t s0) { return 0xE0000000u << (uint32_t)s0; }, 3, bp - offEnd);
+                v |= take([&](uint32_t s0) { return shift_fetch32(s0); }, lenFirst, bp - (int32_t)offFirst);
+        } else {
+            v |= take([&](uint32_t s0) { return fields_fetch32<DEPTH>(sampleField, N * CH, s0); }, lenFirst, bp - (int32_t)offFirst);
+        }
+        v |= take([](uint32_t s0) { return 0xE0000000u << s0; }, 3, bp - (int32_t)offEnd);
         return v;
     };
-    Pair seamU = {0, 0}, seamV = {0, 0};
-    const uint32_t seamAw = seam_word(lane);
-    const int64_t seamBp = (int64_t)seamAw * 32 - (int64_t)mis * 8;
-    if (seamWave) {
-        if (lane < kHdrWords) hdr[lane] = 0;
-        const uint32_t perChan = A.lpc ? 1u + kLpcMaxOrder : 9u;
-        const LpcChan *lpcRec = A.lpc ? A.lpc + (uint64_t)p * 2 : nullptr;
-        const uint32_t base = 23 + (partial ? 32u : 0u);
-        for (uint32_t f = lane; f < 3 + perChan * CH; f += 64) {
-            uint32_t fpos = 0, fn = 0, fv = 0;
-            if (f == 0) {
-                fn = 23;
-                fv = ((CH == 2 ? 1u : 0u) << 20) | (rec.escape ? ((partial << 3) | 1u) : ((partial << 3) | (SHB << 1)));
-            } else if (f == 1) {
-                fpos = 23, fn = partial ? 32u : 0u, fv = N;
-            } else if (!rec.escape) {
-                if (f == 2) {
-                    fpos = base, fn = 16, fv = CH == 2 ? (((uint32_t)kMixBits << 8) | (rec.mixRes & 0xffu)) : 0u;
-                } else {
-                    const uint32_t c = (f - 3) / perChan, k = (f - 3) - perChan * c;
-                    const uint32_t num = c ? rec.c[CH - 1].num : rec.c[0].num;
-                    const uint32_t cstart = base + 16 + (c ? 16 + 16 * (uint32_t)rec.c[0].num : 0u);
-                    const bool own = lpcRec && lpcRec[c].num != 0;
-                    if (k == 0) {
-                        const uint32_t den = own ? lpcRec[c].den : kDenShift;
-                        fpos = cstart, fn = 16, fv = (((0u << 4) | den) << 8) | ((4u << 5) | num);
-                    } else if (k - 1 < num) {
-                        uint32_t coef = 0;
-                        if (own) {
-                            coef = (uint16_t)lpcRec[c].coefs[k - 1];
-                        } else {
-#pragma unroll
-                            for (int q = 0; q < 8; q++) {
-                                const uint32_t cq = (uint16_t)(c ? rec.c[CH - 1].coefs[q] : rec.c[0].coefs[q]);
-                                coef = (k - 1 == (uint32_t)q) ? cq : coef;
-                            }
-                        }
-                        fpos = cstart + 16 * k, fn = 16, fv = coef;
-                    }
-                }
-            }
-            if (fn) {
-                const uint32_t i = fpos >> 5, o = fpos & 31;
-                const uint64_t x = ((uint64_t)fv << (64 - fn)) >> o;
-                atomicOr(&hdr[i], (uint32_t)(x >> 32));
-                if (o + fn > 32) atomicOr(&hdr[i + 1], (uint32_t)x);
-            }
-        }
-        if (!rec.escape && lane < nSeam) {
-            seamU = fetch_pair(wU, lenU, seamBp - offU);
-            if constexpr (CH == 2) seamV = fetch_pair(wV, lenV, seamBp - offV);
-        }
-    }
-    if (!rec.escape) {
-        copy_bulk(spS, spU, spV);
+    auto seam_value = [&](int32_t bp, const Pair &h, const Pair &u, const Pair &v2) {
+        uint32_t v = seam_rest(bp) | pack_pair_combine(h.a, h.b, lenHdr, bp);
+        if (!escape) {
+            v |= pack_pair_combine(u.a, u.b, lenU, bp - (int32_t)offU);
+            if constexpr (CH == 2) v |= pack_pair_combine(v2.a, v2.b, lenV, bp - (int32_t)offV);
+        }
+        return v;
+    };
+    Pair seamH = {0, 0}, seamU = {0, 0}, seamV = {0, 0};
+    const uint32_t seamAw = pack_seam_word(s1, s2, s3, lane);
+    const int32_t seamBp = (int32_t)(seamAw * 32) - (int32_t)(mis * 8);
+    if (seamWave && lane < nSeam) {
+        seamH = fetch_pair(P.hdr, lenHdr, seamBp);
+        if (!escape) {
+            seamU = fetch_pair(wU, lenU, seamBp - (int32_t)offU);
+            if constexpr (CH == 2) seamV = fetch_pair(wV, lenV, seamBp - (int32_t)offV);
+        }
+    }
+    if (!escape) {
+        copy_bulk(s1, s2, s3);
     } else if constexpr (DEPTH == 16) {
         const uint32_t *pw = (const uint32_t *)pk;
-        copy_span(spR, offRaw, [&](uint32_t i) {
+        copy_span(s1, [&](uint32_t i) {
             const uint32_t x = pw[i];
             return (x << 16) | (x >> 16);
         });
     } else if constexpr (DEPTH == 32) {
         const uint32_t *pw = (const uint32_t *)pk;
-        copy_span(spR, offRaw, [&](uint32_t i) { return pw[i]; });
+        copy_span(s1, [&](uint32_t i) { return pw[i]; });
     } else if constexpr (DEPTH == 24) {
         const uint32_t *pw = (const uint32_t *)pk;
         const uint32_t ndw = (N * CH * 3 + 3) / 4;
-        const uint32_t fb = first_bit(spR, offRaw), i0 = fb >> 5, sh = fb & 31;
-        for (uint32_t w = spR.w0 + 4 * threadIdx.x; w < spR.w1; w += 4 * blockDim.x) {
-            const uint32_t i = i0 + (w - spR.w0);
+        const uint32_t i0 = s1.i0, sh = s1.sh;
+        for (uint32_t w = s1.w0 + 4 * threadIdx.x; w < s1.w1; w += 4 * blockDim.x) {
+            const uint32_t i = i0 + (w - s1.w0);
             const uint32_t g = i / 3, r = i - 3 * g, base = 3 * g;
             uint32_t d[9];
             if (base + 9 <= ndw) {
@@ -765,9 +662,9 @@
     } else {
         const uint32_t *pw = (const uint32_t *)pk;
         const uint32_t ndw = (N * CH * 3 + 3) / 4;
-        const uint32_t fb = first_bit(spR, offRaw), i0 = fb >> 5, sh = fb & 31;
-        for (uint32_t w = spR.w0 + 4 * threadIdx.x; w < spR.w1; w += 4 * blockDim.x) {
-            const uint32_t i = i0 + (w - spR.w0);
+        const uint32_t i0 = s1.i0, sh = s1.sh;
+        for (uint32_t w = s1.w0 + 4 * threadIdx.x; w < s1.w1; w += 4 * blockDim.x) {
+            const uint32_t i = i0 + (w - s1.w0);
             const uint32_t g = i / 5, r = i - 5 * g, base = 6 * g;
             uint32_t d[12];
             if (base + 12 <= ndw) {
@@ -805,23 +702,16 @@
     }
 
     if (seamWave) {
-        if (lane < nSeam) {
-            uint32_t v = seam_rest(seamBp);
-            if (!rec.escape) {
-                v |= combine_pair(seamU, lenU, seamBp - offU);
-                if constexpr (CH == 2) v |= combine_pair(seamV, lenV, seamBp - offV);
-            }
-            seam_store(seamAw, v);
-        }
+        if (lane < nSeam) seam_store(seamAw, seam_value(seamBp, seamH, seamU, seamV));
         for (uint32_t k = lane + 64; k < nSeam; k += 64) {
-            const uint32_t aw = seam_word(k);
-            const int64_t bp = (int64_t)aw * 32 - (int64_t)mis * 8;
-            uint32_t v = seam_rest(bp);
-            if (!rec.escape) {
-                v |= combine_pair(fetch_pair(wU, lenU, bp - offU), lenU, bp - offU);
-                if constexpr (CH == 2) v |= combine_pair(fetch_pair(wV, lenV, bp - offV), lenV, bp - offV);
-            }
-            seam_store(aw, v);
+            const uint32_t aw = pack_seam_word(s1, s2, s3, k);
+            const int32_t bp = (int32_t)(aw * 32) - (int32_t)(mis * 8);
+            Pair u = {0, 0}, v2 = {0, 0};
+            if (!escape) {
+                u = fetch_pair(wU, lenU, bp - (int32_t)offU);
+                if constexpr (CH == 2) v2 = fetch_pair(wV, lenV, bp - (int32_t)offV);
+            }
+            seam_store(aw, seam_value(bp, fetch_pair(P.hdr, lenHdr, bp), u, v2));
         }
     }
     }
@@ -835,14 +725,16 @@
     if (ev && recordScan) ALAC_TRY(hipEventRecord(ev[kStageScan], st));
     ALAC_TRY(launch_kernel(k_scan_sizes, dim3(numPackets / 1024 + 1), dim3(1024), st, (const uint32_t *)packetBytes,
                            (uint64_t *)pa.offsets, numPackets, pa.segBad));
+    const ScanPlanArgs sp = {pa.recs, pa.lpc, pa.plans, pa.frameSize, (uint32_t)DEPTH, channels};
+    ALAC_TRY(launch_kernel(k_scan_plans, dim3(numPackets / 64 + 1), dim3(64), st, pa.offsets, numPackets, pa.segBad, sp));
     if (ev) ALAC_TRY(hipEventRecord(ev[kStagePack], st));
     static const uint32_t tpb = getenv("ALAC_HIP_PACK_TPB") ? (uint32_t)atoi(getenv("ALAC_HIP_PACK_TPB")) : 128u;
     static const uint32_t wgs = getenv("ALAC_HIP_PACK_WGS") ? (uint32_t)atoi(getenv("ALAC_HIP_PACK_WGS")) : (1u << 20);
     const uint32_t grid = numPackets < wgs ? numPackets : wgs;
     if (channels == 2)
-        ALAC_TRY(launch_kernel(k_pack<DEPTH, 2>, dim3(grid), dim3(tpb), st, pa, numPackets));
+        ALAC_TRY(launch_kernel(k_pack<DEPTH, 2>, dim3(grid), dim3(tpb), st, pa, (const PackPlan *)pa.plans, numPackets));
     else
-        ALAC_TRY(launch_kernel(k_pack<DEPTH, 1>, dim3(grid), dim3(tpb), st, pa, numPackets));
+        ALAC_TRY(launch_kernel(k_pack<DEPTH, 1>, dim3(grid), dim3(tpb), st, pa, (const PackPlan *)pa.plans, numPackets));
     return ev ? hipEventRecord(ev[kNumStages], st) : hipSuccess;
 }
 
diff --git a/alac_amd/csrc/alac_kernels.hpp b/alac_amd/csrc/alac_kernels.hpp
--- a/alac_amd/csrc/alac_kernels.hpp
+++ b/alac_amd/csrc/alac_kernels.hpp
@@ -2,6 +2,8 @@
 
 #include <hip/hip_runtime.h>
 #include <stdint.h>
+
+#include "alac_pack_plan.hpp"
 
 namespace alacdev {
 
@@ -22,27 +24,6 @@
     return launch_kernel_lds(kernel, grid, block, 0, st, args...);
 }
 
-struct ChanRec {
-    uint32_t bits;
-    uint16_t num;
-    uint16_t pad;
-    int16_t coefs[8];
-};
-struct PacketRec {
-    uint32_t numSamples;
-    uint32_t escape;
-    uint32_t mixRes;
-    uint32_t totalBits;
-    ChanRec c[2];
-};
-static_assert(sizeof(PacketRec) == 64, "PacketRec layout");
-constexpr int kLpcMaxOrder = 30;
-struct LpcChan {
-    uint16_t den;
-    uint16_t num;
-    int16_t coefs[kLpcMaxOrder];
-};
-static_assert(sizeof(LpcChan) == 64, "LpcChan layout");
 
 struct EncodeArgs {
     const uint8_t *pcm;
@@ -73,6 +54,7 @@
     uint8_t *out;
     const uint32_t *segBad;
     const LpcChan *lpc = nullptr;
+    PackPlan *plans = nullptr;
 };
 
 struct LpcArgs {
diff --git a/alac_amd/csrc/alac_pack_plan.hpp b/alac_amd/csrc/alac_pack_plan.hpp
--- /dev/null
+++ b/alac_amd/csrc/alac_pack_plan.hpp
@@ -0,0 +1,196 @@
+#pragma once
+
+#include <stdint.h>
+
+#if defined(__HIPCC__)
+#define ALAC_PLAN_HD __host__ __device__
+#else
+#define ALAC_PLAN_HD
+#endif
+
+namespace alacdev {
+
+constexpr uint32_t kDenShift = 9;
+constexpr int32_t kMixBits = 2;
+
+ALAC_PLAN_HD constexpr uint32_t bytes_per_sample(uint32_t depth)
+{
+    return depth == 16 ? 2u : (depth == 32 ? 4u : 3u);
+}
+ALAC_PLAN_HD constexpr uint32_t bytes_shifted(uint32_t depth)
+{
+    return depth == 32 ? 2u : (depth >= 24 ? 1u : 0u);
+}
+
+struct ChanRec {
+    uint32_t bits;
+    uint16_t num;
+    uint16_t pad;
+    int16_t coefs[8];
+};
+struct PacketRec {
+    uint32_t numSamples;
+    uint32_t escape;
+    uint32_t mixRes;
+    uint32_t totalBits;
+    ChanRec c[2];
+};
+static_assert(sizeof(PacketRec) == 64, "PacketRec layout");
+constexpr int kLpcMaxOrder = 30;
+struct LpcChan {
+    uint16_t den;
+    uint16_t num;
+    int16_t coefs[kLpcMaxOrder];
+};
+static_assert(sizeof(LpcChan) == 64, "LpcChan layout");
+
+constexpr uint32_t kHdrWords = (23 + 32 + 16 + 2 * (16 + 16 * kLpcMaxOrder) + 31) / 32;
+
+struct PackSpan {
+    uint32_t w0, w1, i0, sh;
+};
+
+struct alignas(16) PackPlan {
+    uint64_t outBase;
+    uint32_t mis;
+    uint32_t nb;
+    uint32_t nwords;
+    uint32_t nSeam;
+    uint32_t escape;
+    uint32_t numSamples;
+    uint32_t lenHdr, offU, offV, offEnd;
+    PackSpan span[3];
+    uint32_t hdr[kHdrWords];
+};
+static_assert(sizeof(PackPlan) == 240, "PackPlan layout");
+
+ALAC_PLAN_HD inline PackSpan pack_span_of(uint32_t mis, uint32_t off, uint32_t len)
+{
+    const uint32_t base = off + mis * 8;
+    PackSpan sp;
+    sp.w0 = (((base + 31) >> 5) + 3) & ~3u;
+    sp.w1 = ((base + len) >> 5) & ~3u;
+    if (sp.w1 < sp.w0) sp.w1 = sp.w0;
+    const uint32_t first = sp.w0 * 32 - base;
+    sp.i0 = first >> 5;
+    sp.sh = first & 31;
+    return sp;
+}
+
+ALAC_PLAN_HD inline uint32_t pack_seam_word(const PackSpan &s1, const PackSpan &s2, const PackSpan &s3, uint32_t k)
+{
+    uint32_t aw = k;
+    if (aw >= s1.w0) aw += s1.w1 - s1.w0;
+    if (aw >= s2.w0) aw += s2.w1 - s2.w0;
+    if (aw >= s3.w0) aw += s3.w1 - s3.w0;
+    return aw;
+}
+
+ALAC_PLAN_HD inline void write_pack_plan(PackPlan *out, const PacketRec &rec, uint64_t outOffset, uint32_t frameSize,
+                                        uint32_t depth, uint32_t channels, const LpcChan *lpcRec)
+{
+    PackPlan &P = *out;
+    const uint32_t N = rec.numSamples, escape = rec.escape ? 1u : 0u;
+    const uint32_t partial = N != frameSize ? 1u : 0u;
+    const uint32_t SHB = bytes_shifted(depth);
+    const uint32_t num0 = rec.c[0].num, num1 = channels == 2 ? rec.c[1].num : 0u;
+    uint32_t hb = 3 + 4 + 12 + 4 + (partial ? 32u : 0u);
+    if (!escape) hb += 16 + (16 + 16 * num0) + (channels == 2 ? 16 + 16 * num1 : 0u);
+    const uint32_t lenFirst = escape ? N * channels * depth : N * channels * SHB * 8;
+    const uint32_t offU = hb + lenFirst;
+    const uint32_t offV = offU + (escape ? 0u : rec.c[0].bits);
+    const uint32_t offEnd = offV + ((escape || channels == 1) ? 0u : rec.c[1].bits);
+    const uint32_t mis = (uint32_t)(outOffset & 15);
+    const uint32_t nb = (offEnd + 3 + 7) / 8, nwords = (mis + nb + 3) / 4;
+    const PackSpan s1 = pack_span_of(mis, hb, lenFirst);
+    const PackSpan s2 = pack_span_of(mis, offU, offV - offU);
+    const PackSpan s3 = pack_span_of(mis, offV, offEnd - offV);
+    P.outBase = outOffset - mis;
+    P.mis = mis;
+    P.nb = nb;
+    P.nwords = nwords;
+    P.nSeam = nwords - (s1.w1 - s1.w0) - (s2.w1 - s2.w0) - (s3.w1 - s3.w0);
+    P.escape = escape;
+    P.numSamples = N;
+    P.lenHdr = hb;
+    P.offU = offU;
+    P.offV = offV;
+    P.offEnd = offEnd;
+    P.span[0] = s1;
+    P.span[1] = s2;
+    P.span[2] = s3;
+
+    const bool own0 = lpcRec && lpcRec[0].num != 0, own1 = channels == 2 && lpcRec && lpcRec[1].num != 0;
+    const int16_t *co0 = own0 ? lpcRec[0].coefs : rec.c[0].coefs, *co1 = own1 ? lpcRec[1].coefs : rec.c[1].coefs;
+    const uint32_t cap0 = own0 ? (uint32_t)kLpcMaxOrder : 8u, cap1 = own1 ? (uint32_t)kLpcMaxOrder : 8u;
+    const uint32_t chan0 = ((own0 ? (uint32_t)lpcRec[0].den : kDenShift) << 8) | (4u << 5) | num0;
+    const uint32_t chan1 = ((own1 ? (uint32_t)lpcRec[1].den : kDenShift) << 8) | (4u << 5) | num1;
+    const uint32_t mix = channels == 2 ? (((uint32_t)kMixBits << 8) | (rec.mixRes & 0xffu)) : 0u;
+    auto g = [&](uint32_t j) -> uint32_t {
+        const uint32_t jj = j - 2 * partial;
+        const uint32_t k0 = jj - 2, k1 = jj - 3 - num0;
+        const uint32_t c0 = (uint16_t)co0[k0 < cap0 ? k0 : cap0 - 1], c1 = (uint16_t)co1[k1 < cap1 ? k1 : cap1 - 1];
+        uint32_t v = 0;
+        if (channels == 2 && k1 < num1 && k1 < cap1) v = c1;
+        if (channels == 2 && jj == 2 + num0) v = chan1;
+        if (k0 < num0) v = k0 < cap0 ? c0 : 0u;
+        if (jj == 1) v = chan0;
+        if (jj == 0) v = mix;
+        if (escape || j < 2 * partial) v = 0;
+        if (j < 2 * partial) v = j == 0 ? N >> 16 : N & 0xffffu;
+        return v;
+    };
+    const uint32_t flags = escape ? ((partial << 3) | 1u) : ((partial << 3) | (SHB << 1));
+    const uint32_t first23 = ((channels == 2 ? 1u : 0u) << 20) | flags;
+    uint32_t carry = g(0);
+    P.hdr[0] = (first23 << 9) | (carry >> 7);
+    constexpr uint32_t kHdrWordsShort = (23 + 32 + 16 + 2 * (16 + 16 * 8) + 31) / 32;
+#if defined(__HIP_DEVICE_COMPILE__)
+#pragma unroll
+#endif
+    for (uint32_t w = 1; w < kHdrWordsShort; w++) {
+        const uint32_t mid = g(2 * w - 1), next = g(2 * w);
+        P.hdr[w] = ((carry & 0x7fu) << 25) | (mid << 9) | (next >> 7);
+        carry = next;
+    }
+    if (hb > 32 * kHdrWordsShort) {
+        for (uint32_t w = kHdrWordsShort; w < kHdrWords; w++) {
+            const uint32_t mid = g(2 * w - 1), next = g(2 * w);
+            P.hdr[w] = ((carry & 0x7fu) << 25) | (mid << 9) | (next >> 7);
+            carry = next;
+        }
+    } else {
+        for (uint32_t w = kHdrWordsShort; w < kHdrWords; w++) P.hdr[w] = 0;
+    }
+}
+
+ALAC_PLAN_HD inline PackPlan make_pack_plan(const PacketRec &rec, uint64_t outOffset, uint32_t frameSize, uint32_t depth,
+                                            uint32_t channels, const LpcChan *lpcRec)
+{
+    PackPlan P;
+    write_pack_plan(&P, rec, outOffset, frameSize, depth, channels, lpcRec);
+    return P;
+}
+
+ALAC_PLAN_HD inline void pack_pair_index(uint32_t len, int32_t s, uint32_t &ia, uint32_t &ib)
+{
+    const uint32_t nw = (len + 31) >> 5;
+    const uint32_t i = s > 0 ? (uint32_t)s >> 5 : 0u;
+    const uint32_t last = nw ? nw - 1 : 0u;
+    ia = i < last ? i : last;
+    ib = i + 1 < last ? i + 1 : last;
+}
+ALAC_PLAN_HD inline uint32_t pack_pair_combine(uint32_t a, uint32_t b, uint32_t len, int32_t s)
+{
+    if (len == 0 || s >= (int32_t)len || s <= -32) return 0u;
+    const uint32_t s0 = s > 0 ? (uint32_t)s : 0u;
+    const uint32_t i = s0 >> 5, sh = s0 & 31;
+    const uint32_t nw = (len + 31) >> 5;
+    if (i + 1 >= nw) b = 0u;
+    uint32_t v = sh ? ((a << sh) | (b >> (32 - sh))) : a;
+    const uint32_t rem = len - s0;
+    if (rem < 32) v &= ~0u << (32 - rem);
+    return s < 0 ? v >> (uint32_t)(-s) : v;
+}
+
+}
```

Result: no change. 29430 (-0.4%).
